# mooch443/trex

Measured on AMD Instinct MI355X. Metric: frames/s end-to-end (segment+CNN-ID), 2048x2048 x100 individuals, higher is better.
Workload: dtype fp16x3-split

## Files before the change

### include/trexhip.h

```cpp
#ifndef TREXHIP_H
#define TREXHIP_H
#include <stddef.h>
#include <stdint.h>
#ifdef __cplusplus
extern "C" {
#endif

#define TREXHIP_ABI_VERSION 25

enum {
    TREXHIP_OK = 0,
    TREXHIP_E_INVALID = -1,
    TREXHIP_E_DEVICE = -2,
    TREXHIP_E_CAPACITY = -3,
    TREXHIP_E_UNSUPPORTED = -4,
    TREXHIP_E_NOMEM = -5
};

#define TREXHIP_FRAME_OVERFLOW_RUNS   1u
#define TREXHIP_FRAME_OVERFLOW_OUTPUT 2u
#define TREXHIP_FRAME_MALFORMED       4u

typedef struct trexhip_params {
    int32_t device;
    int32_t width, height;
    int32_t max_batch;
    int32_t max_runs;
    int32_t max_blobs;
    int32_t max_pixels;
    int32_t threshold;
    int32_t threshold_maximum;
    int32_t enable_difference;
    int32_t absolute_difference;
    int32_t image_invert;
    int32_t inclusive;
    int32_t zero_is_background;
    int32_t connectivity;
    int32_t dilation_size;
    int32_t use_closing;
    int32_t closing_size;
    int32_t n_ranges;
    double  cm_per_pixel;
    double  ranges[16];
    int32_t pixel_encoding;
    int32_t image_adjust, blur_difference, equalize_histogram, correct_luminance, use_adaptive_threshold;
    int32_t device_color_reduce;
    int32_t reserved_[1];
} trexhip_params;
enum { TREXHIP_ENC_GRAY = 0, TREXHIP_ENC_R3G3B2 = 1, TREXHIP_ENC_RGB8 = 2 };

#define TREXHIP_BLOB_IN_RANGE    0u
#define TREXHIP_BLOB_BELOW_RANGE 1u
#define TREXHIP_BLOB_BIG         2u

typedef struct trexhip_run { uint16_t x0, x1, y, pad; } trexhip_run;

typedef struct trexhip_blob {
    uint32_t run_begin, n_runs;
    uint32_t pix_begin, n_pixels;
    uint16_t x0, y0, x1, y1;
    uint32_t bid;
// ... 21 lines not shown
    const trexhip_run* runs;
    const uint8_t* pixels;
    uint32_t pixel_channels;
    uint32_t reserved_;
} trexhip_batch_result;

typedef struct trexhip_device_view {
    const trexhip_frame_info* frames;
    const trexhip_blob* blobs;
    const trexhip_run* runs;
    const uint8_t* pixels;
    const uint32_t* totals;
    const uint32_t* blob_frame;
} trexhip_device_view;

typedef struct trexhip_ctx trexhip_ctx;

int trexhip_abi_version(void);
const char* trexhip_last_error(void);
void trexhip_default_params(trexhip_params* p, int32_t width, int32_t height);

int trexhip_create(const trexhip_params* p, trexhip_ctx** out);
void trexhip_destroy(trexhip_ctx* ctx);
typedef struct trexhip_live_params {
    int32_t threshold, threshold_maximum, inclusive;
    int32_t enable_difference, absolute_difference, image_invert, zero_is_background;
    int32_t n_ranges;
    double  cm_per_pixel;
    double  ranges[16];
} trexhip_live_params;
int trexhip_get_live_params(trexhip_ctx* ctx, trexhip_live_params* out);
int trexhip_update_params(trexhip_ctx* ctx, const trexhip_live_params* lp);
int trexhip_set_stream(trexhip_ctx* ctx, void* hip_stream);

int trexhip_set_background(trexhip_ctx* ctx, const uint8_t* gray, int32_t stride);
int trexhip_set_background_device(trexhip_ctx* ctx, const uint8_t* d_gray);
int trexhip_set_background_color(trexhip_ctx* ctx, const uint8_t* bgr, int32_t stride_bytes, int32_t channels, int32_t color_channel);
int trexhip_set_background_color_device(trexhip_ctx* ctx, const uint8_t* d_bgr, int32_t channels, int32_t color_channel);

int trexhip_generate_average_device(trexhip_ctx* ctx, const uint8_t* d_frames, int32_t n, int32_t method);
int trexhip_get_background(trexhip_ctx* ctx, uint8_t* gray, int32_t stride);

int trexhip_segment_device(trexhip_ctx* ctx, const uint8_t* d_frames, int32_t n);
int trexhip_segment(trexhip_ctx* ctx, const uint8_t* const* frames, int32_t stride, int32_t n);
int trexhip_segment_color(trexhip_ctx* ctx, const uint8_t* const* frames, int32_t stride, int32_t n,
                          int32_t channels, int32_t color_channel);
int trexhip_segment_color_device(trexhip_ctx* ctx, const uint8_t* d_color_frames, int32_t n, int32_t channels, int32_t color_channel);
int trexhip_pixel_channels(trexhip_ctx* ctx);
int trexhip_device_alloc(trexhip_ctx* ctx, size_t bytes, void** out_device_ptr);
int trexhip_device_free(trexhip_ctx* ctx, void* device_ptr);
int trexhip_copy_to_host(trexhip_ctx* ctx, void* host_dst, const void* device_src, size_t bytes);
int trexhip_copy_to_device(trexhip_ctx* ctx, void* device_dst, const void* host_src, size_t bytes);
int trexhip_fetch(trexhip_ctx* ctx, trexhip_batch_result* out);
int trexhip_device_view_get(trexhip_ctx* ctx, trexhip_device_view* out);
int trexhip_synchronize(trexhip_ctx* ctx);

int trexhip_pack_frames_v6_device(trexhip_ctx* ctx, const uint64_t* timestamps, uint8_t* d_out, size_t capacity, uint64_t* d_offsets);

int trexhip_load_frames_v6_device(trexhip_ctx* ctx, const uint8_t* d_bodies, const uint64_t* d_offsets, int32_t n_frames, uint64_t* d_timestamps);

size_t trexhip_lzo1x_bound(size_t n);
int trexhip_lzo1x_compress(const uint8_t* in, size_t n, uint8_t* out, size_t capacity, size_t* out_len);
int trexhip_pv_write_frames(const uint8_t* bodies, const uint64_t* offsets, int32_t n_frames, int32_t always_compress, uint64_t file_offset,
                            uint8_t* out, size_t capacity, uint64_t* index_table, size_t* out_bytes);
int trexhip_lzo1x_decompress(const uint8_t* in, size_t n, uint8_t* out, size_t capacity, size_t* out_len);
int trexhip_pv_read_frames(const uint8_t* data, size_t bytes, uint64_t file_offset, const uint64_t* index_table, int32_t n_frames,
                           uint8_t* bodies, size_t capacity, uint64_t* offsets, size_t* out_bytes);

int trexhip_rethreshold_device(trexhip_ctx* ctx, int32_t threshold, int32_t method, const double* size_ranges, int32_t n_ranges);
int trexhip_rethreshold_per_blob_device(trexhip_ctx* ctx, int32_t threshold, const int32_t* d_blob_thresholds, int32_t method,
                                        const double* size_ranges, int32_t n_ranges);
int trexhip_fetch_rethreshold(trexhip_ctx* ctx, trexhip_batch_result* out);

enum { TREXHIP_FILTER_OUTSIDE_INCLUDE = 0, TREXHIP_FILTER_INSIDE_IGNORE = 1, TREXHIP_FILTER_BDX_IGNORED = 2, TREXHIP_FILTER_OUTSIDE_RANGE = 3,
       TREXHIP_FILTER_SECOND_THRESHOLD = 4 };
enum { TREXHIP_DECISION_COMMITTED = 0, TREXHIP_DECISION_BIG = 1, TREXHIP_DECISION_FILTERED = 16, TREXHIP_DECISION_NONE = 255 };
typedef struct trexhip_prefilter_params {
    int32_t track_threshold;
    int32_t method;
    int32_t track_threshold_2;
    int32_t n_ranges;
    float   threshold_ratio_range[2];
    double  size_ranges[16];
} trexhip_prefilter_params;
typedef struct trexhip_prefilter_tables {
    const float*    d_include_points;  const int32_t* d_include_offsets;  int32_t n_include_shapes, n_include_points;
    const float*    d_ignore_points;   const int32_t* d_ignore_offsets;   int32_t n_ignore_shapes, n_ignore_points;
    const uint32_t* d_ignore_bdx;      const int32_t* d_ignore_bdx_offsets;  int32_t n_ignore_bdx, reserved_;
    int32_t*        d_second_count;
} trexhip_prefilter_tables;
void trexhip_default_prefilter_params(trexhip_prefilter_params* p);
int trexhip_prefilter_device(trexhip_ctx* ctx, const trexhip_prefilter_params* pp, const trexhip_prefilter_tables* tables ,
                             uint8_t* d_decision, int32_t* d_order, int32_t* d_counts, int32_t* d_presumed_nr);

typedef struct trexhip_split_params {
    int32_t track_threshold;
    int32_t track_posture_threshold;
    int32_t calculate_posture;
    int32_t algorithm;
    float   blob_split_max_shrink;
    float   blob_split_global_shrink_limit;
    int32_t n_ranges;
    int32_t reserved_;
    double  size_ranges[16];
} trexhip_split_params;
typedef struct trexhip_split_info {
// ... 18 lines not shown
    int32_t outline_smooth_step;
    int32_t outline_approximate;
    float   outline_curvature_range_ratio;
    float   midline_walk_offset;
    int32_t max_points;
    int32_t posture_closing_steps, peak_mode, posture_direction_smoothing;
} trexhip_posture_params;
typedef struct trexhip_posture_info { int32_t status, n_outline, n_segments, tail_index, head_index, n_traced, reserved[2]; } trexhip_posture_info;
void trexhip_default_posture_params(trexhip_posture_params* p);
int trexhip_posture_device(trexhip_ctx* ctx, int32_t table, const trexhip_posture_params* pp, int32_t n_blobs,
                           float* d_outline, float* d_segments, trexhip_posture_info* d_info);

int trexhip_posture_auto_device(trexhip_ctx* ctx, const trexhip_posture_params* pp, int32_t method, int32_t track_posture_threshold,
                                int32_t n_blobs, float* d_outline, float* d_segments, trexhip_posture_info* d_info,
                                int32_t* d_threshold_used, int32_t* d_iterations);

typedef struct trexhip_midline_params {
    int32_t midline_resolution;
    float   midline_stiff_percentage;
    int32_t midline_invert;
    int32_t midline_start_with_head;
} trexhip_midline_params;
typedef struct trexhip_midline_info { int32_t status, n; float len, angle, offx, offy; int32_t reserved[2]; } trexhip_midline_info;
void trexhip_default_midline_params(trexhip_midline_params* p);
int trexhip_midline_device(trexhip_ctx* ctx, const trexhip_midline_params* mp, int32_t n_blobs, int32_t max_points,
                           const trexhip_posture_info* d_posture_info, float* d_segments, float* d_midline,
                           trexhip_midline_info* d_midline_info);
int trexhip_midline_movement_device(trexhip_ctx* ctx, const trexhip_midline_params* mp, int32_t n_blobs, int32_t max_points,
                                    const trexhip_posture_info* d_posture_info, float* d_segments, float* d_midline,
                                    trexhip_midline_info* d_midline_info, const float* d_movement_direction);

enum { TREXHIP_NORMALIZE_NONE = 0, TREXHIP_NORMALIZE_MOMENTS = 1, TREXHIP_NORMALIZE_POSTURE = 2 };
int trexhip_crops_device(trexhip_ctx* ctx, uint8_t* d_crops, int32_t n_blobs, int32_t out_w, int32_t out_h,
                         int32_t normalization, int32_t difference);

int trexhip_crops_transformed_device(trexhip_ctx* ctx, uint8_t* d_crops, int32_t n_blobs, int32_t out_w, int32_t out_h,
                                     const float* transforms, const float* midline_lengths, int32_t use_legacy,
                                     float image_scale, int32_t difference);
int trexhip_crops_posture_device(trexhip_ctx* ctx, uint8_t* d_crops, int32_t n_blobs, int32_t out_w, int32_t out_h,
                                 const trexhip_midline_info* d_midline_info, const float* midline_lengths, int32_t use_legacy,
                                 float image_scale, int32_t difference);

int trexhip_load_weights(trexhip_ctx* ctx, const void* blob, size_t bytes);
int trexhip_num_classes(trexhip_ctx* ctx);
int trexhip_network_channels(trexhip_ctx* ctx);
int trexhip_network_image_size(trexhip_ctx* ctx, int32_t* width, int32_t* height);
enum { TREXHIP_NET_V118_3 = 0, TREXHIP_NET_V100 = 1, TREXHIP_NET_V110 = 2, TREXHIP_NET_V119 = 3, TREXHIP_NET_V200 = 4 };
int trexhip_network_version(trexhip_ctx* ctx);
size_t trexhip_network_blob_bytes(int32_t version, int32_t classes, int32_t channels, int32_t width, int32_t height);
int trexhip_identify_chunk_crops(trexhip_ctx* ctx, int32_t* crops);
enum { TREXHIP_CNN_FP32 = 0, TREXHIP_CNN_BF16X6 = 1, TREXHIP_CNN_BF16X3 = 2, TREXHIP_CNN_FP16X3 = 3 };
int trexhip_set_identity_precision(trexhip_ctx* ctx, int32_t mode);
int trexhip_identify_device(trexhip_ctx* ctx, const uint8_t* d_crops, int32_t n, float* d_probs, float* d_logits);
int trexhip_identify(trexhip_ctx* ctx, const uint8_t* crops, int32_t n, float* probs);
int trexhip_identify_guard_stats(trexhip_ctx* ctx, uint32_t* rerun_crops, uint32_t* whole_batch);
int trexhip_identify_skip_stats(trexhip_ctx* ctx, uint32_t* passes, uint32_t* listed, uint64_t* bytes_filled);

int trexhip_identify_skip3_stats(trexhip_ctx* ctx, uint32_t* pairs, uint32_t* listed, uint32_t* passes, uint64_t* bytes_filled);

int trexhip_identify_skip3x_stats(trexhip_ctx* ctx, uint32_t* crops_windowed, uint32_t* windowed_passes, uint32_t* full_passes);

int trexhip_identify_skipx_stats(trexhip_ctx* ctx, uint32_t* crops_windowed, uint32_t* windowed_passes, uint32_t* full_passes);

int trexhip_identify_bgrow_stats(trexhip_ctx* ctx, uint32_t* rows_read, uint32_t* rows_made);

int trexhip_identify_fc1_stats(trexhip_ctx* ctx, uint32_t* rows, uint32_t* listed);

int trexhip_export_id_table_device(trexhip_ctx* ctx, const float* d_probs, int32_t n_blobs, int32_t classes,
                                   uint32_t frame_base, void* d_table, int32_t max_rows);
int trexhip_export_id_table_ex_device(trexhip_ctx* ctx, const float* d_probs, int32_t n_blobs, int32_t classes, uint32_t frame_base,
                                      const float* d_midline, const trexhip_midline_info* d_midline_info, int32_t midline_resolution,
                                      void* d_table, int32_t max_rows);

typedef struct trexhip_comm trexhip_comm;
int trexhip_comm_unique_id(void* id128);
int trexhip_comm_create(trexhip_ctx* ctx, const void* id128, int32_t rank, int32_t world, trexhip_comm** out);
void trexhip_comm_destroy(trexhip_comm* comm);
int trexhip_comm_rank(trexhip_comm* comm);
int trexhip_comm_world(trexhip_comm* comm);
int trexhip_comm_gather_device(trexhip_comm* comm, const void* d_send, size_t bytes, void* d_recv_rank0);
int trexhip_comm_gather_device_on(trexhip_comm* comm, trexhip_ctx* stream_ctx, const void* d_send, size_t bytes, void* d_recv_rank0);
int trexhip_comm_count_ranks(trexhip_comm* comm, int32_t* ranks_seen);

enum { TREXHIP_STAGE_ROWS = 0, TREXHIP_STAGE_SEGMENT_ALL = 1, TREXHIP_STAGE_CONV2 = 2, TREXHIP_STAGE_CONV3 = 3,
       TREXHIP_STAGE_CNN_ALL = 4, TREXHIP_STAGE_CROPS = 5, TREXHIP_STAGE_POSTURE = 6,
       TREXHIP_STAGE_UPLOAD_COPY = 8, TREXHIP_STAGE_UPLOAD_DMA = 9, TREXHIP_STAGE_COUNT = 10 };
int trexhip_profile_enable(trexhip_ctx* ctx, int32_t on);
int trexhip_profile_read(trexhip_ctx* ctx, int32_t stage, double* total_ms, int64_t* launches);
int trexhip_profile_reset(trexhip_ctx* ctx);

#define TREXHIP_NET_CATEGORY 100
typedef struct trexhip_trainer trexhip_trainer;
typedef struct {
    int32_t max_batch;
    float lr;
    float beta1, beta2, eps;
    float bn_momentum;
    float dropout;
    int32_t precision;
    uint64_t seed;
} trexhip_train_params;
size_t trexhip_weight_blob_bytes(int32_t classes, int32_t channels);
int trexhip_trainer_create(trexhip_ctx* ctx, const void* blob, size_t bytes, const trexhip_train_params* params, trexhip_trainer** out);
void trexhip_trainer_destroy(trexhip_trainer* trainer);
int trexhip_trainer_set_lr(trexhip_trainer* trainer, float lr);
int64_t trexhip_trainer_steps(trexhip_trainer* trainer);
int trexhip_trainer_image_size(trexhip_trainer* trainer, int32_t* width, int32_t* height);
int trexhip_trainer_version(trexhip_trainer* trainer, int32_t* version);
size_t trexhip_trainer_keep_mask_bytes(trexhip_trainer* trainer, int32_t n);
int trexhip_train_step_device(trexhip_trainer* trainer, const float* d_inputs, const int32_t* d_targets, int32_t n, const uint8_t* d_keep_masks,
                              float* loss, int32_t* correct);
int trexhip_train_eval_device(trexhip_trainer* trainer, const float* d_inputs, const int32_t* d_targets, int32_t n, float* loss, int32_t* correct);
int trexhip_train_eval(trexhip_trainer* trainer, const float* inputs, const int32_t* targets, int32_t n, float* loss, int32_t* correct);
int trexhip_train_step(trexhip_trainer* trainer, const float* inputs, const int32_t* targets, int32_t n, const uint8_t* keep_masks, float* loss,
                       int32_t* correct);
int trexhip_train_predict_device(trexhip_trainer* trainer, const uint8_t* d_crops, int32_t n, float* d_probs);
int trexhip_trainer_read(trexhip_trainer* trainer, int32_t tensor, int32_t kind, float* out, size_t count);
int trexhip_trainer_export(trexhip_trainer* trainer, void* blob, size_t capacity, size_t* bytes);

typedef struct {
    float degrees;
    float translate_x, translate_y;
    float brightness_lo, brightness_hi;
    float contrast_lo, contrast_hi;
    float saturation_lo, saturation_hi;
    float hue_lo, hue_hi;
    uint64_t seed;
} trexhip_augment_params;
typedef struct {
    float angle; int32_t tx, ty;
    float brightness, contrast, saturation, hue;
    int32_t order;
} trexhip_augment_draw;
void trexhip_default_augment_params(trexhip_augment_params* p, int32_t width, int32_t height);
int trexhip_augment_device(trexhip_ctx* ctx, const trexhip_augment_params* ap, const uint8_t* d_pool, const int32_t* d_pool_targets,
                           int32_t pool_size, const int32_t* indices, int32_t n, int32_t width, int32_t height, int32_t channels,
                           trexhip_augment_draw* d_draws, int32_t draws_given, uint64_t counter, float* d_out, int32_t* d_targets_out);

typedef struct {
// ... 68 lines not shown
```

### trex_amd/capi.py

```python
import collections
import ctypes as C
import os
import numpy as np

_HERE = os.path.dirname(os.path.abspath(__file__))
LIB_PATH = os.environ.get("TREXHIP_LIB_PATH") or os.path.join(_HERE, "libtrexhip.so")
_LIB = None

RUN_DTYPE = np.dtype([("x0", "<u2"), ("x1", "<u2"), ("y", "<u2"), ("pad", "<u2")])
BLOB_DTYPE = np.dtype([
    ("run_begin", "<u4"), ("n_runs", "<u4"), ("pix_begin", "<u4"), ("n_pixels", "<u4"),
    ("x0", "<u2"), ("y0", "<u2"), ("x1", "<u2"), ("y1", "<u2"),
    ("bid", "<u4"), ("px_min_max", "<u4"), ("parent", "<u4"), ("flags", "<u4"),
    ("m10", "<u8"), ("m01", "<u8"), ("m20", "<u8"), ("m11", "<u8"), ("m02", "<u8"),
    ("sp", "<u8"), ("spx", "<u8"), ("spy", "<u8"),
])
INFO_DTYPE = np.dtype([
    ("n_blobs", "<u4"), ("n_runs", "<u4"), ("n_pixels", "<u4"),
    ("blob_begin", "<u4"), ("run_begin", "<u4"), ("pix_begin", "<u4"),
    ("n_raw_runs", "<u4"), ("n_raw_blobs", "<u4"), ("flags", "<u4"), ("reserved", "<u4", (3,)),
])
assert BLOB_DTYPE.itemsize == 104 and RUN_DTYPE.itemsize == 8 and INFO_DTYPE.itemsize == 48

CNN_FP32, CNN_BF16X6, CNN_BF16X3, CNN_FP16X3 = 0, 1, 2, 3
STAGE_ROWS, STAGE_SEGMENT_ALL, STAGE_CONV2, STAGE_CONV3, STAGE_CNN_ALL, STAGE_CROPS, STAGE_POSTURE = 0, 1, 2, 3, 4, 5, 6
STAGE_UPLOAD_COPY, STAGE_UPLOAD_DMA = 8, 9


class Params(C.Structure):
    _fields_ = [
        ("device", C.c_int32), ("width", C.c_int32), ("height", C.c_int32),
        ("max_batch", C.c_int32), ("max_runs", C.c_int32), ("max_blobs", C.c_int32), ("max_pixels", C.c_int32),
        ("threshold", C.c_int32), ("threshold_maximum", C.c_int32),
        ("enable_difference", C.c_int32), ("absolute_difference", C.c_int32),
        ("image_invert", C.c_int32), ("inclusive", C.c_int32), ("zero_is_background", C.c_int32),
        ("connectivity", C.c_int32), ("dilation_size", C.c_int32), ("use_closing", C.c_int32),
        ("closing_size", C.c_int32), ("n_ranges", C.c_int32),
        ("cm_per_pixel", C.c_double), ("ranges", C.c_double * 16),
        ("pixel_encoding", C.c_int32),
        ("image_adjust", C.c_int32), ("blur_difference", C.c_int32), ("equalize_histogram", C.c_int32), ("correct_luminance", C.c_int32),
        ("use_adaptive_threshold", C.c_int32), ("device_color_reduce", C.c_int32), ("reserved_", C.c_int32 * 1),
    ]


class LiveParams(C.Structure):
    _fields_ = [("threshold", C.c_int32), ("threshold_maximum", C.c_int32), ("inclusive", C.c_int32),
                ("enable_difference", C.c_int32), ("absolute_difference", C.c_int32), ("image_invert", C.c_int32), ("zero_is_background", C.c_int32),
                ("n_ranges", C.c_int32), ("cm_per_pixel", C.c_double), ("ranges", C.c_double * 16)]


class PostureParams(C.Structure):
    _fields_ = [("outline_resample", C.c_float), ("outline_smooth_samples", C.c_int32), ("outline_smooth_step", C.c_int32),
                ("outline_approximate", C.c_int32), ("outline_curvature_range_ratio", C.c_float),
                ("midline_walk_offset", C.c_float), ("max_points", C.c_int32),
                ("posture_closing_steps", C.c_int32), ("peak_mode", C.c_int32), ("posture_direction_smoothing", C.c_int32)]


class MidlineParams(C.Structure):
    _fields_ = [("midline_resolution", C.c_int32), ("midline_stiff_percentage", C.c_float), ("midline_invert", C.c_int32),
                ("midline_start_with_head", C.c_int32)]


class SplitParams(C.Structure):
    _fields_ = [("track_threshold", C.c_int32), ("track_posture_threshold", C.c_int32), ("calculate_posture", C.c_int32), ("algorithm", C.c_int32),
                ("blob_split_max_shrink", C.c_float), ("blob_split_global_shrink_limit", C.c_float), ("n_ranges", C.c_int32), ("reserved_", C.c_int32),
                ("size_ranges", C.c_double * 16)]


class PrefilterParams(C.Structure):
    _fields_ = [("track_threshold", C.c_int32), ("method", C.c_int32), ("track_threshold_2", C.c_int32), ("n_ranges", C.c_int32),
                ("threshold_ratio_range", C.c_float * 2), ("size_ranges", C.c_double * 16)]


class PrefilterTables(C.Structure):
    _fields_ = [("d_include_points", C.c_void_p), ("d_include_offsets", C.c_void_p), ("n_include_shapes", C.c_int32), ("n_include_points", C.c_int32),
                ("d_ignore_points", C.c_void_p), ("d_ignore_offsets", C.c_void_p), ("n_ignore_shapes", C.c_int32), ("n_ignore_points", C.c_int32),
                ("d_ignore_bdx", C.c_void_p), ("d_ignore_bdx_offsets", C.c_void_p), ("n_ignore_bdx", C.c_int32), ("reserved_", C.c_int32),
                ("d_second_count", C.c_void_p)]

# ... 58 lines not shown

AUGMENT_DRAW_DTYPE = np.dtype([("angle", "<f4"), ("tx", "<i4"), ("ty", "<i4"), ("brightness", "<f4"), ("contrast", "<f4"), ("saturation", "<f4"),
                               ("hue", "<f4"), ("order", "<i4")])
assert AUGMENT_DRAW_DTYPE.itemsize == 32
AUGMENT_IDENTITY_ORDER = 0xE4


class UniquenessResult(C.Structure):
    _fields_ = [("good_frames", C.c_uint32), ("bad_frames", C.c_uint32), ("good_ratio", C.c_float), ("mean_unique", C.c_float), ("mean_unique_raw", C.c_float)]


class ValidationMetrics:
    __slots__ = ("confusion", "per_class_accuracy", "good_frames", "bad_frames", "good_ratio", "mean_unique", "mean_unique_raw",
                 "unique_percent", "unique_percent_raw", "uniqueness_per_class")

    def __init__(self):
        for k in self.__slots__:
            setattr(self, k, None)


class ClassAverages:
    __slots__ = ("samples", "values", "max_index", "max_p")

    def __init__(self, samples, values, max_index, max_p):
        self.samples, self.values, self.max_index, self.max_p = samples, values, max_index, max_p


class VisualFieldResult:
    __slots__ = VF_OUTPUTS

    def __init__(self):
        for k in self.__slots__:
            setattr(self, k, None)


TrackletLabels = collections.namedtuple("TrackletLabels", "counts rows label share skipped")


SYMBOLS = [
    "trexhip_abi_version", "trexhip_network_channels", "trexhip_network_image_size", "trexhip_network_version", "trexhip_network_blob_bytes", "trexhip_identify_chunk_crops", "trexhip_comm_unique_id", "trexhip_comm_create", "trexhip_comm_destroy", "trexhip_comm_rank", "trexhip_comm_world", "trexhip_comm_gather_device", "trexhip_comm_gather_device_on", "trexhip_comm_count_ranks", "trexhip_last_error", "trexhip_default_params", "trexhip_create", "trexhip_destroy",
    "trexhip_set_stream", "trexhip_get_live_params", "trexhip_update_params", "trexhip_set_background", "trexhip_set_background_device", "trexhip_set_background_color", "trexhip_set_background_color_device", "trexhip_generate_average_device", "trexhip_get_background", "trexhip_segment_device",
    "trexhip_segment", "trexhip_segment_color", "trexhip_segment_color_device", "trexhip_rethreshold_device", "trexhip_rethreshold_per_blob_device", "trexhip_fetch_rethreshold", "trexhip_fetch", "trexhip_device_view_get", "trexhip_synchronize",
    "trexhip_profile_enable", "trexhip_profile_read", "trexhip_profile_reset",
    "trexhip_default_posture_params", "trexhip_posture_device", "trexhip_posture_auto_device", "trexhip_pack_frames_v6_device", "trexhip_crops_device", "trexhip_pixel_channels", "trexhip_device_alloc", "trexhip_device_free", "trexhip_copy_to_host", "trexhip_copy_to_device", "trexhip_crops_transformed_device", "trexhip_crops_posture_device", "trexhip_default_midline_params", "trexhip_midline_device", "trexhip_midline_movement_device", "trexhip_default_split_params", "trexhip_split_search_device", "trexhip_export_id_table_device", "trexhip_export_id_table_ex_device", "trexhip_load_weights", "trexhip_set_identity_precision", "trexhip_num_classes", "trexhip_identify_device", "trexhip_identify", "trexhip_identify_guard_stats", "trexhip_identify_skip_stats", "trexhip_identify_skip3_stats", "trexhip_identify_skip3x_stats", "trexhip_identify_skipx_stats", "trexhip_identify_bgrow_stats", "trexhip_identify_fc1_stats",
    "trexhip_weight_blob_bytes", "trexhip_trainer_create", "trexhip_trainer_destroy", "trexhip_trainer_set_lr", "trexhip_trainer_steps", "trexhip_trainer_image_size", "trexhip_trainer_version", "trexhip_trainer_keep_mask_bytes", "trexhip_train_step_device", "trexhip_train_step", "trexhip_train_eval_device", "trexhip_train_eval", "trexhip_trainer_read", "trexhip_trainer_export",
    "trexhip_default_augment_params", "trexhip_augment_device",
    "trexhip_train_predict_device", "trexhip_validation_metrics_device", "trexhip_class_averages_device",
    "trexhip_lzo1x_bound", "trexhip_lzo1x_compress", "trexhip_pv_write_frames",
    "trexhip_load_frames_v6_device", "trexhip_lzo1x_decompress", "trexhip_pv_read_frames",
    "trexhip_default_prefilter_params", "trexhip_prefilter_device",
    "trexhip_default_vf_params", "trexhip_visual_field_device",
    "trexhip_categorize_load_weights", "trexhip_categorize_info", "trexhip_categorize_blob_bytes", "trexhip_categorize_device", "trexhip_categorize",
    "trexhip_tracklet_labels_device", "trexhip_tracklet_medians_device",
]


def lib():
    global _LIB
    if _LIB is None:
        if not os.path.exists(LIB_PATH):
            raise TrexHipError(-1, f"{LIB_PATH} is missing: run __graft_entry__.build() (make -C trex_amd/csrc)")
        L = C.CDLL(LIB_PATH)
        L.trexhip_last_error.restype = C.c_char_p
        L.trexhip_default_params.argtypes = [C.POINTER(Params), C.c_int32, C.c_int32]
        L.trexhip_default_params.restype = None
        L.trexhip_create.argtypes = [C.POINTER(Params), C.POINTER(C.c_void_p)]
        L.trexhip_destroy.argtypes = [C.c_void_p]
        L.trexhip_destroy.restype = None
        L.trexhip_set_stream.argtypes = [C.c_void_p, C.c_void_p]
        L.trexhip_get_live_params.argtypes = [C.c_void_p, C.POINTER(LiveParams)]
        L.trexhip_update_params.argtypes = [C.c_void_p, C.POINTER(LiveParams)]
        L.trexhip_set_background.argtypes = [C.c_void_p, C.c_void_p, C.c_int32]
        L.trexhip_set_background_device.argtypes = [C.c_void_p, C.c_void_p]
        L.trexhip_set_background_color.argtypes = [C.c_void_p, C.c_void_p, C.c_int32, C.c_int32, C.c_int32]
        L.trexhip_set_background_color_device.argtypes = [C.c_void_p, C.c_void_p, C.c_int32, C.c_int32]
        L.trexhip_generate_average_device.argtypes = [C.c_void_p, C.c_void_p, C.c_int32, C.c_int32]
        L.trexhip_get_background.argtypes = [C.c_void_p, C.c_void_p, C.c_int32]
        L.trexhip_segment_device.argtypes = [C.c_void_p, C.c_void_p, C.c_int32]
        L.trexhip_segment.argtypes = [C.c_void_p, C.POINTER(C.c_void_p), C.c_int32, C.c_int32]
        L.trexhip_segment_color.argtypes = [C.c_void_p, C.POINTER(C.c_void_p), C.c_int32, C.c_int32, C.c_int32, C.c_int32]
        L.trexhip_segment_color_device.argtypes = [C.c_void_p, C.c_void_p, C.c_int32, C.c_int32, C.c_int32]
        L.trexhip_rethreshold_device.argtypes = [C.c_void_p, C.c_int32, C.c_int32, C.c_void_p, C.c_int32]
        L.trexhip_rethreshold_per_blob_device.argtypes = [C.c_void_p, C.c_int32, C.c_void_p, C.c_int32, C.c_void_p, C.c_int32]
        L.trexhip_fetch_rethreshold.argtypes = [C.c_void_p, C.POINTER(BatchResult)]
        L.trexhip_fetch.argtypes = [C.c_void_p, C.POINTER(BatchResult)]
        L.trexhip_device_view_get.argtypes = [C.c_void_p, C.POINTER(DeviceView)]
        L.trexhip_synchronize.argtypes = [C.c_void_p]
        L.trexhip_profile_enable.argtypes = [C.c_void_p, C.c_int32]
        L.trexhip_profile_read.argtypes = [C.c_void_p, C.c_int32, C.POINTER(C.c_double), C.POINTER(C.c_int64)]
        L.trexhip_profile_reset.argtypes = [C.c_void_p]
        L.trexhip_default_midline_params.argtypes = [C.POINTER(MidlineParams)]
        L.trexhip_default_midline_params.restype = None
        L.trexhip_midline_device.argtypes = [C.c_void_p, C.POINTER(MidlineParams), C.c_int32, C.c_int32, C.c_void_p, C.c_void_p, C.c_void_p, C.c_void_p]
        L.trexhip_midline_movement_device.argtypes = [C.c_void_p, C.POINTER(MidlineParams), C.c_int32, C.c_int32, C.c_void_p, C.c_void_p, C.c_void_p, C.c_void_p, C.c_void_p]
        L.trexhip_default_split_params.argtypes = [C.POINTER(SplitParams)]
        L.trexhip_default_split_params.restype = None
        L.trexhip_split_search_device.argtypes = [C.c_void_p, C.POINTER(SplitParams), C.c_int32, C.c_void_p, C.c_int32, C.c_void_p, C.c_void_p]
        L.trexhip_crops_posture_device.argtypes = [C.c_void_p, C.c_void_p, C.c_int32, C.c_int32, C.c_int32, C.c_void_p, C.c_void_p, C.c_int32, C.c_float, C.c_int32]
        L.trexhip_default_posture_params.argtypes = [C.POINTER(PostureParams)]
        L.trexhip_default_posture_params.restype = None
        L.trexhip_posture_device.argtypes = [C.c_void_p, C.c_int32, C.POINTER(PostureParams), C.c_int32, C.c_void_p, C.c_void_p, C.c_void_p]
        L.trexhip_posture_auto_device.argtypes = [C.c_void_p, C.POINTER(PostureParams), C.c_int32, C.c_int32, C.c_int32, C.c_void_p, C.c_void_p, C.c_void_p, C.c_void_p, C.c_void_p]
        L.trexhip_crops_transformed_device.argtypes = [C.c_void_p, C.c_void_p, C.c_int32, C.c_int32, C.c_int32, C.c_void_p, C.c_void_p, C.c_int32, C.c_float, C.c_int32]
        L.trexhip_crops_device.argtypes = [C.c_void_p, C.c_void_p] + [C.c_int32] * 5
        L.trexhip_export_id_table_device.argtypes = [C.c_void_p, C.c_void_p, C.c_int32, C.c_int32, C.c_uint32, C.c_void_p, C.c_int32]
        L.trexhip_export_id_table_ex_device.argtypes = [C.c_void_p, C.c_void_p, C.c_int32, C.c_int32, C.c_uint32, C.c_void_p, C.c_void_p, C.c_int32, C.c_void_p, C.c_int32]
        L.trexhip_load_weights.argtypes = [C.c_void_p, C.c_void_p, C.c_size_t]
        L.trexhip_num_classes.argtypes = [C.c_void_p]
        L.trexhip_network_channels.argtypes = [C.c_void_p]
        L.trexhip_network_image_size.argtypes = [C.c_void_p, C.POINTER(C.c_int32), C.POINTER(C.c_int32)]
        L.trexhip_network_version.argtypes = [C.c_void_p]
        L.trexhip_network_blob_bytes.argtypes = [C.c_int32] * 5; L.trexhip_network_blob_bytes.restype = C.c_size_t
        L.trexhip_identify_chunk_crops.argtypes = [C.c_void_p, C.POINTER(C.c_int32)]
        L.trexhip_pack_frames_v6_device.argtypes = [C.c_void_p, C.c_void_p, C.c_void_p, C.c_size_t, C.c_void_p]
        L.trexhip_lzo1x_bound.argtypes = [C.c_size_t]; L.trexhip_lzo1x_bound.restype = C.c_size_t
        L.trexhip_lzo1x_compress.argtypes = [C.c_void_p, C.c_size_t, C.c_void_p, C.c_size_t, C.POINTER(C.c_size_t)]
        L.trexhip_pv_write_frames.argtypes = [C.c_void_p, C.c_void_p, C.c_int32, C.c_int32, C.c_uint64, C.c_void_p, C.c_size_t, C.c_void_p, C.POINTER(C.c_size_t)]
        L.trexhip_load_frames_v6_device.argtypes = [C.c_void_p, C.c_void_p, C.c_void_p, C.c_int32, C.c_void_p]
        L.trexhip_lzo1x_decompress.argtypes = [C.c_void_p, C.c_size_t, C.c_void_p, C.c_size_t, C.POINTER(C.c_size_t)]
        L.trexhip_pv_read_frames.argtypes = [C.c_void_p, C.c_size_t, C.c_uint64, C.c_void_p, C.c_int32, C.c_void_p, C.c_size_t, C.c_void_p, C.POINTER(C.c_size_t)]
        L.trexhip_comm_unique_id.argtypes = [C.c_void_p]
        L.trexhip_comm_create.argtypes = [C.c_void_p, C.c_void_p, C.c_int32, C.c_int32, C.POINTER(C.c_void_p)]
        L.trexhip_comm_destroy.argtypes = [C.c_void_p]
        L.trexhip_comm_destroy.restype = None
        L.trexhip_comm_rank.argtypes = [C.c_void_p]
        L.trexhip_comm_world.argtypes = [C.c_void_p]
        L.trexhip_comm_gather_device.argtypes = [C.c_void_p, C.c_void_p, C.c_size_t, C.c_void_p]
        L.trexhip_comm_gather_device_on.argtypes = [C.c_void_p, C.c_void_p, C.c_void_p, C.c_size_t, C.c_void_p]
        L.trexhip_comm_count_ranks.argtypes = [C.c_void_p, C.POINTER(C.c_int32)]
        L.trexhip_set_identity_precision.argtypes = [C.c_void_p, C.c_int32]
        L.trexhip_identify_device.argtypes = [C.c_void_p, C.c_void_p, C.c_int32, C.c_void_p, C.c_void_p]
        L.trexhip_identify.argtypes = [C.c_void_p, C.c_void_p, C.c_int32, C.c_void_p]
        L.trexhip_identify_guard_stats.argtypes = [C.c_void_p, C.POINTER(C.c_uint32), C.POINTER(C.c_uint32)]
        L.trexhip_identify_skip_stats.argtypes = [C.c_void_p, C.POINTER(C.c_uint32), C.POINTER(C.c_uint32), C.POINTER(C.c_uint64)]
        L.trexhip_identify_skipx_stats.argtypes = [C.c_void_p, C.POINTER(C.c_uint32), C.POINTER(C.c_uint32), C.POINTER(C.c_uint32)]
        L.trexhip_identify_bgrow_stats.argtypes = [C.c_void_p, C.POINTER(C.c_uint32), C.POINTER(C.c_uint32)]
        L.trexhip_identify_skip3x_stats.argtypes = [C.c_void_p, C.POINTER(C.c_uint32), C.POINTER(C.c_uint32), C.POINTER(C.c_uint32)]
        L.trexhip_identify_skip3_stats.argtypes = [C.c_void_p, C.POINTER(C.c_uint32), C.POINTER(C.c_uint32), C.POINTER(C.c_uint32), C.POINTER(C.c_uint64)]
        L.trexhip_identify_fc1_stats.argtypes = [C.c_void_p, C.POINTER(C.c_uint32), C.POINTER(C.c_uint32)]
        L.trexhip_weight_blob_bytes.argtypes = [C.c_int32, C.c_int32]
        L.trexhip_weight_blob_bytes.restype = C.c_size_t
        L.trexhip_trainer_create.argtypes = [C.c_void_p, C.c_void_p, C.c_size_t, C.POINTER(TrainParams), C.POINTER(C.c_void_p)]
        L.trexhip_trainer_destroy.argtypes = [C.c_void_p]
        L.trexhip_trainer_destroy.restype = None
        L.trexhip_trainer_set_lr.argtypes = [C.c_void_p, C.c_float]
        L.trexhip_trainer_steps.argtypes = [C.c_void_p]
        L.trexhip_trainer_steps.restype = C.c_int64
        L.trexhip_trainer_image_size.argtypes = [C.c_void_p, C.POINTER(C.c_int32), C.POINTER(C.c_int32)]
        L.trexhip_trainer_version.argtypes = [C.c_void_p, C.POINTER(C.c_int32)]
        L.trexhip_trainer_keep_mask_bytes.argtypes = [C.c_void_p, C.c_int32]
        L.trexhip_trainer_keep_mask_bytes.restype = C.c_size_t
        L.trexhip_train_step_device.argtypes = [C.c_void_p, C.c_void_p, C.c_void_p, C.c_int32, C.c_void_p, C.POINTER(C.c_float), C.POINTER(C.c_int32)]
        L.trexhip_train_step.argtypes = [C.c_void_p, C.c_void_p, C.c_void_p, C.c_int32, C.c_void_p, C.POINTER(C.c_float), C.POINTER(C.c_int32)]
        L.trexhip_train_eval_device.argtypes = [C.c_void_p, C.c_void_p, C.c_void_p, C.c_int32, C.POINTER(C.c_float), C.POINTER(C.c_int32)]
        L.trexhip_train_eval.argtypes = [C.c_void_p, C.c_void_p, C.c_void_p, C.c_int32, C.POINTER(C.c_float), C.POINTER(C.c_int32)]
        L.trexhip_trainer_read.argtypes = [C.c_void_p, C.c_int32, C.c_int32, C.c_void_p, C.c_size_t]
        L.trexhip_trainer_export.argtypes = [C.c_void_p, C.c_void_p, C.c_size_t, C.POINTER(C.c_size_t)]
        L.trexhip_default_augment_params.argtypes = [C.POINTER(AugmentParams), C.c_int32, C.c_int32]
        L.trexhip_default_augment_params.restype = None
        L.trexhip_augment_device.argtypes = [C.c_void_p, C.POINTER(AugmentParams), C.c_void_p, C.c_void_p, C.c_int32, C.c_void_p, C.c_int32, C.c_int32, C.c_int32,
                                             C.c_int32, C.c_void_p, C.c_int32, C.c_uint64, C.c_void_p, C.c_void_p]
        L.trexhip_train_predict_device.argtypes = [C.c_void_p, C.c_void_p, C.c_int32, C.c_void_p]
        L.trexhip_validation_metrics_device.argtypes = [C.c_void_p, C.c_void_p, C.c_int32, C.c_int32, C.c_void_p, C.c_void_p, C.c_int32, C.c_void_p,
                                                        C.POINTER(UniquenessResult), C.c_void_p, C.c_void_p, C.c_void_p]
        L.trexhip_class_averages_device.argtypes = [C.c_void_p, C.c_void_p, C.c_int32, C.c_int32, C.c_void_p, C.c_int32, C.c_void_p, C.c_void_p, C.c_void_p, C.c_void_p]
        L.trexhip_device_alloc.argtypes = [C.c_void_p, C.c_size_t, C.POINTER(C.c_void_p)]
        L.trexhip_device_free.argtypes = [C.c_void_p, C.c_void_p]
        L.trexhip_copy_to_host.argtypes = [C.c_void_p, C.c_void_p, C.c_void_p, C.c_size_t]
        L.trexhip_copy_to_device.argtypes = [C.c_void_p, C.c_void_p, C.c_void_p, C.c_size_t]
        L.trexhip_default_prefilter_params.argtypes = [C.POINTER(PrefilterParams)]
        L.trexhip_default_prefilter_params.restype = None
        L.trexhip_prefilter_device.argtypes = [C.c_void_p, C.POINTER(PrefilterParams), C.POINTER(PrefilterTables), C.c_void_p, C.c_void_p, C.c_void_p, C.c_void_p]
        L.trexhip_default_vf_params.argtypes = [C.c_void_p, C.POINTER(VfParams)]
        L.trexhip_default_vf_params.restype = None
        L.trexhip_visual_field_device.argtypes = [C.c_void_p, C.POINTER(VfParams), C.c_void_p, C.c_void_p, C.c_void_p, C.c_int32, C.c_void_p, C.c_int32,
                                                  C.c_void_p, C.c_int32, C.c_void_p, C.c_void_p, C.c_void_p, C.c_void_p, C.c_void_p, C.c_void_p]
        L.trexhip_categorize_load_weights.argtypes = [C.c_void_p, C.c_void_p, C.c_size_t]
        L.trexhip_categorize_info.argtypes = [C.c_void_p, C.POINTER(C.c_int32), C.POINTER(C.c_int32), C.POINTER(C.c_int32), C.POINTER(C.c_int32)]
        L.trexhip_categorize_blob_bytes.argtypes = [C.c_int32, C.c_int32, C.c_int32, C.c_int32]
        L.trexhip_categorize_blob_bytes.restype = C.c_size_t
        L.trexhip_categorize_device.argtypes = [C.c_void_p, C.c_void_p, C.c_int32, C.c_void_p, C.c_void_p, C.c_void_p]
        L.trexhip_categorize.argtypes = [C.c_void_p, C.c_void_p, C.c_int32, C.c_void_p]
        L.trexhip_tracklet_labels_device.argtypes = [C.c_void_p, C.c_void_p, C.c_void_p, C.c_int32, C.c_int32, C.c_int32, C.c_void_p, C.c_void_p, C.c_void_p,
                                                     C.c_void_p, C.POINTER(C.c_uint32)]
# ... 110 lines not shown
            bg = np.ascontiguousarray(bg, np.uint8)
            assert bg.shape == (self.params.height, self.params.width)
            _check(lib().trexhip_set_background(self._h, bg.ctypes.data_as(C.c_void_p), bg.shape[1]))
        else:
            assert bg.is_cuda and bg.is_contiguous() and bg.numel() == self.params.height * self.params.width
            _check(lib().trexhip_set_background_device(self._h, C.c_void_p(bg.data_ptr())))

    def generate_average(self, d_frames_ptr, n, method=0):
        _check(lib().trexhip_generate_average_device(self._h, C.c_void_p(d_frames_ptr), n, method))
        out = np.empty((self.params.height, self.params.width), np.uint8)
        _check(lib().trexhip_get_background(self._h, out.ctypes.data_as(C.c_void_p), out.shape[1]))
        return out

    def get_background(self):
        out = np.empty((self.params.height, self.params.width), np.uint8)
        _check(lib().trexhip_get_background(self._h, out.ctypes.data_as(C.c_void_p), out.shape[1]))
        return out

    def segment_device(self, d_ptr, n):
        _check(lib().trexhip_segment_device(self._h, C.c_void_p(d_ptr), n))

    def segment_host(self, frames):
        frames = [np.ascontiguousarray(f, np.uint8) for f in frames]
        ptrs = (C.c_void_p * len(frames))(*[f.ctypes.data for f in frames])
        stride = frames[0].shape[1] if frames else self.params.width
        _check(lib().trexhip_segment(self._h, ptrs, stride, len(frames)))

    def set_background_color(self, bgc, color_channel=-1):
        bgc = np.ascontiguousarray(bgc, np.uint8)
        assert bgc.shape[:2] == (self.params.height, self.params.width)
        _check(lib().trexhip_set_background_color(self._h, bgc.ctypes.data_as(C.c_void_p), bgc.shape[1] * bgc.shape[2], bgc.shape[2], color_channel))

    def segment_color_host(self, frames, color_channel=-1):
        frames = [np.ascontiguousarray(f, np.uint8) for f in frames]
        ch = frames[0].shape[2]
        ptrs = (C.c_void_p * len(frames))(*[f.ctypes.data for f in frames])
        _check(lib().trexhip_segment_color(self._h, ptrs, frames[0].shape[1] * ch, len(frames), ch, color_channel))

    def segment_color_device(self, d_color_ptr, n, channels, color_channel=-1):
        _check(lib().trexhip_segment_color_device(self._h, C.c_void_p(d_color_ptr), n, channels, color_channel))

    def synchronize(self):
        _check(lib().trexhip_synchronize(self._h))

    def fetch_raw(self, rethreshold=False):
        r = BatchResult()
        rc = (lib().trexhip_fetch_rethreshold if rethreshold else lib().trexhip_fetch)(self._h, C.byref(r))
        if rc != 0 and rc != -3:
            _check(rc)
        if rc == -3:
            self.last_capacity_error = lib().trexhip_last_error().decode()
        return r

    def fetch(self, copy=True, rethreshold=False):
        r = BatchResult()
        rc = (lib().trexhip_fetch_rethreshold if rethreshold else lib().trexhip_fetch)(self._h, C.byref(r))
        malformed = rc == -1 and r.n_frames > 0 and bool((_from_addr(r.frames, r.n_frames, INFO_DTYPE)["flags"] & FRAME_MALFORMED).any())
        if rc != 0 and rc != -3 and not malformed:
            _check(rc)
        info = _from_addr(r.frames, r.n_frames, INFO_DTYPE)
        blobs = _from_addr(r.blobs, r.total_blobs, BLOB_DTYPE)
        runs = _from_addr(r.runs, r.total_runs, RUN_DTYPE)
        pc = int(r.pixel_channels) or 1
        pixels = _from_addr(r.pixels, r.total_pixels * pc, np.dtype(np.uint8))
        out = []
        for i in range(r.n_frames):
            fi = info[i]
            if fi["flags"]:
                out.append(FrameResult(fi.copy(), np.zeros(0, BLOB_DTYPE), np.zeros(0, RUN_DTYPE), np.zeros(0, np.uint8)))
                continue
            b = blobs[fi["blob_begin"]:fi["blob_begin"] + fi["n_blobs"]]
            ru = runs[fi["run_begin"]:fi["run_begin"] + fi["n_runs"]]
            px = pixels[int(fi["pix_begin"]) * pc:(int(fi["pix_begin"]) + int(fi["n_pixels"])) * pc]
            if copy:
                b, ru, px = b.copy(), ru.copy(), px.copy()
            out.append(FrameResult(fi.copy(), b, ru, px))
        if malformed:
            e = TrexHipError(rc, lib().trexhip_last_error().decode())
            e.frames = out
            raise e
        if rc == -3:
            self.last_capacity_error = lib().trexhip_last_error().decode()
        return out

    def posture_device(self, n_blobs, d_outline_ptr, d_segments_ptr, d_info_ptr, table=0, **kw):
        pp = PostureParams()
        lib().trexhip_default_posture_params(C.byref(pp))
        for k, v in kw.items():
            setattr(pp, k, v)
        _check(lib().trexhip_posture_device(self._h, table, C.byref(pp), n_blobs, C.c_void_p(d_outline_ptr),
                                            C.c_void_p(d_segments_ptr), C.c_void_p(d_info_ptr)))
        return pp

    def posture_auto_device(self, n_blobs, d_outline_ptr, d_segments_ptr, d_info_ptr, method=0, track_posture_threshold=15, d_threshold_ptr=0, d_iterations_ptr=0, **kw):
        pp = PostureParams()
        lib().trexhip_default_posture_params(C.byref(pp))
        for k, v in kw.items():
            setattr(pp, k, v)
        _check(lib().trexhip_posture_auto_device(self._h, C.byref(pp), method, track_posture_threshold, n_blobs, C.c_void_p(d_outline_ptr),
                                                 C.c_void_p(d_segments_ptr), C.c_void_p(d_info_ptr), C.c_void_p(d_threshold_ptr or 0), C.c_void_p(d_iterations_ptr or 0)))

    def pack_frames_v6_device(self, d_out_ptr, capacity, d_offsets_ptr, timestamps=None):
        ts = np.ascontiguousarray(timestamps, np.uint64) if timestamps is not None else None
        _check(lib().trexhip_pack_frames_v6_device(self._h, ts.ctypes.data if ts is not None else None, C.c_void_p(d_out_ptr), capacity, C.c_void_p(d_offsets_ptr)))

    def load_frames_v6_device(self, d_bodies_ptr, d_offsets_ptr, n, d_timestamps_ptr=0):
# ... 70 lines not shown
        return int(c.value)

    def probabilities(self, crops):
        crops = np.ascontiguousarray(crops, np.uint8)
        w, h = self.network_image_size()
        if w:
            want = (h, w, lib().trexhip_network_channels(self._h))
            if crops.ndim != 4 or tuple(crops.shape[1:]) != want:
                raise ValueError(f"crops must have shape (n, {want[0]}, {want[1]}, {want[2]}) for the loaded network, got {crops.shape}")
        n = crops.shape[0]
        out = np.empty((n, self.num_classes()), np.float32)
        _check(lib().trexhip_identify(self._h, crops.ctypes.data_as(C.c_void_p), n, out.ctypes.data_as(C.c_void_p)))
        return out

    def guard_stats(self):
        a, b = C.c_uint32(0), C.c_uint32(0)
        _check(lib().trexhip_identify_guard_stats(self._h, C.byref(a), C.byref(b)))
        return int(a.value), bool(b.value)

    def skip_stats(self):
        a, b, c = C.c_uint32(0), C.c_uint32(0), C.c_uint64(0)
        _check(lib().trexhip_identify_skip_stats(self._h, C.byref(a), C.byref(b), C.byref(c)))
        return int(a.value), int(b.value), int(c.value)

    def skipx_stats(self):
        a, b, c = C.c_uint32(0), C.c_uint32(0), C.c_uint32(0)
        _check(lib().trexhip_identify_skipx_stats(self._h, C.byref(a), C.byref(b), C.byref(c)))
        return int(a.value), int(b.value), int(c.value)

    def bgrow_stats(self):
        a, b = C.c_uint32(0), C.c_uint32(0)
        _check(lib().trexhip_identify_bgrow_stats(self._h, C.byref(a), C.byref(b)))
        return int(a.value), int(b.value)

    def skip3_stats(self):
        a, b, c, d = C.c_uint32(0), C.c_uint32(0), C.c_uint32(0), C.c_uint64(0)
        _check(lib().trexhip_identify_skip3_stats(self._h, C.byref(a), C.byref(b), C.byref(c), C.byref(d)))
        return int(a.value), int(b.value), int(c.value), int(d.value)

    def skip3x_stats(self):
        a, b, c = C.c_uint32(0), C.c_uint32(0), C.c_uint32(0)
        _check(lib().trexhip_identify_skip3x_stats(self._h, C.byref(a), C.byref(b), C.byref(c)))
        return int(a.value), int(b.value), int(c.value)

    def fc1_stats(self):
        a, b = C.c_uint32(0), C.c_uint32(0)
        _check(lib().trexhip_identify_fc1_stats(self._h, C.byref(a), C.byref(b)))
        return int(a.value), int(b.value)

    def identify_device(self, d_crops_ptr, n, d_probs_ptr, d_logits_ptr=None):
        _check(lib().trexhip_identify_device(self._h, C.c_void_p(d_crops_ptr), n, C.c_void_p(d_probs_ptr),
                                             C.c_void_p(d_logits_ptr) if d_logits_ptr else None))

    def device_alloc(self, nbytes):
        out = C.c_void_p()
        _check(lib().trexhip_device_alloc(self._h, nbytes, C.byref(out)))
        return int(out.value)

    def device_free(self, d_ptr):
        _check(lib().trexhip_device_free(self._h, C.c_void_p(d_ptr or 0)))

    def copy_to_device(self, d_ptr, array):
        a = np.ascontiguousarray(array)
        _check(lib().trexhip_copy_to_device(self._h, C.c_void_p(d_ptr), a.ctypes.data_as(C.c_void_p), a.nbytes))

    def copy_to_host(self, d_ptr, shape, dtype):
        out = np.empty(shape, dtype)
        _check(lib().trexhip_copy_to_host(self._h, out.ctypes.data_as(C.c_void_p), C.c_void_p(d_ptr), out.nbytes))
        return out

    def augment_device(self, d_pool_ptr, pool_size, n, width, height, channels, d_out_ptr, ap=None, indices=None, d_pool_targets_ptr=0,
                       d_targets_out_ptr=0, d_draws_ptr=0, draws_given=False, counter=0):
        idx = None
        if indices is not None:
            idx = np.ascontiguousarray(indices, np.int32)
            if idx.shape != (n,):
                raise ValueError(f"indices must hold n = {n} entries, got shape {idx.shape}")
        _check(lib().trexhip_augment_device(self._h, C.byref(ap) if ap is not None else None, C.c_void_p(d_pool_ptr), C.c_void_p(d_pool_targets_ptr or 0), pool_size,
                                            idx.ctypes.data_as(C.c_void_p) if idx is not None else None, n, width, height, channels,
                                            C.c_void_p(d_draws_ptr or 0), 1 if draws_given else 0, counter, C.c_void_p(d_out_ptr), C.c_void_p(d_targets_out_ptr or 0)))

    def validation_metrics(self, d_probs_ptr, n, classes, d_targets_ptr=0, frame_ranges=None):
        out = ValidationMetrics()
        conf = np.zeros((classes, classes), np.uint32) if d_targets_ptr else None
        fr = None
        res = UniquenessResult()
        up = upr = upc = None
        if frame_ranges is not None:
            fr = np.ascontiguousarray(frame_ranges, np.int32).reshape(-1, 2)
            up, upr, upc = np.zeros(len(fr), np.float32), np.zeros(len(fr), np.float32), np.zeros(classes, np.float32)
        ptr = lambda a: a.ctypes.data_as(C.c_void_p) if a is not None else None
        _check(lib().trexhip_validation_metrics_device(self._h, C.c_void_p(d_probs_ptr or 0), n, classes, C.c_void_p(d_targets_ptr or 0), ptr(fr),
                                                       len(fr) if fr is not None else 0, ptr(conf), C.byref(res) if fr is not None else None,
                                                       ptr(up), ptr(upr), ptr(upc)))
        if conf is not None:
            rows = conf.sum(axis=1, dtype=np.int64)
            out.confusion = conf
            out.per_class_accuracy = np.zeros(classes, np.float64)
            np.divide(np.diagonal(conf), rows, out=out.per_class_accuracy, where=rows > 0)
        if fr is not None:
            out.good_frames, out.bad_frames = int(res.good_frames), int(res.bad_frames)
            out.good_ratio, out.mean_unique, out.mean_unique_raw = float(res.good_ratio), float(res.mean_unique), float(res.mean_unique_raw)
            out.unique_percent, out.unique_percent_raw, out.uniqueness_per_class = up, upr, upc
        return out

    def class_averages(self, d_probs_ptr, n, classes, d_ids_ptr, n_ids):
# ... 442 lines not shown
```

### trex_amd/csrc/capi.hip

```cpp
#include "internal.h"
#include "cnn_plan.h"
#include <cstdio>
#include <cstring>
#include <cstdlib>
#include <algorithm>
#include <new>
#include <vector>

namespace trexhip {

static thread_local std::string g_error;
void set_error(const std::string& msg) { g_error = msg; }

static void stage_fold(Stage& s, bool all) {
    size_t keep = 0;
    for (size_t i = 0; i < s.pending.size(); ++i) {
        EvPair p = s.pending[i];
        hipError_t q = all ? hipEventSynchronize(p.b) : hipEventQuery(p.b);
        float ms = 0.f;
        if (q == hipSuccess && hipEventElapsedTime(&ms, p.a, p.b) == hipSuccess) {
            s.total_ms += ms; s.launches++;
            s.freelist.push_back(p);
        } else if (q == hipErrorNotReady) {
            s.pending[keep++] = p;
// ... 6 lines not shown
}
void stage_begin(trexhip_ctx* ctx, int stage) {
    if (!ctx->profiling) return;
    Stage& s = ctx->stages[stage];
    if (s.pending.size() > 1024) stage_fold(s, false);
    EvPair p;
    if (!s.freelist.empty()) { p = s.freelist.back(); s.freelist.pop_back(); }
    else {
        hipEventCreateWithFlags(&p.a, hipEventDisableSystemFence); hipEventCreateWithFlags(&p.b, hipEventDisableSystemFence);
    }
    hipEventRecord(p.a, ctx->stream);
    s.cur = p;
}
void stage_end(trexhip_ctx* ctx, int stage) {
    if (!ctx->profiling) return;
    Stage& s = ctx->stages[stage];
    if (!s.cur.a) return;
    hipEventRecord(s.cur.b, ctx->stream);
    s.pending.push_back(s.cur);
    s.cur = EvPair();
}
void stage_read(trexhip_ctx* ctx, int stage) { stage_fold(ctx->stages[stage], true); }
void stage_free(trexhip_ctx* ctx) {
    for (auto& s : ctx->stages) {
        stage_fold(s, true);
        for (auto& p : s.freelist) { hipEventDestroy(p.a); hipEventDestroy(p.b); }
        s.freelist.clear();
    }
}

static int alloc_tables(Mem& m, BlobTables& t, LabelState& l, size_t B, size_t H, size_t R, size_t NB, size_t P, size_t pix_ch, const char* who) {
    int rc = TREXHIP_OK;
#define TRY(x) do { if (rc == TREXHIP_OK) rc = (x); } while (0)
    TRY(m.device(&l.d_row_cnt, B * H, who)); TRY(m.device(&l.d_row_base, B * (H + 1), who)); TRY(m.device(&l.d_raster, B * R, who));
    TRY(m.device(&l.d_parent, B * R, who)); TRY(m.device(&l.d_root_ord, B * R, who)); TRY(m.device(&l.d_cnt_runs, B * R, who));
    TRY(m.device(&l.d_cnt_px, B * R, who)); TRY(m.device(&l.d_cur_run, B * R, who)); TRY(m.device(&l.d_pix_begin, B * R, who));
    TRY(m.device(&l.d_blob_map, B * R, who));
    if (!t.d_totals) TRY(m.device(&t.d_totals, 4, who));
    TRY(m.device(&t.d_info, B, who)); TRY(m.device(&t.d_blobs, B * NB, who)); TRY(m.device(&t.d_blob_frame, B * NB, who));
    TRY(m.device(&t.d_runs, B * R, who)); TRY(m.device(&t.d_pixels, B * P * pix_ch, who));
    TRY(m.pinned(&t.h_info, B, who)); TRY(m.pinned(&t.h_totals, 4, who)); TRY(m.pinned(&t.h_blobs, B * NB, who));
    TRY(m.pinned(&t.h_runs, B * R, who)); TRY(m.pinned(&t.h_pixels, B * P * pix_ch, who));
#undef TRY
    return rc;
}

static int fetch_info(trexhip_ctx* ctx, BlobTables& t) {
    TH_CHECK_HIP(hipMemcpyAsync(t.h_info, t.d_info, sizeof(trexhip_frame_info) * t.valid_n, hipMemcpyDeviceToHost, ctx->stream));
    TH_CHECK_HIP(hipMemcpyAsync(t.h_totals, t.d_totals, sizeof(uint32_t) * 4, hipMemcpyDeviceToHost, ctx->stream));
    TH_CHECK_HIP(hipStreamSynchronize(ctx->stream));
    return TREXHIP_OK;
}

static int fetch_tables(trexhip_ctx* ctx, BlobTables& t, bool copy, trexhip_batch_result* out) {
    std::memset(out, 0, sizeof(*out));
    out->n_frames = t.valid_n;
    out->frames = t.h_info; out->blobs = t.h_blobs; out->runs = t.h_runs; out->pixels = t.h_pixels;
    out->pixel_channels = (uint32_t)ctx->pix_ch;
    if (t.valid_n == 0) return TREXHIP_OK;
    const uint32_t tb = std::min(t.h_totals[0], ctx->cfg.pool_blobs), tr = std::min(t.h_totals[1], ctx->cfg.pool_runs), tp = std::min(t.h_totals[2], ctx->cfg.pool_pixels);
    if (copy) {
        hipStream_t s = ctx->stream;
        if (tb) TH_CHECK_HIP(hipMemcpyAsync(t.h_blobs, t.d_blobs, sizeof(trexhip_blob) * tb, hipMemcpyDeviceToHost, s));
        if (tr) TH_CHECK_HIP(hipMemcpyAsync(t.h_runs, t.d_runs, sizeof(trexhip_run) * tr, hipMemcpyDeviceToHost, s));
        if (tp) TH_CHECK_HIP(hipMemcpyAsync(t.h_pixels, t.d_pixels, (size_t)tp * ctx->pix_ch, hipMemcpyDeviceToHost, s));
        TH_CHECK_HIP(hipStreamSynchronize(s));
    }
    out->total_blobs = tb; out->total_runs = tr; out->total_pixels = tp;
    t.fetched = true;
    return TREXHIP_OK;
}

static int fill_cfg(trexhip_ctx* ctx) {
    const trexhip_params& p = ctx->p;
    SegCfg& c = ctx->cfg;
    c.W = p.width; c.H = p.height; c.B = p.max_batch; c.ctr_frames = p.max_batch; c.R = p.max_runs;
    c.T = p.height * TREXHIP_ROW_SLOT + p.max_runs;
    const int thr = p.threshold < 0 ? -p.threshold : p.threshold;
    if (p.threshold_maximum < 255) { c.tmin = thr; c.tmax = p.threshold_maximum; }
    else { c.tmin = p.inclusive ? thr : thr + 1; c.tmax = 255; }
    c.enable_diff = p.enable_difference; c.absdiff = p.absolute_difference;
    c.invert = p.image_invert; c.zero_bg = p.zero_is_background;
    c.slack = p.connectivity == 4 ? 0 : 1;
    c.n_ranges = p.n_ranges;
    c.sqcm = (float)(p.cm_per_pixel * p.cm_per_pixel);
    for (int i = 0; i < 16; ++i) c.ranges[i] = p.ranges[i];
    c.pool_blobs = (uint32_t)p.max_batch * (uint32_t)p.max_blobs;
    c.pool_runs = (uint32_t)p.max_batch * (uint32_t)p.max_runs;
    c.pool_pixels = (uint32_t)p.max_batch * (uint32_t)p.max_pixels;
    c.cap_blobs = (uint32_t)p.max_blobs; c.cap_pixels = (uint32_t)p.max_pixels;
    return TREXHIP_OK;
}

}

using namespace trexhip;

extern "C" int trexhip_rethreshold_per_blob_device(trexhip_ctx* ctx, int32_t threshold, const int32_t* d_blob_thresholds, int32_t method,
                                                   const double* size_ranges, int32_t n_ranges);

extern "C" {

int trexhip_abi_version(void) { return TREXHIP_ABI_VERSION; }
const char* trexhip_last_error(void) { return g_error.c_str(); }

void trexhip_default_params(trexhip_params* p, int32_t width, int32_t height) {
    if (!p) return;
    std::memset(p, 0, sizeof(*p));
    p->device = 0;
    p->width = width; p->height = height;
    p->max_batch = 16;
    p->max_runs = 65536;
    p->max_blobs = 2048;
    p->max_pixels = 1 << 20;
    p->threshold = 15; p->threshold_maximum = 255;
    p->enable_difference = 1; p->absolute_difference = 1;
    p->image_invert = 0; p->zero_is_background = 1;
    p->inclusive = 1;
    p->connectivity = 8;
// ... 28 lines not shown
    if (p->n_ranges < 0 || p->n_ranges > 8) { set_error("trexhip_create: n_ranges must be 0..8"); return TREXHIP_E_INVALID; }
    if ((p->use_closing && (p->closing_size < 1 || p->closing_size > 15)) || p->dilation_size > 7 || p->dilation_size < -7) {
        set_error("trexhip_create: structuring elements larger than 15x15 are not supported (closing_size <= 15, |dilation_size| <= 7)");
        return TREXHIP_E_UNSUPPORTED;
    }
    if (p->pixel_encoding < 0 || p->pixel_encoding > 2) { set_error("trexhip_create: pixel_encoding must be TREXHIP_ENC_GRAY / R3G3B2 / RGB8"); return TREXHIP_E_INVALID; }
    if (p->pixel_encoding != TREXHIP_ENC_GRAY && p->image_invert) {
        set_error("trexhip_create: image_invert with a colour pixel_encoding is not supported"); return TREXHIP_E_UNSUPPORTED;
    }
    int ndev = 0;
    TH_CHECK_HIP(hipGetDeviceCount(&ndev));
    if (p->device < 0 || p->device >= ndev) { set_error("trexhip_create: no such HIP device"); return TREXHIP_E_DEVICE; }
    TH_CHECK_HIP(hipSetDevice(p->device));
    trexhip_ctx* ctx = new (std::nothrow) trexhip_ctx();
    if (!ctx) { set_error("out of host memory"); return TREXHIP_E_NOMEM; }
    ctx->p = *p;
    ctx->pix_ch = p->pixel_encoding == TREXHIP_ENC_RGB8 ? 3 : 1;
    fill_cfg(ctx);
    { int cus = 0; if (hipDeviceGetAttribute(&cus, hipDeviceAttributeMultiprocessorCount, p->device) == hipSuccess && cus > 0) ctx->n_cus = cus; }
    if (const char* e = std::getenv("TREXHIP_CONV_GEOM")) ctx->tune_conv_geom = std::atoi(e) & GEOM_MASK;
    if (const char* e = std::getenv("TREXHIP_CCL_BANDS")) ctx->tune_ccl_bands = std::atoi(e);
    const size_t B = p->max_batch, H = p->height, W = p->width, R = p->max_runs, NB = p->max_blobs, P = p->max_pixels;
    if (hipStreamCreateWithFlags(&ctx->own_stream, hipStreamNonBlocking) != hipSuccess) { set_error("hipStreamCreate failed"); delete ctx; return TREXHIP_E_DEVICE; }
    ctx->stream = ctx->own_stream;
    Mem& m = ctx->mem;
    const char* who = "trexhip_create";
    int rc = m.device(&ctx->d_bg, H * W + 16, who);
#define TRY(x) do { if (rc == TREXHIP_OK) rc = (x); } while (0)
    TRY(m.device(&ctx->d_ctr, B * TREXHIP_CTR_STRIDE + 4, who));
    if (rc == TREXHIP_OK && hipMemset(ctx->d_ctr, 0, sizeof(uint32_t) * (B * TREXHIP_CTR_STRIDE + 4)) != hipSuccess) { set_error("hipMemset of the counters failed"); rc = TREXHIP_E_DEVICE; }
    TRY(m.device(&ctx->d_band_fail, B, who));
    if (rc == TREXHIP_OK && hipMemset(ctx->d_band_fail, 0, sizeof(uint32_t) * B) != hipSuccess) { set_error("hipMemset of the band flags failed"); rc = TREXHIP_E_DEVICE; }
    TRY(m.device(&ctx->d_row_off, B * H, who));
    TRY(m.device(&ctx->d_tmp_runs, B * (H * TREXHIP_ROW_SLOT + R), who));
    if (rc == TREXHIP_OK) ctx->tables.d_totals = ctx->d_ctr + B * TREXHIP_CTR_STRIDE;
    TRY(alloc_tables(m, ctx->tables, ctx->label, B, H, R, NB, P, ctx->pix_ch, who));
    ctx->tables.fetched = true;
    if (p->use_closing || p->dilation_size != 0) {
        const size_t WBw = (W + 31) / 32;
        TRY(m.device(&ctx->d_bits[0], B * H * WBw + 4, who));
        TRY(m.device(&ctx->d_bits[1], B * H * WBw + 4, who));
    }
    TRY(m.pinned(&ctx->h_ccl_hint, 2, who));
    if (rc == TREXHIP_OK) ctx->h_ccl_hint[0] = ctx->h_ccl_hint[1] = 0u;
#undef TRY
    if (rc != TREXHIP_OK) { trexhip_destroy(ctx); return rc; }
    *out = ctx;
    return TREXHIP_OK;
}

void trexhip_destroy(trexhip_ctx* ctx) {
    if (!ctx) return;
    hipSetDevice(ctx->p.device);
    if (ctx->stream) hipStreamSynchronize(ctx->stream);
    net_free(ctx);
    ctx->pass2.mem.free_all();
    upload_free(ctx);
    ctx->mem.free_all();
    stage_free(ctx);
    if (ctx->own_stream) hipStreamDestroy(ctx->own_stream);
    delete ctx;
}

int trexhip_pixel_channels(trexhip_ctx* ctx) { return ctx ? ctx->pix_ch : 0; }

int trexhip_device_alloc(trexhip_ctx* ctx, size_t bytes, void** out_device_ptr) {
    if (!ctx || !out_device_ptr) { set_error("trexhip_device_alloc: null argument"); return TREXHIP_E_INVALID; }
    *out_device_ptr = nullptr;
    TH_CHECK_HIP(hipSetDevice(ctx->p.device));
    TH_CHECK_HIP(hipMalloc(out_device_ptr, bytes ? bytes : 1));
    return TREXHIP_OK;
}

int trexhip_device_free(trexhip_ctx* ctx, void* device_ptr) {
    if (!ctx) { set_error("null ctx"); return TREXHIP_E_INVALID; }
    if (!device_ptr) return TREXHIP_OK;
    TH_CHECK_HIP(hipSetDevice(ctx->p.device));
    TH_CHECK_HIP(hipStreamSynchronize(ctx->stream));
    TH_CHECK_HIP(hipFree(device_ptr));
    return TREXHIP_OK;
}

int trexhip_copy_to_host(trexhip_ctx* ctx, void* host_dst, const void* device_src, size_t bytes) {
    if (!ctx || (bytes && (!host_dst || !device_src))) { set_error("trexhip_copy_to_host: null argument"); return TREXHIP_E_INVALID; }
    TH_CHECK_HIP(hipSetDevice(ctx->p.device));
    if (bytes) TH_CHECK_HIP(hipMemcpyAsync(host_dst, device_src, bytes, hipMemcpyDeviceToHost, ctx->stream));
    TH_CHECK_HIP(hipStreamSynchronize(ctx->stream));
    return TREXHIP_OK;
}

int trexhip_copy_to_device(trexhip_ctx* ctx, void* device_dst, const void* host_src, size_t bytes) {
    if (!ctx || (bytes && (!device_dst || !host_src))) { set_error("trexhip_copy_to_device: null argument"); return TREXHIP_E_INVALID; }
    TH_CHECK_HIP(hipSetDevice(ctx->p.device));
    if (bytes) TH_CHECK_HIP(hipMemcpyAsync(device_dst, host_src, bytes, hipMemcpyHostToDevice, ctx->stream));
    TH_CHECK_HIP(hipStreamSynchronize(ctx->stream));
    return TREXHIP_OK;
}

int trexhip_get_live_params(trexhip_ctx* ctx, trexhip_live_params* out) {
    if (!ctx || !out) { set_error("trexhip_get_live_params: null argument"); return TREXHIP_E_INVALID; }
    const trexhip_params& p = ctx->p;
    std::memset(out, 0, sizeof(*out));
    out->threshold = p.threshold; out->threshold_maximum = p.threshold_maximum; out->inclusive = p.inclusive;
    out->enable_difference = p.enable_difference; out->absolute_difference = p.absolute_difference;
    out->image_invert = p.image_invert; out->zero_is_background = p.zero_is_background;
    out->n_ranges = p.n_ranges; out->cm_per_pixel = p.cm_per_pixel;
    for (int i = 0; i < 16; ++i) out->ranges[i] = p.ranges[i];
    return TREXHIP_OK;
}

int trexhip_update_params(trexhip_ctx* ctx, const trexhip_live_params* lp) {
    if (!ctx || !lp) { set_error("trexhip_update_params: null argument"); return TREXHIP_E_INVALID; }
    if (lp->n_ranges < 0 || lp->n_ranges > 8) { set_error("trexhip_update_params: n_ranges must be 0..8 (detect_size_filter with more than 8 ranges is not supported)"); return TREXHIP_E_INVALID; }
    if (!(lp->cm_per_pixel > 0.0)) { set_error("trexhip_update_params: cm_per_pixel must be positive"); return TREXHIP_E_INVALID; }
    if (ctx->p.pixel_encoding != TREXHIP_ENC_GRAY && lp->image_invert) {
        set_error("trexhip_update_params: image_invert with a colour pixel_encoding is not supported"); return TREXHIP_E_UNSUPPORTED;
    }
    trexhip_params& p = ctx->p;
    p.threshold = lp->threshold; p.threshold_maximum = lp->threshold_maximum; p.inclusive = lp->inclusive;
    p.enable_difference = lp->enable_difference; p.absolute_difference = lp->absolute_difference;
    p.image_invert = lp->image_invert; p.zero_is_background = lp->zero_is_background;
    p.n_ranges = lp->n_ranges; p.cm_per_pixel = lp->cm_per_pixel;
    for (int i = 0; i < 16; ++i) p.ranges[i] = i < 2 * lp->n_ranges ? lp->ranges[i] : 0.0;
    return fill_cfg(ctx);
}

int trexhip_set_stream(trexhip_ctx* ctx, void* hip_stream) {
    if (!ctx) { set_error("null ctx"); return TREXHIP_E_INVALID; }
    TH_CHECK_HIP(hipStreamSynchronize(ctx->stream));
    ctx->stream = hip_stream ? reinterpret_cast<hipStream_t>(hip_stream) : ctx->own_stream;
    return TREXHIP_OK;
}

int trexhip_set_background(trexhip_ctx* ctx, const uint8_t* gray, int32_t stride) {
    if (!ctx || !gray) { set_error("trexhip_set_background: null argument"); return TREXHIP_E_INVALID; }
    if (stride < ctx->p.width) { set_error("trexhip_set_background: stride < width"); return TREXHIP_E_INVALID; }
    TH_CHECK_HIP(hipSetDevice(ctx->p.device));
    TH_CHECK_HIP(hipMemcpy2DAsync(ctx->d_bg, ctx->p.width, gray, stride, ctx->p.width, ctx->p.height,
                                  hipMemcpyHostToDevice, ctx->stream));
    TH_CHECK_HIP(hipStreamSynchronize(ctx->stream));
    ctx->has_bg = true;
    return TREXHIP_OK;
}

int trexhip_set_background_device(trexhip_ctx* ctx, const uint8_t* d_gray) {
    if (!ctx || !d_gray) { set_error("trexhip_set_background_device: null argument"); return TREXHIP_E_INVALID; }
    TH_CHECK_HIP(hipSetDevice(ctx->p.device));
    TH_CHECK_HIP(hipMemcpyAsync(ctx->d_bg, d_gray, (size_t)ctx->p.width * ctx->p.height, hipMemcpyDeviceToDevice, ctx->stream));
    TH_CHECK_HIP(hipStreamSynchronize(ctx->stream));
    ctx->has_bg = true;
    return TREXHIP_OK;
}

static int check_segment_args(trexhip_ctx* ctx, const void* frames, int32_t n) {
    if (!ctx || !frames) { set_error("trexhip_segment: null argument"); return TREXHIP_E_INVALID; }
    if (!ctx->has_bg) { set_error("trexhip_segment: background image not set"); return TREXHIP_E_INVALID; }
    if (n < 0 || n > ctx->p.max_batch) { set_error("trexhip_segment: n outside 0..max_batch"); return TREXHIP_E_INVALID; }
    return TREXHIP_OK;
}

int trexhip_segment_device(trexhip_ctx* ctx, const uint8_t* d_frames, int32_t n) {
    int rc = check_segment_args(ctx, d_frames, n);
    if (rc) return rc;
    if (ctx->pix_ch != 1 || ctx->p.pixel_encoding != TREXHIP_ENC_GRAY) { set_error("trexhip_segment_device: a colour pixel_encoding needs colour input (trexhip_segment_color*)"); return TREXHIP_E_INVALID; }
    ctx->d_color_src = nullptr; ctx->color_ch = 0;
    TH_CHECK_HIP(hipSetDevice(ctx->p.device));
    if (n == 0) { ctx->tables.valid_n = 0; ctx->tables.fetched = false; return TREXHIP_OK; }
    return launch_segment(ctx, d_frames, n);
}

int trexhip_segment(trexhip_ctx* ctx, const uint8_t* const* frames, int32_t stride, int32_t n) {
    int rc = check_segment_args(ctx, frames, n);
    if (rc) return rc;
    if (ctx->p.pixel_encoding != TREXHIP_ENC_GRAY) { set_error("trexhip_segment: a colour pixel_encoding needs colour input (trexhip_segment_color*)"); return TREXHIP_E_INVALID; }
    ctx->d_color_src = nullptr; ctx->color_ch = 0;
    if (stride < ctx->p.width) { set_error("trexhip_segment: stride < width"); return TREXHIP_E_INVALID; }
    TH_CHECK_HIP(hipSetDevice(ctx->p.device));
    if (n == 0) { ctx->tables.valid_n = 0; ctx->tables.fetched = false; return TREXHIP_OK; }
    const size_t W = ctx->p.width, H = ctx->p.height;
    rc = ensure_staging(ctx, "trexhip_segment");
    if (rc) return rc;
    for (int i = 0; i < n; ++i)
        if (!frames[i]) { set_error("trexhip_segment: null frame pointer"); return TREXHIP_E_INVALID; }
    rc = upload_frames(ctx, frames, n, H, W, (size_t)stride, ctx->d_staging, nullptr);
    if (rc) return rc;
    return launch_segment(ctx, ctx->d_staging, n);
}

int trexhip_synchronize(trexhip_ctx* ctx) {
    if (!ctx) { set_error("null ctx"); return TREXHIP_E_INVALID; }
    TH_CHECK_HIP(hipStreamSynchronize(ctx->stream));
    return TREXHIP_OK;
}


}
namespace trexhip {
__global__ __launch_bounds__(256) void k_export(const trexhip_frame_info* __restrict__ info, const uint32_t* __restrict__ totals,
                                                const trexhip_blob* __restrict__ blobs, const trexhip_run* __restrict__ runs, const uint8_t* __restrict__ pixels,
                                                trexhip_frame_info* __restrict__ h_info, uint32_t* __restrict__ h_totals, trexhip_blob* __restrict__ h_blobs,
                                                trexhip_run* __restrict__ h_runs, uint8_t* __restrict__ h_pixels, const int n,
                                                const uint32_t pool_blobs, const uint32_t pool_runs, const uint32_t pool_pixels, const int pix_ch) {
    const uint32_t tb = min(totals[0], pool_blobs), tr = min(totals[1], pool_runs), tp = min(totals[2], pool_pixels);
    const size_t gtid = (size_t)blockIdx.x * 256 + threadIdx.x, gstep = (size_t)gridDim.x * 256;
    auto words = [&](const void* src, void* dst, const size_t nw) {
        const uint32_t* a = static_cast<const uint32_t*>(src);
        uint32_t* b = static_cast<uint32_t*>(dst);
        for (size_t i = gtid; i < nw; i += gstep) b[i] = a[i];
    };
    words(info, h_info, (size_t)n * sizeof(trexhip_frame_info) / 4);
    if (gtid < 4) h_totals[gtid] = totals[gtid];
    words(blobs, h_blobs, (size_t)tb * sizeof(trexhip_blob) / 4);
    words(runs, h_runs, (size_t)tr * sizeof(trexhip_run) / 4);
    const size_t pb = (size_t)tp * pix_ch;
    words(pixels, h_pixels, pb / 4);
    if (gtid < (pb & 3)) h_pixels[(pb & ~(size_t)3) + gtid] = pixels[(pb & ~(size_t)3) + gtid];
}
static_assert(sizeof(trexhip_frame_info) % 4 == 0 && sizeof(trexhip_blob) % 4 == 0 && sizeof(trexhip_run) % 4 == 0, "k_export copies 4-byte words");
static constexpr int EXPORT_MAX_FRAMES = 16;
static int export_or_fetch_info(trexhip_ctx* ctx, bool by_kernel) {
    BlobTables& t = ctx->tables;
    if (!by_kernel) return fetch_info(ctx, t);
    hipLaunchKernelGGL(k_export, dim3(32), dim3(256), 0, ctx->stream, t.d_info, t.d_totals, t.d_blobs, t.d_runs, t.d_pixels, t.h_info, t.h_totals, t.h_blobs,
                       t.h_runs, t.h_pixels, t.valid_n, ctx->cfg.pool_blobs, ctx->cfg.pool_runs, ctx->cfg.pool_pixels, ctx->pix_ch);
    TH_CHECK_HIP(hipGetLastError());
    TH_CHECK_HIP(hipStreamSynchronize(ctx->stream));
    return TREXHIP_OK;
}
}
extern "C" {

int trexhip_fetch(trexhip_ctx* ctx, trexhip_batch_result* out) {
    if (!ctx || !out) { set_error("trexhip_fetch: null argument"); return TREXHIP_E_INVALID; }
    TH_CHECK_HIP(hipSetDevice(ctx->p.device));
    BlobTables& t = ctx->tables;
    const int n = t.valid_n;
    const bool by_kernel = n <= EXPORT_MAX_FRAMES;
    if (n) {
        int rc1 = export_or_fetch_info(ctx, by_kernel);
        if (rc1) return rc1;
        bool pending = false;
        for (int i = 0; i < n; ++i) pending |= t.h_info[i].reserved[0] == 1u;
        if (pending) {
            rc1 = launch_pending(ctx);
            if (rc1 == TREXHIP_OK) rc1 = export_or_fetch_info(ctx, by_kernel);
            if (rc1) return rc1;
        }
    }
    int rc = fetch_tables(ctx, t, !by_kernel, out);
    if (rc || n == 0) return rc;
    for (int i = 0; i < n; ++i)
        if (t.h_info[i].flags & TREXHIP_FRAME_MALFORMED) {
            char buf[160];
            std::snprintf(buf, sizeof(buf), "frame %d of the batch is malformed: its V_6 body breaks the layout (flags=%u); it holds no blobs", i, t.h_info[i].flags);
            set_error(buf);
            return TREXHIP_E_INVALID;
        }
    for (int i = 0; i < n; ++i)
        if (t.h_info[i].flags) {
            char buf[160];
            std::snprintf(buf, sizeof(buf), "frame %d of the batch exceeded capacity (flags=%u, raw runs=%u): raise max_runs/max_blobs/max_pixels",
                          i, t.h_info[i].flags, t.h_info[i].n_raw_runs);
            set_error(buf);
            rc = TREXHIP_E_CAPACITY;
        }
    return rc;
}

static int pass2_alloc(trexhip_ctx* ctx, const char* who) {
    Pass2& q = ctx->pass2;
    if (q.allocated) return TREXHIP_OK;
    const size_t B = ctx->p.max_batch, R = ctx->p.max_runs;
    int rc = alloc_tables(q.mem, q.tables, q.label, B, ctx->p.height, R, ctx->p.max_blobs, ctx->p.max_pixels, ctx->pix_ch, who);
    if (rc == TREXHIP_OK) rc = q.mem.device(&q.d_sub_cnt, B * R, who);
    if (rc == TREXHIP_OK) rc = q.mem.device(&q.d_sub_base, B * R, who);
    if (rc == TREXHIP_OK) rc = q.mem.device(&q.d_run_parent, B * R, who);
    if (rc != TREXHIP_OK) { q.mem.free_all(); q = Pass2(); }
    q.allocated = rc == TREXHIP_OK;
    return rc;
}

int trexhip_rethreshold_device(trexhip_ctx* ctx, int32_t threshold, int32_t method, const double* size_ranges, int32_t n_ranges) {
    return trexhip_rethreshold_per_blob_device(ctx, threshold, nullptr, method, size_ranges, n_ranges);
}

int trexhip_rethreshold_per_blob_device(trexhip_ctx* ctx, int32_t threshold, const int32_t* d_blob_thresholds, int32_t method,
                                        const double* size_ranges, int32_t n_ranges) {
    int rc = trexhip::rethreshold_prepare(ctx, "trexhip_rethreshold_device", method, size_ranges, n_ranges);
    if (rc) return rc;
    return launch_rethreshold(ctx, threshold, method, size_ranges, n_ranges, d_blob_thresholds);
}

int trexhip_fetch_rethreshold(trexhip_ctx* ctx, trexhip_batch_result* out) {
    if (!ctx || !out) { set_error("trexhip_fetch_rethreshold: null argument"); return TREXHIP_E_INVALID; }
    Pass2& q = ctx->pass2;
    if (!q.allocated || q.tables.valid_n == 0) { set_error("trexhip_fetch_rethreshold: no re-thresholded batch"); return TREXHIP_E_INVALID; }
    TH_CHECK_HIP(hipSetDevice(ctx->p.device));
    const int n = q.tables.valid_n;
    int rc = fetch_info(ctx, q.tables);
    if (rc == TREXHIP_OK) rc = fetch_tables(ctx, q.tables, true, out);
    if (rc) return rc;
    for (int i = 0; i < n; ++i)
        if (q.tables.h_info[i].flags) { set_error("a frame exceeded capacity during re-threshold: raise max_runs/max_blobs/max_pixels"); return TREXHIP_E_CAPACITY; }
    return TREXHIP_OK;
}

int trexhip_device_view_get(trexhip_ctx* ctx, trexhip_device_view* out) {
    if (!ctx || !out) { set_error("trexhip_device_view_get: null argument"); return TREXHIP_E_INVALID; }
    out->frames = ctx->tables.d_info; out->blobs = ctx->tables.d_blobs; out->runs = ctx->tables.d_runs; out->pixels = ctx->tables.d_pixels;
    out->totals = ctx->tables.d_totals; out->blob_frame = ctx->tables.d_blob_frame;
    return TREXHIP_OK;
}

int trexhip_profile_enable(trexhip_ctx* ctx, int32_t on) {
    if (!ctx) { set_error("null ctx"); return TREXHIP_E_INVALID; }
    ctx->profiling = on != 0;
    return TREXHIP_OK;
}

int trexhip_profile_read(trexhip_ctx* ctx, int32_t stage, double* total_ms, int64_t* launches) {
    if (!ctx || stage < 0 || stage >= TREXHIP_STAGE_COUNT) { set_error("trexhip_profile_read: bad argument"); return TREXHIP_E_INVALID; }
// ... 44 lines not shown
```

### trex_amd/csrc/cnn.hip

```cpp
#include "cnn_net.h"
#include "cnn_arch.h"
#include "cnn_split.h"
#include "conv_tiled.h"
#include "cnn_weights.h"
#include <algorithm>
#include <cmath>
#include <cstdio>
#include <cstdlib>
#include <cstring>
#include <vector>

namespace trexhip {

template <int CH>
__global__ __launch_bounds__(256, 2) void k_conv1(const uint8_t* __restrict__ crops, const float* __restrict__ w ,
                                                  const float* __restrict__ bias , float* __restrict__ out, int S) {
    extern __shared__ __attribute__((aligned(16))) float lds[];
    const int PW = S + 4;
    float* wl = lds;
    float* img = lds + CH * 25 * 16;
    const int crop = blockIdx.x;
    const uint8_t* src = crops + (size_t)crop * S * S * CH;
    for (int i = threadIdx.x; i < CH * PW * PW; i += 256) img[i] = 0.f;
    for (int i = threadIdx.x; i < CH * 25 * 16; i += 256) wl[i] = w[i];
// ... 1112 lines not shown
                lg[r] = s;
                if (logits_out) logits_out[(size_t)crop * C + c] = s;
            }
            mx = fmaxf(mx, lg[r]);
        }
    }
    mx = wave_max(mx);
#pragma unroll
    for (int r = 0; r < 16; ++r)
        if (r < nrep && r * 64 + lane < C) { lg[r] = expf(lg[r] - mx); sum += lg[r]; }
    sum = 1.f / wave_sum(sum);
#pragma unroll
    for (int r = 0; r < 16; ++r)
        if (r < nrep && r * 64 + lane < C) probs[(size_t)crop * C + r * 64 + lane] = lg[r] * sum;
}

static void destroy_graph_entry(Net::GraphEntry& g) {
    if (g.exec) {
        if (g.last) (void)hipEventSynchronize(g.last);
        (void)hipGraphExecDestroy(g.exec);
    }
    if (g.last) (void)hipEventDestroy(g.last);
    g.exec = nullptr; g.last = nullptr;
}
static void drop_graphs(Net* n) {
    for (auto& g : n->graphs) destroy_graph_entry(g);
    n->graphs.clear();
}

void free_net(Net* n) {
    if (!n) return;
    drop_graphs(n);
    delete n->arch;
    n->weights.free_all();
    n->batch.free_all();
    delete n;
}

template <class T>
static int upload(Net* net, T** dst, const void* data, size_t bytes) {
    const int rc = net->weights.device_bytes(dst, bytes, "trexhip_load_weights");
    if (rc != TREXHIP_OK) return rc;
    TH_CHECK_HIP(hipMemcpy(*dst, data, bytes, hipMemcpyHostToDevice));
    return TREXHIP_OK;
}
template <class T, class V>
static int upload(Net* net, T** dst, const std::vector<V>& v) { return upload(net, dst, v.data(), v.size() * sizeof(V)); }
template <class T>
static int upload(Net* net, T** dst, float* inv, const ScaledImage& im) { *inv = im.inv; return upload(net, dst, im.v); }

#define TRY(x) do { if (rc == TREXHIP_OK) rc = (x); } while (0)
static int make_empty_v3(trexhip_ctx* ctx, Net* net);
int net_load(trexhip_ctx* ctx, const void* blob, size_t bytes) {
    const int arch = blob_arch_id(blob, bytes);
    if (arch >= TREXHIP_NET_V100 && arch <= TREXHIP_NET_V200) return arch_load(ctx, blob, bytes);
    WeightBlob wb;
    const int prc = parse_weight_blob(blob, bytes, "trexhip_load_weights", &wb, [](int W, int H) -> int {
        if (W < 8 || W > 256 || H < 8 || H > 256) {
            set_error("trexhip_load_weights: individual_image_size " + std::to_string(W) + "x" + std::to_string(H) + " is outside 8..256 x 8..256");
            return TREXHIP_E_UNSUPPORTED;
        }
        return TREXHIP_OK;
    });
    if (prc != TREXHIP_OK) return prc;
    const int classes = wb.classes, W = wb.W, H = wb.H, CH = wb.CH;
    const bool at80 = W == 80 && H == 80;

    TH_CHECK_HIP(hipSetDevice(ctx->p.device));
    free_net(static_cast<Net*>(ctx->net));
    ctx->net = nullptr;
    Net* net = new Net();
    net->classes = classes; net->W = W; net->H = H; net->CH = CH;
    int rc = TREXHIP_OK;
    const Folded c1 = fold_conv1(&wb.t[T_C1W], CH);
    TRY(upload(net, &net->w1, c1.w)); TRY(upload(net, &net->b1, c1.b));
    if (at80) TRY(upload(net, &net->w1h, &net->inv1h, pack_conv1_frags(c1.w, CH)));
    const Folded c2 = fold_conv(&wb.t[T_C2W], 64, 16, 16);
    TRY(upload(net, &net->w2, c2.w)); TRY(upload(net, &net->b2, c2.b));
    TRY(upload(net, &net->w2s, pack_bf16x3(c2.w, 16, 64)));
    TRY(upload(net, &net->w2h, &net->inv2h, pack_f16x2(c2.w, 16, 64)));
    if (at80) TRY(upload(net, &net->w2w, &net->inv2w, pack_wino_f16(c2.w, 16, 64)));
    const Folded c3 = fold_conv(&wb.t[T_C3W], 128, 64, 16);
    TRY(upload(net, &net->w3s, pack_bf16x3(c3.w, 64, 128)));
    TRY(upload(net, &net->w3h, &net->inv3h, pack_f16x2(c3.w, 64, 128)));
    if (at80) TRY(upload(net, &net->w3w, &net->inv3w, pack_wino_f16(c3.w, 64, 128)));
    TRY(net->weights.device_bytes(&net->d_ovf, OVF_WORDS * 4, "trexhip_load_weights"));
    if (rc == TREXHIP_OK && hipMemset(net->d_ovf, 0, OVF_WORDS * 4) != hipSuccess) rc = TREXHIP_E_DEVICE;
    const Folded c3x = fold_conv(&wb.t[T_C3W], 128, 64, 32);
    TRY(upload(net, &net->w3, c3x.w)); TRY(upload(net, &net->b3, c3x.b));
    const Folded f1 = pack_fc1(wb.t[T_F1W], wb.t[T_F1B], W, H);
    TRY(upload(net, &net->wf1, f1.w)); TRY(upload(net, &net->bf1, f1.b));
    if (at80) TRY(upload(net, &net->wf1h, &net->invf1h, pack_fc1_f16(f1.w)));
    TRY(upload(net, &net->lng, wb.t[T_LNG], 100 * sizeof(float)));
    TRY(upload(net, &net->lnb, wb.t[T_LNB], 100 * sizeof(float)));
    TRY(upload(net, &net->wf2t, pack_fc2(wb.t[T_F2W], classes)));
    TRY(upload(net, &net->bf2, wb.t[T_F2B], classes * sizeof(float)));
    if (at80 && CH == 1) TRY(make_empty_v3(ctx, net));
    if (rc != TREXHIP_OK) { free_net(net); return rc; }
    ctx->net = net;
    return TREXHIP_OK;
}

static int ensure_act(trexhip_ctx* ctx, Net* net, int n) {
    if (n <= net->max_crops) return TREXHIP_OK;
    drop_graphs(net);
    net->batch.free_all();
    net->h_probs = nullptr;
    net->max_crops = 0;
    Mem& B = net->batch;
    const char* who = "trexhip_identify_device";
    const size_t N = n;
    const size_t W = net->W, H = net->H;
    int rc = B.device_bytes(&net->d_ovfc, N, who);
    TRY(B.device_bytes(&net->act1, N * (H / 2) * (W / 2) * 16 * 4, who));
    TRY(B.device_bytes(&net->act2, N * (H / 4) * (W / 4) * 64 * 4, who));
    TRY(B.device_bytes(&net->act3, N * (H / 8) * (W / 8) * 128 * 4, who));
    TRY(B.device_bytes(&net->fc1, N * 128 * 4 * FC1_KSPLIT, who));
    TRY(B.device_bytes(&net->probs, N * net->classes * 4, who));
    TRY(B.device_bytes(&net->logits, N * net->classes * 4, who));
    if (W == 80 && H == 80) {
        TRY(B.device_bytes(&net->v2, N * 40 * V2_ROWB, who));
        const size_t img = net->v3e ? (size_t)SkipGeom::V3_ROWS * V3_ROWB : 0;
        TRY(B.device_bytes(&net->v3, N * 20 * V3_ROWB + 2 * img, who));
        if (rc == TREXHIP_OK && img) {
            TH_CHECK_HIP(hipMemcpyAsync(net->v3, net->v3e, img, hipMemcpyDeviceToDevice, ctx->stream));
            TH_CHECK_HIP(hipMemcpyAsync(net->v3 + img + N * 20 * V3_ROWB, net->v3e, img, hipMemcpyDeviceToDevice, ctx->stream));
            net->v3 += img;
        }
    }
    if (net->v3e) {
        const size_t n_pass = (N * SkipGeom::V3_ROWS + SkipGeom::RPP - 1) / SkipGeom::RPP;
        TRY(B.device_bytes(&net->skip_bands, N * sizeof(int2), who));
        TRY(B.device_bytes(&net->skip_counts, ((n_pass + SKIP_LB - 1) / SKIP_LB) * SKIP_NCNT * 4, who));
        TRY(B.device_bytes(&net->skip_list, (n_pass + SKIP_PAD) * 4, who));
        TRY(B.device_bytes(&net->skipx_cols, N * sizeof(int2), who));
        TRY(B.device_bytes(&net->skipx_list, (N * skipx_passes({0, SkipGeom::V3_ROWS - 1}) + SKIP_PAD) * 4, who));
        TRY(B.device_bytes(&net->skipx_rows, (N * skipx_passes({0, SkipGeom::V3_ROWS - 1}) + SKIP_PAD) * 4, who));
        const size_t blocks3 = (N + Skip3Geom::BLOCK - 1) / Skip3Geom::BLOCK;
        TRY(B.device_bytes(&net->skip3_counts, ((blocks3 + SKIP3_TB - 1) / SKIP3_TB) * sizeof(uint4), who));
        TRY(B.device_bytes(&net->skip3_tcounts, blocks3 * 2 * sizeof(uint32_t), who));
        TRY(B.device_bytes(&net->skip3_desc, blocks3 * Skip3Geom::BLOCK_PASSES * Skip3Geom::DESC * 4, who));
        TRY(B.device_bytes(&net->skip3_rows, blocks3 * Skip3Geom::BLOCK_PASSES * Skip3Reach::WORDS * 4, who));
        TRY(B.device_bytes(&net->skip3x_desc, blocks3 * Skip3XGeom::BLOCK_PASSES * Skip3XGeom::DESC * 4, who));
        TRY(B.device_bytes(&net->skip3x_rows, blocks3 * Skip3XGeom::BLOCK_PASSES * Skip3Reach::WORDS * 4, who));
        TRY(B.device_bytes(&net->fc1_list, Skip3Geom::PAIRS * N * sizeof(int), who));
    }
    TRY(B.device_bytes(&net->crops, N * net->W * net->H * net->CH, who));
    TRY(B.pinned(&net->h_probs, N * net->classes, who));
    if (rc != TREXHIP_OK) return rc;
    TH_CHECK_HIP(hipMemsetAsync(net->d_ovfc, 0, N, ctx->stream));
    net->max_crops = n;
    return TREXHIP_OK;
}
#undef TRY

std::vector<LdsAttr>& lds_attrs() { static std::vector<LdsAttr> v; return v; }

static const ByChannels K_CONV1{Kern(k_conv1<1>, 256, (84 * 84 + 25 * 16) * 4, false), Kern(k_conv1<3>, 256, 3 * (84 * 84 + 25 * 16) * 4, false)};
// ... 79 lines not shown
                     p.head_plans ? net.ovf(OVF_RANGE) : nullptr, net.d_ovfc, p.head_plans ? net.ovf(OVF_PLAN) : nullptr);
}

static void launch_rerun(const Pass& f) {
    const uint32_t* g = f.net.ovf(OVF_PLAN);
    if (!f.p.head_plans) K_GUARD_PLAN(f.s, 1, f.net.ovf(OVF_RANGE), f.net.d_ovfc, f.n, f.net.ovf(OVF_PLAN));
    if (f.p.rerun_conv1) launch_conv1(f, Conv1::MFMA, g);
    for (const int layer : {2, 3}) {
        if (f.p.chain == Chain::ANY_SIZE) any_conv(f.s, f.net, f.p, layer, TREXHIP_CNN_BF16X6, g);
        else launch_exact(f, layer, TREXHIP_CNN_BF16X6, g);
    }
    launch_tail(f, g);
}

static int make_empty_v3(trexhip_ctx* ctx, Net* net) {
    const char* who = "trexhip_load_weights";
    uint8_t* zero = nullptr;
    int rc = net->weights.device_bytes(&net->v3e, (size_t)SkipGeom::V3_ROWS * V3_ROWB, who);
    if (rc == TREXHIP_OK) rc = net->weights.device_bytes(&net->act3e, (size_t)Skip3Geom::PAIRS * 10 * 128 * 4, who);
    if (rc == TREXHIP_OK) rc = net->weights.device_bytes(&net->fc1e, (size_t)FC1_KSPLIT * 128 * 4, who);
    if (rc == TREXHIP_OK) rc = net->weights.device_bytes(&net->d_skip, SK_WORDS * 4, who);
    if (rc == TREXHIP_OK) rc = net->weights.device_bytes(&net->act2e, (size_t)SkipGeom::V3_ROWS * 20 * 64 * 4, who);
    if (rc == TREXHIP_OK) rc = net->weights.device_bytes(&net->bgtab, (size_t)W2xGeom::NBG * W2xGeom::BG_UNITS * sizeof(uint4), who);
    if (rc == TREXHIP_OK) rc = net->weights.device_bytes(&zero, SkipGeom::CROP_ROWS * 80, who);
    if (rc != TREXHIP_OK) return rc;
    const CnnPlan p = cnn_plan(80, 80, 1, TREXHIP_CNN_FP16X3, true, GEOM_ROLE_SPLIT | GEOM_NO_SKIP, 1, ctx->n_cus);
    TH_CHECK_HIP(hipFuncSetAttribute(reinterpret_cast<const void*>(K_CONV12_RS.fn), hipFuncAttributeMaxDynamicSharedMemorySize, K_CONV12_RS.lds));
    TH_CHECK_HIP(hipMemsetAsync(net->d_skip, 0, SK_WORDS * 4, ctx->stream));
    TH_CHECK_HIP(hipMemsetAsync(zero, 0, SkipGeom::CROP_ROWS * 80, ctx->stream));
    K_CONV12_RS(ctx->stream, p.conv2.grid, zero, net->w1h, net->b1, net->inv1h, net->w2w, net->b2, net->v3e, net->inv2w, net->d_skip + SK_EMPTY_RANGE, 1,
                net->d_skip + SK_EMPTY_CTR, p.pk2, nullptr, nullptr, nullptr, net->act2e, nullptr, nullptr);
    TH_CHECK_HIP(hipGetLastError());
    TH_CHECK_HIP(hipFuncSetAttribute(reinterpret_cast<const void*>(K_CONV12_RSX.fn), hipFuncAttributeMaxDynamicSharedMemorySize, K_CONV12_RSX.lds));
    K_CONV12_RSX(ctx->stream, 1, zero, net->w1h, net->b1, net->inv1h, net->w2w, net->b2, net->v3e, net->inv2w, net->d_skip + SK_EMPTY_RANGE, 1,
                 net->d_skip + SKX_CTR, 1, nullptr, nullptr, nullptr, net->act2e, nullptr, net->bgtab);
    TH_CHECK_HIP(hipGetLastError());
    TH_CHECK_HIP(hipFuncSetAttribute(reinterpret_cast<const void*>(K_CONV3_WPAIR.fn), hipFuncAttributeMaxDynamicSharedMemorySize, K_CONV3_WPAIR.lds));
    K_CONV3_WPAIR(ctx->stream, p.conv3.grid, net->v3e, net->w3w, net->b3, net->act3e, net->inv3w, 1, net->d_skip + SK3_EMPTY_CTR, p.n_big3, nullptr, nullptr, nullptr);
    TH_CHECK_HIP(hipGetLastError());
    const CnnPlan pf = cnn_plan(80, 80, 1, TREXHIP_CNN_FP16X3, true, 0, 1, ctx->n_cus);
    K_FC1_SPLIT4(ctx->stream, dim3(1, pf.planes), net->act3e, net->wf1h, net->bf1, net->fc1e, 1, pf.K, net->invf1h, net->d_skip + SK3_FC1E_RANGE, nullptr,
                 nullptr, nullptr, 0);
    TH_CHECK_HIP(hipGetLastError());
    uint32_t range = 0;
    TH_CHECK_HIP(hipMemcpyAsync(&range, net->d_skip + SK3_FC1E_RANGE, 4, hipMemcpyDeviceToHost, ctx->stream));
    TH_CHECK_HIP(hipStreamSynchronize(ctx->stream));
    if (range) {
        const uint32_t one = 1;
        TH_CHECK_HIP(hipMemcpy(net->d_skip + SK_EMPTY_RANGE, &one, 4, hipMemcpyHostToDevice));
    }
    return TREXHIP_OK;
}

static void launch_skip_prep(const Pass& f, const bool direct, const bool x3 ) {
    const Net& net = f.net;
    const CnnPlan& p = f.p;
    const int n = f.n, lb = ceil_div(p.conv2.items, SKIP_LB);
    int2* cols = p.skipx ? net.skipx_cols : nullptr;
    K_CROP_BANDS(f.s, ceil_div(n, 4), f.crops, n, net.skip_bands, cols || x3 ? net.skipx_cols : nullptr);
    K_PASS_COUNT(f.s, lb, net.skip_bands, cols, n, net.d_skip, net.skip_counts, (int)p.bgrows);
    K_PASS_LIST(f.s, lb, net.skip_bands, cols, n, net.d_skip, net.skip_counts, net.skip_list, net.skipx_list, net.skipx_rows, (int)p.bgrows);
    if (p.skip3) {
        const int2* cols3 = x3 ? net.skipx_cols : nullptr;
        K_PAIR_COUNT(f.s, p.skip3_grid, net.skip_bands, cols3, n, net.d_skip, net.skip3_counts, net.skip3_tcounts);
        K_PAIR_LIST(f.s, p.skip3_grid, net.skip_bands, cols3, n, net.d_skip, net.skip3_counts, net.skip3_tcounts, net.skip3_desc, net.skip3x_desc);
        if (p.fc1_listed) K_FC1_LIST(f.s, Skip3Geom::PAIRS, net.skip_bands, n, net.d_skip, net.fc1_list, net.max_crops);
    }
    K_V3_FILL(f.s, ceil_div(n * SkipGeom::V3_ROWS, SKIP_FILL_TB), net.skip_bands, cols, n, net.d_skip, reinterpret_cast<const uint4*>(net.v3e),
              reinterpret_cast<uint4*>(net.v3), (int)direct);
}

static int net_forward_launch(trexhip_ctx* ctx, const uint8_t* d_crops, int n, float* d_probs, float* d_logits) {
    const Net& net = *static_cast<Net*>(ctx->net);
    if (!ctx->attr_cnn) {
        for (const LdsAttr& a : lds_attrs()) TH_CHECK_HIP(hipFuncSetAttribute(a.fn, hipFuncAttributeMaxDynamicSharedMemorySize, a.bytes));
        ctx->attr_cnn = true;
    }
    const CnnPlan p = cnn_plan(net.W, net.H, net.CH, ctx->cnn_mode, (reinterpret_cast<uintptr_t>(d_crops) & 15) == 0, ctx->tune_conv_geom, n, ctx->n_cus);
    const Pass f{net, p, ctx->stream, ctx->cnn_mode, d_crops, n, d_probs, d_logits};
    hipStream_t s = f.s;
    const long long alloc_rows = (long long)net.max_crops * SkipGeom::V3_ROWS;
    const bool direct = p.v3_direct && skip3_direct_fits(alloc_rows);
    const bool x3 = p.skip3x && direct && skip3x_direct_fits(alloc_rows);
    stage_begin(ctx, TREXHIP_STAGE_CNN_ALL);
    launch_conv1(f, p.conv1, nullptr);
    if (p.chain == Chain::ANY_SIZE) {
        any_conv(s, net, p, 2, f.mode, nullptr);
        any_conv(s, net, p, 3, f.mode, nullptr);
    } else {
        const bool pre = p.chain == Chain::ROLE_SPLIT || p.chain == Chain::FUSED_2WG || p.chain == Chain::TWO_KERNEL;
        stage_begin(ctx, TREXHIP_STAGE_CONV2);
        switch (p.chain) {
        case Chain::ROLE_SPLIT:
            if (p.skip) launch_skip_prep(f, direct, x3);
            if (p.skipx)
                K_CONV12_RSX(s, p.conv2.grid, d_crops, net.w1h, net.b1, net.inv1h, net.w2w, net.b2, net.v3, net.inv2w, net.ovf(OVF_RANGE), n, net.d_skip + SKX_CTR,
                             p.pk2, net.d_ovfc, net.skipx_list, net.d_skip + SKX_PASSES, net.act2e, net.skipx_rows, net.bgtab);
            K_CONV12_RS(s, p.conv2.grid, d_crops, net.w1h, net.b1, net.inv1h, net.w2w, net.b2, net.v3, net.inv2w, net.ovf(OVF_RANGE), n, net.ovf(OVF_PASS2),
                        p.pk2, net.d_ovfc, p.skip ? net.skip_list : nullptr, p.skip ? net.d_skip + (p.skipx ? SKX_FULL : SK_LEN) : nullptr, nullptr, nullptr, nullptr);
            break;
        case Chain::FUSED_2WG:
            K_CONV12_WPRE(s, p.conv2.grid, d_crops, net.w1h, net.b1, net.inv1h, net.w2w, net.b2, net.v3, net.inv2w, net.ovf(OVF_RANGE), n, net.ovf(OVF_PASS2),
                          p.pk2, net.d_ovfc);
            break;
        case Chain::TWO_KERNEL:
            K_CONV2_WPRE2(s, p.conv2.grid, net.v2, net.w2w, net.b2, net.v3, net.inv2w, net.ovf(OVF_RANGE), n, net.ovf(OVF_PASS2));
            break;
        case Chain::FP32_ACT:
            K_CONV2_STREAM(s, p.conv2.grid, net.act1, net.w2h, net.b2, net.act2, net.inv2h, net.ovf(OVF_RANGE), p.conv2.items);
            break;
        default: launch_exact(f, 2, f.mode, nullptr);
        }
        stage_end(ctx, TREXHIP_STAGE_CONV2);
        stage_begin(ctx, TREXHIP_STAGE_CONV3);
        if (pre) {
            if (p.skip3) {
                K_ACT3_FILL(s, p.act3_fill.grid, net.skip_bands, x3 ? net.skipx_cols : nullptr, n, net.d_skip, reinterpret_cast<const uint4*>(net.act3e),
                            reinterpret_cast<uint4*>(net.act3), net.skip3_desc, net.skip3_rows, net.skip3x_desc, net.skip3x_rows, alloc_rows, (int)direct, (int)!p.fc1_listed);
                if (x3)
                    K_CONV3_WPAIR_LISTX(s, p.conv3.grid, net.v3, net.w3w, net.b3, net.act3, net.inv3w, n, net.d_skip + SK3X_CTR, 0, net.skip3x_desc, net.skip3x_rows, net.d_skip);
                K_CONV3_WPAIR_LIST(s, p.conv3.grid, net.v3, net.w3w, net.b3, net.act3, net.inv3w, n, net.ovf(OVF_PASS3), 0, net.skip3_desc, net.skip3_rows, net.d_skip);
            }
            K_CONV3_WPAIR(s, p.conv3.grid, net.v3, net.w3w, net.b3, net.act3, net.inv3w, n, net.ovf(OVF_PASS3), p.n_big3, nullptr, nullptr, p.skip3 ? net.d_skip : nullptr);
        }
        else if (p.chain == Chain::FP32_ACT)
            K_CONV3_WINO(s, p.conv3.grid, net.act2, net.w3w, net.b3, net.act3, net.inv3w, net.ovf(OVF_RANGE), n, net.ovf(OVF_PASS3));
        else launch_exact(f, 3, f.mode, nullptr);
        stage_end(ctx, TREXHIP_STAGE_CONV3);
    }
    launch_tail(f, nullptr);
    if (p.rerun) launch_rerun(f);
    stage_end(ctx, TREXHIP_STAGE_CNN_ALL);
    TH_CHECK_HIP(hipGetLastError());
    return TREXHIP_OK;
}

static constexpr int GRAPH_MAX_CROPS = 6400;
static constexpr size_t GRAPH_CACHE = 8;
static constexpr int GRAPH_MIN_SEEN = 3;

static int net_forward_inner(trexhip_ctx* ctx, const uint8_t* d_crops, int n, float* d_probs, float* d_logits);
int net_forward(trexhip_ctx* ctx, const uint8_t* d_crops, int n, float* d_probs, float* d_logits) {
    Net* net = static_cast<Net*>(ctx->net);
    if (ctx->cnn_mode == TREXHIP_CNN_FP16X3) {
        if (!net->ovf_clean) TH_CHECK_HIP(hipMemsetAsync(net->d_ovf, 0, OVF_PLAN * 4, ctx->stream));
        net->ovf_clean = false;
    }
    const int rc = net_forward_inner(ctx, d_crops, n, d_probs, d_logits);
    if (rc == TREXHIP_OK) { net->last_mode = ctx->cnn_mode; if (ctx->cnn_mode == TREXHIP_CNN_FP16X3) net->ovf_clean = true; }
    net->last_fc1_n = rc == TREXHIP_OK && !net->arch && cnn_plan(net->W, net->H, net->CH, ctx->cnn_mode, (reinterpret_cast<uintptr_t>(d_crops) & 15) == 0,
                                                                 ctx->tune_conv_geom, n, ctx->n_cus).fc1_listed ? n : 0;
    return rc;
}

static bool capture_chain(trexhip_ctx* ctx, Net* net, Net::GraphEntry* cand, const uint8_t* d_crops, int n, float* d_probs, float* d_logits) {
    hipGraph_t graph = nullptr;
    hipGraphExec_t exec = nullptr;
    hipEvent_t ev = nullptr;
    bool ok = hipStreamBeginCapture(ctx->stream, hipStreamCaptureModeThreadLocal) == hipSuccess;
    if (ok) {
        const int rc = net_forward_launch(ctx, d_crops, n, d_probs, d_logits);
        const hipError_t e_end = hipStreamEndCapture(ctx->stream, &graph);
        ok = rc == TREXHIP_OK && e_end == hipSuccess && graph && hipGraphInstantiate(&exec, graph, nullptr, nullptr, 0) == hipSuccess &&
             hipEventCreateWithFlags(&ev, hipEventDisableTiming) == hipSuccess;
    }
    if (graph) (void)hipGraphDestroy(graph);
    if (!ok) {
        (void)hipGetLastError();
        if (exec) (void)hipGraphExecDestroy(exec);
        net->graphs_ok = false;
        return false;
    }
    cand->exec = exec; cand->last = ev;
    return true;
}

static int net_forward_inner(trexhip_ctx* ctx, const uint8_t* d_crops, int n, float* d_probs, float* d_logits) {
    Net* net = static_cast<Net*>(ctx->net);
    if (net->arch) return arch_forward(ctx, *net, d_crops, n, d_probs, d_logits);
    static const bool enabled = [] { const char* e = std::getenv("TREXHIP_GRAPHS"); return !(e && std::atoi(e) == 0); }();
    if (!enabled || !net->graphs_ok || n > GRAPH_MAX_CROPS || ctx->profiling || !ctx->attr_cnn) return net_forward_launch(ctx, d_crops, n, d_probs, d_logits);
    hipStream_t s = ctx->stream;
    const Net::GraphKey key{d_crops, n, d_probs, d_logits, ctx->cnn_mode, ctx->tune_conv_geom, s};
    ++net->tick;
    Net::GraphEntry* cand = nullptr;
    for (auto& g : net->graphs)
        if (g.key == key) { cand = &g; break; }
    if (!cand) {
        if (net->graphs.size() >= GRAPH_CACHE) {
            size_t lru = 0;
            for (size_t i = 1; i < net->graphs.size(); ++i) if (net->graphs[i].used < net->graphs[lru].used) lru = i;
            destroy_graph_entry(net->graphs[lru]);
            net->graphs.erase(net->graphs.begin() + (long)lru);
        }
        net->graphs.push_back({key, nullptr, net->tick, nullptr, 1});
        return net_forward_launch(ctx, d_crops, n, d_probs, d_logits);
    }
    cand->used = net->tick;
    if (!cand->exec && (++cand->seen < GRAPH_MIN_SEEN || !capture_chain(ctx, net, cand, d_crops, n, d_probs, d_logits)))
        return net_forward_launch(ctx, d_crops, n, d_probs, d_logits);
    TH_CHECK_HIP(hipGraphLaunch(cand->exec, s));
    TH_CHECK_HIP(hipEventRecord(cand->last, s));
    return TREXHIP_OK;
}

static int identify_prepare(trexhip_ctx* ctx, const bool args, const char* who, const int32_t n, Net** net) {
    *net = nullptr;
    if (!args) { set_error(std::string(who) + ": null argument"); return TREXHIP_E_INVALID; }
    Net* loaded = static_cast<Net*>(ctx->net);
    if (!loaded) { set_error("trexhip_identify: weights not loaded (VINetwork status().weights.loaded())"); return TREXHIP_E_INVALID; }
    if (n < 0) { set_error("trexhip_identify: n < 0"); return TREXHIP_E_INVALID; }
    if (n == 0) return TREXHIP_OK;
    TH_CHECK_HIP(hipSetDevice(ctx->p.device));
    const int rc = loaded->arch ? arch_ensure_act(ctx, loaded, n) : ensure_act(ctx, loaded, n);
    if (rc == TREXHIP_OK) *net = loaded;
    return rc;
}

}

using namespace trexhip;

extern "C" {

int trexhip_load_weights(trexhip_ctx* ctx, const void* blob, size_t bytes) {
    if (!ctx || !blob) { set_error("trexhip_load_weights: null argument"); return TREXHIP_E_INVALID; }
    return net_load(ctx, blob, bytes);
}

int trexhip_identify_device(trexhip_ctx* ctx, const uint8_t* d_crops, int32_t n, float* d_probs, float* d_logits) {
    Net* net;
    const int rc = identify_prepare(ctx, ctx && d_crops && d_probs, "trexhip_identify_device", n, &net);
    if (rc || !net) return rc;
    return net_forward(ctx, d_crops, n, d_probs, d_logits);
}

int trexhip_identify(trexhip_ctx* ctx, const uint8_t* crops, int32_t n, float* probs) {
    Net* net;
    int rc = identify_prepare(ctx, ctx && crops && probs, "trexhip_identify", n, &net);
    if (rc || !net) return rc;
    const size_t cb = (size_t)net->W * net->H * net->CH;
    TH_CHECK_HIP(hipMemcpyAsync(net->crops, crops, cb * n, hipMemcpyHostToDevice, ctx->stream));
    rc = net_forward(ctx, net->crops, n, net->probs, nullptr);
    if (rc) return rc;
    TH_CHECK_HIP(hipMemcpyAsync(probs, net->probs, (size_t)n * net->classes * 4, hipMemcpyDeviceToHost, ctx->stream));
    TH_CHECK_HIP(hipStreamSynchronize(ctx->stream));
    return TREXHIP_OK;
}

int trexhip_identify_guard_stats(trexhip_ctx* ctx, uint32_t* rerun_crops, uint32_t* whole_batch) {
    if (!ctx || !ctx->net) { set_error("trexhip_identify_guard_stats: no context / weights not loaded"); return TREXHIP_E_INVALID; }
    Net* net = static_cast<Net*>(ctx->net);
    uint32_t plan[2] = {0, 0};
    TH_CHECK_HIP(hipStreamSynchronize(ctx->stream));
    if (net->last_mode == TREXHIP_CNN_FP16X3 && net->arch) {
        uint32_t st[2] = {0, 0};
        TH_CHECK_HIP(hipMemcpy(st, net->ovf(ARCH_STAT_RERUN), 8, hipMemcpyDeviceToHost));
        if (rerun_crops) *rerun_crops = st[0];
        if (whole_batch) *whole_batch = st[1] ? 1u : 0u;
        return TREXHIP_OK;
    }
    if (net->last_mode == TREXHIP_CNN_FP16X3) TH_CHECK_HIP(hipMemcpy(plan, net->ovf(OVF_PLAN), 8, hipMemcpyDeviceToHost));
    if (rerun_crops) *rerun_crops = plan[1] == 1u ? plan[0] : 0u;
    if (whole_batch) *whole_batch = plan[1] == 2u ? 1u : 0u;
    return TREXHIP_OK;
}

static int read_skip_words(trexhip_ctx* ctx, const char* who, uint32_t (&w)[SK_WORDS]) {
    if (!ctx || !ctx->net) { set_error(std::string(who) + ": no context / weights not loaded"); return TREXHIP_E_INVALID; }
    const Net* net = static_cast<Net*>(ctx->net);
    std::fill(w, w + SK_WORDS, 0u);
    TH_CHECK_HIP(hipStreamSynchronize(ctx->stream));
    if (net->d_skip) TH_CHECK_HIP(hipMemcpy(w, net->d_skip, sizeof w, hipMemcpyDeviceToHost));
    return TREXHIP_OK;
}

int trexhip_identify_skip_stats(trexhip_ctx* ctx, uint32_t* passes, uint32_t* listed, uint64_t* bytes_filled) {
    uint32_t w[SK_WORDS];
    if (const int rc = read_skip_words(ctx, "trexhip_identify_skip_stats", w)) return rc;
    if (passes) *passes = w[SK_NPASS];
    if (listed) *listed = w[SK_LEN];
    if (bytes_filled) *bytes_filled = (uint64_t)w[SK_FILLED] * V3_ROWB;
    return TREXHIP_OK;
}

int trexhip_identify_skipx_stats(trexhip_ctx* ctx, uint32_t* crops_windowed, uint32_t* windowed_passes, uint32_t* full_passes) {
    uint32_t w[SK_WORDS];
// ... 12 lines not shown
    return TREXHIP_OK;
}

int trexhip_identify_skip3x_stats(trexhip_ctx* ctx, uint32_t* crops_windowed, uint32_t* windowed_passes, uint32_t* full_passes) {
    uint32_t w[SK_WORDS];
    if (const int rc = read_skip_words(ctx, "trexhip_identify_skip3x_stats", w)) return rc;
    if (crops_windowed) *crops_windowed = w[SK3_USE] ? w[SK3X_CROPS] : 0u;
    if (windowed_passes) *windowed_passes = w[SK3_USE] ? w[SK3X_PASSES] : 0u;
    if (full_passes) *full_passes = w[SK3_USE] ? w[SK3_PASSES] : 0u;
    return TREXHIP_OK;
}

int trexhip_identify_skip3_stats(trexhip_ctx* ctx, uint32_t* pairs, uint32_t* listed, uint32_t* passes, uint64_t* bytes_filled) {
    uint32_t w[SK_WORDS];
    if (const int rc = read_skip_words(ctx, "trexhip_identify_skip3_stats", w)) return rc;
    if (pairs) *pairs = w[SK3_PAIRS];
    if (listed) *listed = w[SK3_LISTED];
    uint32_t by_rows = w[SK3_PASSES];
    if (passes && w[SK3_USE] && w[SK3X_PASSES]) {
        const Net* net = static_cast<Net*>(ctx->net);
        const int n = (int)(w[SK3_PAIRS] / Skip3Geom::PAIRS);
        std::vector<int2> bands((size_t)n);
        TH_CHECK_HIP(hipMemcpy(bands.data(), net->skip_bands, (size_t)n * sizeof(int2), hipMemcpyDeviceToHost));
        int count = 0;
        for (int c0 = 0; c0 < n; c0 += Skip3Geom::BLOCK) {
            Skip3Pass p{};
            for (int c = c0; c < n && c < c0 + Skip3Geom::BLOCK; ++c) {
                const SkipPairs r = skip3_pairs({bands[(size_t)c].x, bands[(size_t)c].y});
                if (r.lo <= r.hi) skip3_add_run(p, count, c * Skip3Geom::PAIRS + r.lo, r.hi - r.lo + 1, [](int, const Skip3Pass&) {});
            }
            skip3_flush(p, count, [](int, const Skip3Pass&) {});
        }
        by_rows = (uint32_t)count;
    }
    if (passes) *passes = w[SK3_USE] ? by_rows : 0u;
    if (bytes_filled) *bytes_filled = (uint64_t)w[SK3_FILLED] * (10 * 128 * 4);
    return TREXHIP_OK;
}

int trexhip_identify_fc1_stats(trexhip_ctx* ctx, uint32_t* rows, uint32_t* listed) {
    uint32_t w[SK_WORDS];
    if (const int rc = read_skip_words(ctx, "trexhip_identify_fc1_stats", w)) return rc;
    const Net* net = static_cast<Net*>(ctx->net);
    uint32_t sum = 0;
    for (int q = 0; q < Skip3Geom::PAIRS && net->last_fc1_n; ++q) sum += w[SK3_FC1_LEN + q];
    if (rows) *rows = (uint32_t)net->last_fc1_n * Skip3Geom::PAIRS;
    if (listed) *listed = sum;
    return TREXHIP_OK;
}

int trexhip_set_identity_precision(trexhip_ctx* ctx, int32_t mode) {
    if (!ctx || mode < 0 || mode > 3) { set_error("trexhip_set_identity_precision: mode must be one of TREXHIP_CNN_*"); return TREXHIP_E_INVALID; }
    ctx->cnn_mode = mode;
    return TREXHIP_OK;
}

int trexhip_num_classes(trexhip_ctx* ctx) {
    if (!ctx || !ctx->net) return 0;
    return static_cast<Net*>(ctx->net)->classes;
}

int trexhip_network_version(trexhip_ctx* ctx) {
    if (!ctx || !ctx->net) return 0;
    const Net* net = static_cast<const Net*>(ctx->net);
    return net->arch ? net->arch->plan.spec->id : TREXHIP_NET_V118_3;
}

size_t trexhip_network_blob_bytes(int32_t version, int32_t classes, int32_t channels, int32_t width, int32_t height) {
    return arch_blob_bytes(version, classes, channels, width, height);
}

int trexhip_identify_chunk_crops(trexhip_ctx* ctx, int32_t* crops) {
    if (!ctx || !crops) { set_error("trexhip_identify_chunk_crops: null argument"); return TREXHIP_E_INVALID; }
    const Net* net = static_cast<const Net*>(ctx->net);
    *crops = net && net->arch ? net->arch->plan.chunk : 0;
    return TREXHIP_OK;
}

int trexhip_network_channels(trexhip_ctx* ctx) {
    if (!ctx || !ctx->net) return 0;
    return static_cast<Net*>(ctx->net)->CH;
}

int trexhip_network_image_size(trexhip_ctx* ctx, int32_t* width, int32_t* height) {
    if (!ctx) { set_error("trexhip_network_image_size: null context"); return TREXHIP_E_INVALID; }
    const Net* net = static_cast<const Net*>(ctx->net);
    if (width) *width = net ? net->W : 0;
    if (height) *height = net ? net->H : 0;
    return TREXHIP_OK;
}

}

namespace trexhip {
void net_free(trexhip_ctx* ctx) {
    free_net(static_cast<Net*>(ctx->net)); ctx->net = nullptr;
    free_net(static_cast<Net*>(ctx->cat)); ctx->cat = nullptr;
}
}
```

### trex_amd/csrc/internal.h

```cpp
#pragma once
#include <hip/hip_runtime.h>
#include <stdint.h>
#include <functional>
#include <string>
#include <vector>
#include "../../include/trexhip.h"

#define TREXHIP_ROW_SLOT 16
#define TREXHIP_CTR_STRIDE 32

namespace trexhip {

void set_error(const std::string& msg);

#define TH_CHECK_HIP(expr)                                                                    \
    do {                                                                                      \
        hipError_t _e = (expr);                                                               \
        if (_e != hipSuccess) {                                                               \
            ::trexhip::set_error(std::string(#expr) + ": " + hipGetErrorString(_e));          \
            return TREXHIP_E_DEVICE;                                                          \
        }                                                                                     \
    } while (0)

struct SegCfg {
    int W, H, B;
    int ctr_frames;
    int R;
    int T;
    int tmin;
    int tmax;
    int enable_diff, absdiff, invert, zero_bg;
    int slack;
    int n_ranges;
    float sqcm;
    double ranges[16];
    uint32_t pool_blobs, pool_runs, pool_pixels;
    uint32_t cap_blobs, cap_pixels;
};

struct EvPair { hipEvent_t a = nullptr, b = nullptr; };
struct Stage {
    std::vector<EvPair> pending, freelist;
    EvPair cur;
    double total_ms = 0.0;
    int64_t launches = 0;
};

}

namespace trexhip {
struct Mem {
    std::vector<void*> dev, host;
    int alloc(void** p, size_t bytes, bool pinned, const char* who);
    template <typename T> int device_bytes(T** p, size_t bytes, const char* who) { return alloc(reinterpret_cast<void**>(p), bytes, false, who); }
    template <typename T> int device(T** p, size_t count, const char* who) { return device_bytes(p, (count ? count : 1) * sizeof(T), who); }
    template <typename T> int pinned(T** p, size_t count, const char* who) { return alloc(reinterpret_cast<void**>(p), (count ? count : 1) * sizeof(T), true, who); }
    void release(void* d);
    void free_all();
};
// ... 17 lines not shown
    trexhip_blob* h_blobs = nullptr;
    trexhip_run* h_runs = nullptr;
    uint8_t* h_pixels = nullptr;
    int valid_n = 0;
    bool fetched = false;
};
struct LabelState {
    uint32_t* d_row_cnt = nullptr;
    uint32_t* d_row_base = nullptr;
    trexhip_run* d_raster = nullptr;
    uint32_t* d_parent = nullptr;
    uint32_t* d_root_ord = nullptr;
    uint32_t* d_cnt_runs = nullptr;
    uint32_t* d_cnt_px = nullptr;
    uint32_t* d_cur_run = nullptr;
    uint32_t* d_pix_begin = nullptr;
    int32_t* d_blob_map = nullptr;
};
struct Pass2 {
    bool allocated = false;
    Mem mem;
    BlobTables tables;
    LabelState label;
    uint32_t *d_sub_cnt = nullptr, *d_sub_base = nullptr, *d_run_parent = nullptr;
};
}

namespace trexhip {
enum { UP_SLOTS = 3 };
static constexpr size_t UP_CHUNK_BYTES = (size_t)32 << 20;
struct Uploader {
    hipStream_t copy_stream = nullptr;
    hipEvent_t ev_start[UP_SLOTS] = {}, ev_done[UP_SLOTS] = {};
    bool busy[UP_SLOTS] = {};
    int frames_in[UP_SLOTS] = {};
    uint8_t* ring = nullptr;
    size_t slot_bytes = 0;
    void* pool = nullptr;
    double copy_ms = 0.0, dma_ms = 0.0;
    int64_t copy_n = 0, dma_n = 0;
};
}

struct trexhip_ctx {
    trexhip_params p;
    trexhip::SegCfg cfg;
    hipStream_t own_stream = nullptr;
    hipStream_t stream = nullptr;
    bool has_bg = false;
    int batch_invert = 0, batch_zero_bg = 0;

    trexhip::Mem mem;
    trexhip::BlobTables tables;
    trexhip::LabelState label;
    uint8_t* d_bg = nullptr;
    uint8_t* d_staging = nullptr;
    const uint8_t* d_frames = nullptr;
    uint32_t* d_ctr = nullptr;
    uint32_t* d_band_fail = nullptr;
    uint32_t* d_row_off = nullptr;
    uint32_t* d_tmp_runs = nullptr;
    trexhip::Scratch warp;
    trexhip::Scratch len;
    trexhip::Scratch aug_idx;
    trexhip::Scratch val;
    trexhip::Scratch avg;
    trexhip::Scratch vf;
    trexhip::Scratch autos;
    trexhip::Scratch pre;
    trexhip::Scratch load;
    trexhip::Scratch bg_color;
    uint32_t* d_bits[2] = {nullptr, nullptr};
    uint8_t* d_color = nullptr;

    void* net = nullptr;
    void* cat = nullptr;
    trexhip::Scratch vote;
    trexhip::Scratch med;
    trexhip::Pass2 pass2;
    int cnn_mode = TREXHIP_CNN_FP16X3;

    bool profiling = false;
    int tune_conv_geom = 0;
    bool attr_cnn = false, attr_ccl = false, attr_split = false, attr_prefilter = false;
    bool ctr_dirty = false;
    int attr_posture_bytes = 0;
    int pix_ch = 1;
    const uint8_t* d_color_src = nullptr;
    int color_ch = 0;
    int bg_color_ch = 0;
    int n_cus = 256;
    int tune_ccl_bands = -1;
    uint32_t* h_ccl_hint = nullptr;
    uint32_t ccl_calls = 0;
    trexhip::Stage stages[TREXHIP_STAGE_COUNT];
    trexhip::Uploader up;
};

namespace trexhip {
int launch_segment(trexhip_ctx* ctx, const uint8_t* d_frames, int n);
void stage_begin(trexhip_ctx* ctx, int stage);
void stage_end(trexhip_ctx* ctx, int stage);
void net_free(trexhip_ctx* ctx);
int launch_pending(trexhip_ctx* ctx);
int launch_morphology(trexhip_ctx* ctx, const uint8_t* d_frames, int n, const uint32_t** result);
int launch_rethreshold(trexhip_ctx* ctx, int thr, int method, const double* ranges, int n_ranges, const int32_t* d_blob_thr);
int rethreshold_prepare(trexhip_ctx* ctx, const char* who, int32_t method, const double* size_ranges, int32_t n_ranges);
int launch_prefilter(trexhip_ctx* ctx, const trexhip_prefilter_params* pp, const trexhip_prefilter_tables* tb, uint8_t* d_decision, int32_t* d_order,
                     int32_t* d_counts, int32_t* d_presumed_nr);
int launch_to_gray(trexhip_ctx* ctx, const uint8_t* d_color, uint8_t* d_gray, size_t npix, int channels, int color_channel);
int ensure_staging(trexhip_ctx* ctx, const char* who);
void upload_free(trexhip_ctx* ctx);
int upload_frames(trexhip_ctx* ctx, const uint8_t* const* frames, int n, size_t rows, size_t row_bytes, size_t stride, uint8_t* d_dst,
                  const std::function<int(int, int)>& after_chunk, int reduce_channels = 0, int color_channel = -1);
}
```

### trex_amd/csrc/posture.hip

```cpp
#include "internal.h"
#include <algorithm>

namespace trexhip {

static constexpr int P_NP = 4096;
static constexpr int P_NR = 2048;
static constexpr int P_ROWS = 1022;
__host__ __device__ constexpr int posture_wave_lds(int np, int nr, int nrows) { return np * 8 * 2 + np * 4 * 2 + nr * 4 + (nrows + 2) * 4; }
__host__ __device__ constexpr size_t posture_walk_lds(int max_points) { return (size_t)max_points * 8 + ((((size_t)max_points / 2 + 1) * 4 + 7) & ~(size_t)7); }
__host__ __device__ inline int walk_max_offset(float offset, int n) { float mo = offset * (float)n; if (mo < 3.0f) mo = 3.0f; return (int)mo; }

struct PostureCfg {
    float outline_resample; int smooth_samples, smooth_step, approximate;
    float curvature_range_ratio, midline_walk_offset; int max_points;
    int nr_cap, rows_cap;
    int walk_group;
};

struct WaveBlob {
    float2 *bufA, *bufB, *pts, *other;
    float *s_curv, *s_t;
    uint32_t* s_runs; int* s_row;
    int np;
    __device__ __forceinline__ WaveBlob(uint8_t* plds, int wave, const PostureCfg& P) : np(P.max_points) {
// ... 711 lines not shown
    void widen() { P.nr_cap = P_NR; P.rows_cap = P_ROWS; size(); }
    void size() {
        const int wave_lds = posture_wave_lds(P.max_points, P.nr_cap, P.rows_cap);
        wpb = 4;
        while (wpb > 1 && wpb * wave_lds > 150 * 1024) wpb >>= 1;
        lds_bytes = wpb * wave_lds;
    }
};

static int launch_posture(trexhip_ctx* ctx, const PosturePlan& plan, const BlobTables& t, int n, const PostureOut& out, const int32_t* sel, const trexhip_blob* origin) {
    if (plan.lds_bytes > ctx->attr_posture_bytes) {
        TH_CHECK_HIP(hipFuncSetAttribute(reinterpret_cast<const void*>(&k_posture), hipFuncAttributeMaxDynamicSharedMemorySize, plan.lds_bytes));
        ctx->attr_posture_bytes = plan.lds_bytes;
    }
    stage_begin(ctx, TREXHIP_STAGE_POSTURE);
    hipLaunchKernelGGL(k_posture, dim3((n + plan.wpb - 1) / plan.wpb), dim3(plan.wpb * 64), plan.lds_bytes, ctx->stream, plan.P, t.d_info, t.d_blob_frame, t.d_blobs, t.d_runs,
                       n, ctx->tables.valid_n, out.outline, out.segments, out.info, sel, origin);
    if (plan.P.walk_group & 8) launch_posture_walk<8>(ctx->stream, plan.P, n, out);
    if (plan.P.walk_group & 16) launch_posture_walk<16>(ctx->stream, plan.P, n, out);
    stage_end(ctx, TREXHIP_STAGE_POSTURE);
    return TREXHIP_OK;
}

static int validate_posture_params(const trexhip_ctx* ctx, const trexhip_posture_params* pp) {
    if (pp->max_points < 8 || pp->max_points > P_NP || (pp->max_points & 1)) { set_error("trexhip_posture_device: max_points must be even and in 8..4096"); return TREXHIP_E_INVALID; }
    if (pp->outline_smooth_samples < 0 || pp->outline_smooth_samples * (pp->outline_smooth_step > 0 ? pp->outline_smooth_step : 1) > 16 || pp->outline_smooth_step < 1) {
        set_error("trexhip_posture_device: outline_smooth_samples*outline_smooth_step must be <= 16"); return TREXHIP_E_UNSUPPORTED;
    }
    if (pp->outline_approximate > 15 || (pp->outline_approximate > 3 && pp->max_points < 128)) {
        set_error("trexhip_posture_device: outline_approximate > 15 (or > 3 with max_points < 128) is not supported"); return TREXHIP_E_UNSUPPORTED;
    }
    if (pp->posture_closing_steps != 0) { set_error("trexhip_posture_device: posture_closing_steps > 0 is not implemented (closing inside pixel::threshold_get_biggest_blob, Posture.cpp:335)"); return TREXHIP_E_UNSUPPORTED; }
    if (pp->peak_mode != 0) { set_error("trexhip_posture_device: peak_mode = broad is not implemented (needs periodic::find_peaks' peak ranges / integrals, Outline.cpp:627-661); only pointy"); return TREXHIP_E_UNSUPPORTED; }
    if (pp->posture_direction_smoothing < 0) { set_error("trexhip_posture_device: posture_direction_smoothing must not be negative"); return TREXHIP_E_INVALID; }
    if (!ctx->d_frames || ctx->tables.valid_n == 0 || !ctx->tables.fetched) { set_error("trexhip_posture_device: segment and fetch a batch first"); return TREXHIP_E_INVALID; }
    return TREXHIP_OK;
}

}

using namespace trexhip;

extern "C" int trexhip_posture_device(trexhip_ctx* ctx, int32_t table, const trexhip_posture_params* pp, int32_t n_blobs,
                                      float* d_outline, float* d_segments, trexhip_posture_info* d_info) {
    if (!ctx || !pp || !d_outline || !d_segments || !d_info) { set_error("trexhip_posture_device: null argument"); return TREXHIP_E_INVALID; }
    if (int rc = validate_posture_params(ctx, pp)) return rc;
    if (n_blobs < 0 || (uint32_t)n_blobs > ctx->cfg.pool_blobs) { set_error("trexhip_posture_device: n_blobs outside the blob pool"); return TREXHIP_E_INVALID; }
    if (n_blobs == 0) return TREXHIP_OK;
    if (table == 1) {
        if (!ctx->pass2.allocated || ctx->pass2.tables.valid_n == 0) { set_error("trexhip_posture_device: no re-thresholded batch"); return TREXHIP_E_INVALID; }
    } else if (table != 0) { set_error("trexhip_posture_device: table must be 0 (detect) or 1 (re-threshold)"); return TREXHIP_E_INVALID; }
    const BlobTables& t = table == 0 ? ctx->tables : ctx->pass2.tables;
    TH_CHECK_HIP(hipSetDevice(ctx->p.device));
    const PosturePlan plan(pp, t, n_blobs, false);
    if (int rc = launch_posture(ctx, plan, t, n_blobs, PostureOut{reinterpret_cast<float2*>(d_outline), reinterpret_cast<float4*>(d_segments), d_info}, nullptr, nullptr)) return rc;
    TH_CHECK_HIP(hipGetLastError());
    return TREXHIP_OK;
}

namespace trexhip {
struct AutoState {
    unsigned long long* best;
    float2* first;
    int32_t *thr, *sel, *first_n, *first_thr, *used, *iters;
    uint32_t* active;
    static size_t bytes(int n, int max_points) { return (size_t)n * (6 * sizeof(int32_t) + sizeof(unsigned long long) + (size_t)max_points * sizeof(float2)) + 64; }
    static AutoState carve(uint8_t* base, int n, int max_points) {
        AutoState a;
        auto take = [&](size_t each) { uint8_t* p = base; base += (size_t)n * each; return p; };
        a.best = reinterpret_cast<unsigned long long*>(take(8));
        a.first = reinterpret_cast<float2*>(take((size_t)max_points * sizeof(float2)));
        int32_t** const words[6] = {&a.thr, &a.sel, &a.first_n, &a.first_thr, &a.used, &a.iters};
        for (int32_t** w : words) *w = reinterpret_cast<int32_t*>(take(4));
        a.active = reinterpret_cast<uint32_t*>(base);
        return a;
    }
};
__global__ void k_auto_init(const int n, const int tpt, const AutoState a, trexhip_posture_info* info) {
    const int b = blockIdx.x * 256 + threadIdx.x;
    if (b >= n) return;
    a.thr[b] = tpt; a.first_n[b] = 0; a.first_thr[b] = -1; a.used[b] = -1; a.iters[b] = 0; a.best[b] = 0ull;
    trexhip_posture_info z = {}; z.status = 1; info[b] = z;
}
__global__ void k_auto_pick(const trexhip_blob* __restrict__ sub, const uint32_t* __restrict__ totals2, const uint32_t pool, const int n,
                            unsigned long long* best) {
    const uint32_t s = blockIdx.x * 256u + threadIdx.x;
    const uint32_t tot = totals2[0] < pool ? totals2[0] : pool;
    if (s >= tot) return;
    const trexhip_blob B = sub[s];
    if (B.parent >= (uint32_t)n || B.n_pixels == 0) return;
    atomicMax(best + B.parent, ((unsigned long long)B.n_pixels << 32) | (unsigned long long)(0xffffffffu - s));
}
__global__ void k_auto_sel(const int n, const int32_t* thr, const unsigned long long* best, int32_t* sel) {
    const int b = blockIdx.x * 256 + threadIdx.x;
    if (b >= n) return;
    sel[b] = (thr[b] >= 0 && best[b] != 0ull) ? (int32_t)(0xffffffffu - (uint32_t)best[b]) : -1;
}
__global__ __launch_bounds__(256) void k_auto_step(const int n, const int tpt, const int max_points, const trexhip_blob* __restrict__ detect,
                                                   const trexhip_blob* __restrict__ sub, const AutoState a, float2* outline, trexhip_posture_info* info,
                                                   const int nr_cap, const int rows_cap) {
    const int lane = threadIdx.x & 63, b = blockIdx.x * 4 + (threadIdx.x >> 6);
    if (b >= n) return;
    const int t = a.thr[b];
    if (t < 0) return;
    const int s = a.sel[b];
    if (s == -2) return;
// ... 4 lines not shown
        const int sr = (int)sub[s].n_runs, srows = sub[s].y1 - sub[s].y0 + 1;
        if ((sr > nr_cap || srows > rows_cap) && sr <= P_NR && srows <= P_ROWS) {
            if (lane == 0) atomicAdd(a.active + 1, 1u);
            return;
        }
    }
    __builtin_amdgcn_wave_barrier();
    if (lane == 0) { a.iters[b] += 1; a.best[b] = 0ull; a.sel[b] = -2; }
    if (s >= 0 && last.status == 0) { if (lane == 0) { a.used[b] = t; a.thr[b] = -1; } return; }
    float2* mine = outline + (size_t)b * max_points;
    float2* keep = a.first + (size_t)b * max_points;
    int fn = a.first_n[b];
    if (s >= 0 && fn == 0 && last.n_outline > 0) {
        for (int i = lane; i < last.n_outline; i += 64) keep[i] = mine[i];
        fn = last.n_outline;
        if (lane == 0) { a.first_n[b] = fn; a.first_thr[b] = t; }
    }
    const uint32_t initial = detect[b].n_pixels;
    const uint32_t minimum = initial / 10u > 1u ? initial / 10u : 1u;
    const int tn = t + 2;
    if (count < minimum || tn >= tpt + 100) {
        __builtin_amdgcn_wave_barrier();
        for (int i = lane; i < fn; i += 64) mine[i] = keep[i];
        if (lane == 0) {
            last.n_outline = fn; last.n_segments = 0;
            if (last.status == 0) last.status = 1;
            info[b] = last;
            a.used[b] = fn > 0 ? (a.first_thr[b] >= 0 ? a.first_thr[b] : t) : -1;
            a.thr[b] = -1;
        }
        return;
    }
    if (lane == 0) { a.thr[b] = tn; atomicAdd(a.active, 1u); }
}
}

extern "C" int trexhip_posture_auto_device(trexhip_ctx* ctx, const trexhip_posture_params* pp, int32_t method, int32_t track_posture_threshold,
                                           int32_t n_blobs, float* d_outline, float* d_segments, trexhip_posture_info* d_info,
                                           int32_t* d_threshold_used, int32_t* d_iterations) {
    if (!ctx || !pp || !d_outline || !d_segments || !d_info) { set_error("trexhip_posture_auto_device: null argument"); return TREXHIP_E_INVALID; }
    if (method < 0 || method > 2) { set_error("trexhip_posture_auto_device: method must be 0 (absolute), 1 (sign) or 2 (none)"); return TREXHIP_E_INVALID; }
    if (track_posture_threshold < 0 || track_posture_threshold > 255) { set_error("trexhip_posture_auto_device: track_posture_threshold must be 0..255"); return TREXHIP_E_INVALID; }
    if (int rc = validate_posture_params(ctx, pp)) return rc;
    if (n_blobs < 0 || (uint32_t)n_blobs > ctx->cfg.pool_blobs) { set_error("trexhip_posture_auto_device: n_blobs outside the blob pool"); return TREXHIP_E_INVALID; }
    if (n_blobs == 0) return TREXHIP_OK;
    TH_CHECK_HIP(hipSetDevice(ctx->p.device));
    const int n = n_blobs, MPt = pp->max_points;
    if (int rc = ctx->autos.reserve(ctx, AutoState::bytes(n, MPt), "trexhip_posture_auto_device")) return rc;
    const AutoState a = AutoState::carve(ctx->autos.as<uint8_t>(), n, MPt);
    const PostureOut out{reinterpret_cast<float2*>(d_outline), reinterpret_cast<float4*>(d_segments), d_info};
    hipStream_t s = ctx->stream;
    const dim3 g256((unsigned)((n + 255) / 256));
    hipLaunchKernelGGL(k_auto_init, g256, dim3(256), 0, s, n, (int)track_posture_threshold, a, d_info);
    PosturePlan plan(pp, ctx->tables, n, true);
    for (int round = 0; round < 51; ++round) {
        int rc = trexhip_rethreshold_per_blob_device(ctx, 0, a.thr, method, nullptr, 0);
        if (rc) return rc;
        const BlobTables& q = ctx->pass2.tables;
        hipLaunchKernelGGL(k_auto_pick, dim3((ctx->cfg.pool_blobs + 255u) / 256u), dim3(256), 0, s, q.d_blobs, q.d_totals, ctx->cfg.pool_blobs, n, a.best);
        hipLaunchKernelGGL(k_auto_sel, g256, dim3(256), 0, s, n, a.thr, a.best, a.sel);
        uint32_t still[2] = {0, 0};
        for (int attempt = 0; attempt < 2; ++attempt) {
            TH_CHECK_HIP(hipMemsetAsync(a.active, 0, 8, s));
            if (int rc2 = launch_posture(ctx, plan, q, n, out, a.sel, ctx->tables.d_blobs)) return rc2;
            hipLaunchKernelGGL(k_auto_step, dim3((n + 3) / 4), dim3(256), 0, s, n, (int)track_posture_threshold, MPt, ctx->tables.d_blobs, q.d_blobs, a,
                               out.outline, d_info, plan.P.nr_cap, plan.P.rows_cap);
            TH_CHECK_HIP(hipGetLastError());
            TH_CHECK_HIP(hipMemcpyAsync(still, a.active, 8, hipMemcpyDeviceToHost, s));
            TH_CHECK_HIP(hipStreamSynchronize(s));
            if (still[1] == 0) break;
            plan.widen();
        }
        if (still[0] == 0) break;
    }
    if (d_threshold_used) TH_CHECK_HIP(hipMemcpyAsync(d_threshold_used, a.used, (size_t)n * 4, hipMemcpyDeviceToDevice, s));
    if (d_iterations) TH_CHECK_HIP(hipMemcpyAsync(d_iterations, a.iters, (size_t)n * 4, hipMemcpyDeviceToDevice, s));
    return TREXHIP_OK;
}

extern "C" void trexhip_default_posture_params(trexhip_posture_params* p) {
    if (!p) return;
    p->outline_resample = 1.0f; p->outline_smooth_samples = 4; p->outline_smooth_step = 1; p->outline_approximate = 3;
    p->outline_curvature_range_ratio = 0.03f; p->midline_walk_offset = 0.025f; p->max_points = 512;
    p->posture_closing_steps = 0; p->peak_mode = 0; p->posture_direction_smoothing = 0;
}
```

### trex_amd/csrc/segment.hip

```cpp
#include "internal.h"
#include <cstddef>

namespace trexhip {

static constexpr int WAVE = 64;
static constexpr int ROW_SLOT = TREXHIP_ROW_SLOT;
static constexpr int CTR_STRIDE = TREXHIP_CTR_STRIDE;

__device__ __forceinline__ uint32_t lane_id() { return threadIdx.x & 63; }

template <int LPB> __device__ __forceinline__ uint32_t group_incl_scan(uint32_t v) {
    v += (uint32_t)__builtin_amdgcn_update_dpp(0, (int)v, 0x111, 0xf, 0xf, true);
    v += (uint32_t)__builtin_amdgcn_update_dpp(0, (int)v, 0x112, 0xf, 0xf, true);
    v += (uint32_t)__builtin_amdgcn_update_dpp(0, (int)v, 0x114, 0xf, 0xf, true);
    v += (uint32_t)__builtin_amdgcn_update_dpp(0, (int)v, 0x118, 0xf, 0xf, true);
    if constexpr (LPB >= 32) v += (uint32_t)__builtin_amdgcn_update_dpp(0, (int)v, 0x142, 0xa, 0xf, false);
    if constexpr (LPB == 64) v += (uint32_t)__builtin_amdgcn_update_dpp(0, (int)v, 0x143, 0xc, 0xf, false);
    return v;
}
__device__ __forceinline__ uint32_t row_incl_scan(uint32_t v) {
    v += (uint32_t)__builtin_amdgcn_update_dpp(0, (int)v, 0x111, 0xf, 0xf, true);
    v += (uint32_t)__builtin_amdgcn_update_dpp(0, (int)v, 0x112, 0xf, 0xf, true);
    v += (uint32_t)__builtin_amdgcn_update_dpp(0, (int)v, 0x114, 0xf, 0xf, true);
    v += (uint32_t)__builtin_amdgcn_update_dpp(0, (int)v, 0x118, 0xf, 0xf, true);
// ... 1406 lines not shown
        const uint32_t ext[8] = {x0, y0, ~x1, ~y1, pmin, ~pmax, 0xffffffffu, 0xffffffffu};
        const uint32_t te = wave_min8x32<LPB>(ext, lane);
        x0 = bcast_lane<LPB, lane_of_q(0)>(te); y0 = bcast_lane<LPB, lane_of_q(1)>(te);
        x1 = ~bcast_lane<LPB, lane_of_q(2)>(te); y1 = ~bcast_lane<LPB, lane_of_q(3)>(te);
        pmin = bcast_lane<LPB, lane_of_q(4)>(te); pmax = ~bcast_lane<LPB, lane_of_q(5)>(te);
        if (!active) continue;
        trexhip_blob* out = blobs + bi;
        if (sub < 8) {
            const uint32_t q = 4u * (sub & 1u) + 2u * ((sub >> 1) & 1u) + ((sub >> 2) & 1u);
            (&out->m10)[q] = tot;
        }
        if (sub == 0) {
            const trexhip_run first = rr[0];
            out->n_pixels = po;
            out->run_begin = B.run_begin - fi.run_begin; out->pix_begin = B.pix_begin - fi.pix_begin;
            out->x0 = (uint16_t)x0; out->y0 = (uint16_t)y0; out->x1 = (uint16_t)x1; out->y1 = (uint16_t)y1;
            out->bid = make_bid(first.x0, first.x1, first.y, B.n_runs);
            out->px_min_max = pmin | (pmax << 8);
        }
    }
}

template <bool COLOUR, int LPB>
__global__ __launch_bounds__(256) void k_gather(const SegCfg c, const int only_pending, const uint8_t* __restrict__ frames,
                                                const uint32_t* __restrict__ totals,
                                                const trexhip_frame_info* __restrict__ info,
                                                const uint32_t* __restrict__ blob_frame,
                                                trexhip_blob* __restrict__ blobs,
                                                const trexhip_run* __restrict__ runs,
                                                uint8_t* __restrict__ pixels, const uint32_t f0, const uint32_t f1,
                                                const uint8_t* __restrict__ color, const int color_ch, const int enc_) {
    constexpr uint32_t BPW = 64 / LPB;
    gather_blobs<COLOUR, LPB>(c, only_pending, frames, info, blob_frame, blobs, runs, pixels, f0, f1, color, color_ch, enc_,
                              (blockIdx.x * 4 + (threadIdx.x >> 6)) * BPW, gridDim.x * 4 * BPW, min(totals[0], c.pool_blobs), -1, 0u, 0u);
}

#define LAUNCH_GATHER(grid_, stream_, ...) do { if (ctx->p.pixel_encoding != TREXHIP_ENC_GRAY) hipLaunchKernelGGL((k_gather<true, 64>), grid_, dim3(256), 0, stream_, __VA_ARGS__); \
                                                 else hipLaunchKernelGGL((k_gather<false, 32>), grid_, dim3(256), 0, stream_, __VA_ARGS__); } while (0)
template <bool ALIGNED>
static void launch_rows(int nch, dim3 grid, hipStream_t s, const uint8_t* frames, const uint8_t* bg,
                        const SegCfg& c, uint32_t* ctr, uint32_t* row_cnt, uint32_t* row_off, uint32_t* tmp, const uint32_t* bits) {
    switch (nch) {
        case 1: hipLaunchKernelGGL((k_rows<1, ALIGNED>), grid, dim3(256), 0, s, frames, bg, c, ctr, row_cnt, row_off, tmp, bits); break;
        case 2: hipLaunchKernelGGL((k_rows<2, ALIGNED>), grid, dim3(256), 0, s, frames, bg, c, ctr, row_cnt, row_off, tmp, bits); break;
        case 3: hipLaunchKernelGGL((k_rows<3, ALIGNED>), grid, dim3(256), 0, s, frames, bg, c, ctr, row_cnt, row_off, tmp, bits); break;
        case 4: hipLaunchKernelGGL((k_rows<4, ALIGNED>), grid, dim3(256), 0, s, frames, bg, c, ctr, row_cnt, row_off, tmp, bits); break;
        case 5: case 6:
                hipLaunchKernelGGL((k_rows<6, ALIGNED>), grid, dim3(256), 0, s, frames, bg, c, ctr, row_cnt, row_off, tmp, bits); break;
        default: hipLaunchKernelGGL((k_rows<8, ALIGNED>), grid, dim3(256), 0, s, frames, bg, c, ctr, row_cnt, row_off, tmp, bits); break;
    }
}

int launch_segment(trexhip_ctx* ctx, const uint8_t* d_frames, int n) {
    SegCfg c = ctx->cfg;
    c.B = n;
    ctx->batch_invert = c.invert; ctx->batch_zero_bg = c.zero_bg;
    hipStream_t s = ctx->stream;
    const int H = c.H, W = c.W;
    const int nch = (W + 1023) / 1024;
    if (nch > 8) { set_error("frame width > 8192 is not supported yet"); return TREXHIP_E_UNSUPPORTED; }
    stage_begin(ctx, TREXHIP_STAGE_SEGMENT_ALL);
    if (ctx->ctr_dirty) TH_CHECK_HIP(hipMemsetAsync(ctx->d_ctr, 0, sizeof(uint32_t) * ((size_t)ctx->p.max_batch * CTR_STRIDE + 4), s));
    ctx->ctr_dirty = true;
    const bool aligned = (W % 16 == 0) && ((reinterpret_cast<uintptr_t>(d_frames) & 15) == 0) &&
                         ((reinterpret_cast<uintptr_t>(ctx->d_bg) & 15) == 0);
    const uint32_t* bits = nullptr;
    if (ctx->p.use_closing || ctx->p.dilation_size != 0) {
        int rcm = launch_morphology(ctx, d_frames, n, &bits);
        if (rcm) return rcm;
    }
    using LdsM = CclLds<CCL_M_NMAX, CCL_M_SA>;
    using LdsS = CclLds<CCL_S_NMAX, CCL_S_SA>;
    if (!ctx->attr_ccl) {
        TH_CHECK_HIP(hipFuncSetAttribute(reinterpret_cast<const void*>(&k_ccl_lds<1024, CCL_NMAX, CCL_SORT>), hipFuncAttributeMaxDynamicSharedMemorySize, CCL_LDS_BYTES));
        TH_CHECK_HIP(hipFuncSetAttribute(reinterpret_cast<const void*>(&k_ccl_lds<512, CCL_M_NMAX, CCL_M_SA>), hipFuncAttributeMaxDynamicSharedMemorySize, LdsM::BYTES));
        TH_CHECK_HIP(hipFuncSetAttribute(reinterpret_cast<const void*>(&k_ccl_lds<256, CCL_S_NMAX, CCL_S_SA>), hipFuncAttributeMaxDynamicSharedMemorySize, LdsS::BYTES));
        TH_CHECK_HIP(hipFuncSetAttribute(reinterpret_cast<const void*>(&k_ccl_band), hipFuncAttributeMaxDynamicSharedMemorySize, CCLB_LDS_BYTES));
        ctx->attr_ccl = true;
    }
    if ((++ctx->ccl_calls & 63) == 0) { ctx->h_ccl_hint[0] = 0u; ctx->h_ccl_hint[1] = 0u; }
    int inst = 3;
    if (n >= 2 * ctx->n_cus) {
        const uint32_t over_s = __atomic_load_n(&ctx->h_ccl_hint[0], __ATOMIC_RELAXED), over_m = __atomic_load_n(&ctx->h_ccl_hint[1], __ATOMIC_RELAXED);
        inst = over_m ? 3 : (over_s ? 2 : 1);
        if (c.R <= CCL_S_NMAX) inst = 1; else if (c.R <= CCL_M_NMAX && inst > 2) inst = 2;
    }
    uint32_t* totals = ctx->tables.d_totals;
    const bool fuse_gather = ctx->p.pixel_encoding == TREXHIP_ENC_GRAY && 4 * n >= 3 * ctx->n_cus;

    stage_begin(ctx, TREXHIP_STAGE_ROWS);
    const unsigned want = (unsigned)(((size_t)H * n + 3) / 4);
    const int nch32 = (W + 2047) / 2048;
    const bool wide = aligned && !bits && W % 32 == 0 && nch32 <= 4 && W >= 1024;
    unsigned cap = 8192u;
    if (wide) { cap = want / 4; if (cap < 2048u) cap = 2048u; }
    const dim3 grid_rows(want < cap ? want : cap);
    if (wide) {
        int mode = 0;
        if (c.enable_diff && !c.invert && c.tmax >= 255 && c.tmin >= 1) mode = (c.absdiff ? 1 : 2) | (c.zero_bg ? 4 : 0);
        int K = 0;
        for (int k = 8; k >= 2; --k) if (n % k == 0) { K = k; break; }
        const dim3 grid_b(K ? (unsigned)(((size_t)H * (n / K) + 3) / 4) : 1u);
#define TH_ROWS32(NCH_, MODE_) do { if (K && NCH_ == 1) hipLaunchKernelGGL((k_rows32b<1, MODE_>), grid_b, dim3(256), 0, s, d_frames, ctx->d_bg, c, K, ctx->d_ctr, ctx->label.d_row_cnt, ctx->d_row_off, ctx->d_tmp_runs); \
                                    else if (K && NCH_ == 2) hipLaunchKernelGGL((k_rows32b<2, MODE_>), grid_b, dim3(256), 0, s, d_frames, ctx->d_bg, c, K, ctx->d_ctr, ctx->label.d_row_cnt, ctx->d_row_off, ctx->d_tmp_runs); \
                                    else hipLaunchKernelGGL((k_rows32<NCH_, MODE_>), grid_rows, dim3(256), 0, s, d_frames, ctx->d_bg, c, ctx->d_ctr, ctx->label.d_row_cnt, ctx->d_row_off, ctx->d_tmp_runs); } while (0)
#define TH_ROWS32_M(NCH_) do { switch (mode) { case 1: TH_ROWS32(NCH_, 1); break; case 2: TH_ROWS32(NCH_, 2); break; case 5: TH_ROWS32(NCH_, 5); break; \
// ... 219 lines not shown
```

### trex_amd/csrc/split.hip

```cpp
#include "internal.h"

namespace trexhip {

static constexpr int S_PX = 16384;
static constexpr int S_RUNS = 1024;
static constexpr int S_SUB = 2048;
static constexpr int S_PX_SMALL = 2048, S_RUNS_SMALL = 256, S_SUB_SMALL = 1024;
static constexpr int S_PX_HUGE = 61440, S_RUNS_HUGE = 2048, S_SUB_HUGE = 4096;
constexpr int split_lds_bytes(int px, int runs, int sub) { return runs * 4 + sub * 12 + 1024 + runs * 2 + (runs + 2) * 2 + sub * 2 + 256 + px; }

enum { A_KEEP = 0, A_KEEP_ABORT = 1, A_REMOVE = 2, A_ABORT = 3, A_TOO_FEW = 4, A_SKIP = 5, A_NO_CHANCE = 6 };

struct SplitCfg {
    int W, H, B, invert, slack, method, initial_threshold, algorithm, n_ranges;
    float sqcm, max_shrink, global_shrink;
    double ranges[16];
    double max_start, max_end;
};

__device__ __forceinline__ uint32_t wmax_u32(uint32_t v) {
#pragma unroll
    for (int d = 32; d >= 1; d >>= 1) v = max(v, (uint32_t)__shfl_xor((int)v, d));
    return v;
}
// ... 226 lines not shown
            const int start = begin, end = max_pixel;
            const int fs_end = start + (int)((double)(end - start) * 0.3);
            for (int ti = 0; ti < 3 && best == -1 && !capacity; ++ti) {
                bool done = false;
                for (int offset = 0; offset < 2 && !done; ++offset) {
                    if (best != -1) break;
                    for (int t = start + ti * 2 + offset; t < fs_end && !capacity; t += 6) {
                        if (best != -1 && t >= best) break;
                        const int a = perform(t);
                        if (a == A_ABORT || a == A_KEEP_ABORT) { if (a == A_KEEP_ABORT) done = true; break; }
                    }
                }
                if (done || best != -1) continue;
                for (int t = fs_end + ti; t < end && !capacity; t += 3) {
                    if (best != -1 && t >= best) break;
                    const int a = perform(t);
                    if (a == A_ABORT || a == A_KEEP_ABORT) break;
                }
            }
        }
    }
    if (!capacity && best != -1 && action != A_KEEP_ABORT) evaluate(best_eff, first_size, max_size, n_kept, bound);
    if (lane == 0) {
        if (capacity) { res.status = 2; best = -1; best_eff = -1; }
        res.threshold = best; res.effective_threshold = best_eff;
        res.n_result = best != -1 ? n_kept : 0;
        res.min_size_bound = best != -1 ? bound : 0.0;
        res.n_evaluated = n_eval; res.min_pixel = min_pixel; res.max_pixel = max_pixel; res.first_size = first_size;
        out_info[bi] = res;
        out_thr[bi] = best_eff;
    }
}

int launch_split_search(trexhip_ctx* ctx, const trexhip_split_params* sp, int method, const int32_t* d_presumed, int n_blobs, int32_t* d_thr,
                        trexhip_split_info* d_info) {
    SplitCfg C = {};
    C.W = ctx->cfg.W; C.H = ctx->cfg.H; C.B = ctx->tables.valid_n; C.invert = ctx->batch_invert; C.slack = ctx->cfg.slack; C.method = method;
    C.initial_threshold = (sp->calculate_posture ? max(sp->track_threshold, sp->track_posture_threshold) : sp->track_threshold) + 1;
    C.algorithm = sp->algorithm; C.n_ranges = sp->n_ranges;
    C.sqcm = ctx->cfg.sqcm; C.max_shrink = sp->blob_split_max_shrink; C.global_shrink = sp->blob_split_global_shrink_limit;
    C.max_start = -1; C.max_end = -1;
    for (int i = 0; i < sp->n_ranges; ++i) {
        C.ranges[2 * i] = sp->size_ranges[2 * i]; C.ranges[2 * i + 1] = sp->size_ranges[2 * i + 1];
        if (C.max_start == -1 || C.ranges[2 * i] < C.max_start) C.max_start = C.ranges[2 * i];
        if (C.max_end == -1 || C.ranges[2 * i + 1] > C.max_end) C.max_end = C.ranges[2 * i + 1];
    }
    hipLaunchKernelGGL((k_split_search<S_PX_SMALL, S_RUNS_SMALL, S_SUB_SMALL, 0, 0>), dim3((unsigned)n_blobs), dim3(64),
                       split_lds_bytes(S_PX_SMALL, S_RUNS_SMALL, S_SUB_SMALL), ctx->stream, C, ctx->d_frames,
                       ctx->d_bg, ctx->tables.d_info, ctx->tables.d_blob_frame, ctx->tables.d_blobs, ctx->tables.d_runs, d_presumed, n_blobs, d_thr, d_info);
    hipLaunchKernelGGL((k_split_search<S_PX, S_RUNS, S_SUB, S_PX_SMALL, S_RUNS_SMALL>), dim3((unsigned)n_blobs), dim3(64),
                       split_lds_bytes(S_PX, S_RUNS, S_SUB), ctx->stream, C, ctx->d_frames,
                       ctx->d_bg, ctx->tables.d_info, ctx->tables.d_blob_frame, ctx->tables.d_blobs, ctx->tables.d_runs, d_presumed, n_blobs, d_thr, d_info);
    bool huge = false;
    for (int i = 0; i < n_blobs && !huge; ++i) huge = ctx->tables.h_blobs[i].n_pixels > (uint32_t)S_PX || ctx->tables.h_blobs[i].n_runs > (uint32_t)S_RUNS;
    if (huge) {
        const int bytes = split_lds_bytes(S_PX_HUGE, S_RUNS_HUGE, S_SUB_HUGE);
        if (!ctx->attr_split) {
            TH_CHECK_HIP(hipFuncSetAttribute(reinterpret_cast<const void*>(&k_split_search<S_PX_HUGE, S_RUNS_HUGE, S_SUB_HUGE, S_PX, S_RUNS>),
                                             hipFuncAttributeMaxDynamicSharedMemorySize, bytes));
            ctx->attr_split = true;
        }
        hipLaunchKernelGGL((k_split_search<S_PX_HUGE, S_RUNS_HUGE, S_SUB_HUGE, S_PX, S_RUNS>), dim3((unsigned)n_blobs), dim3(64), bytes, ctx->stream, C,
                           ctx->d_frames, ctx->d_bg, ctx->tables.d_info, ctx->tables.d_blob_frame, ctx->tables.d_blobs, ctx->tables.d_runs, d_presumed, n_blobs, d_thr, d_info);
    }
    TH_CHECK_HIP(hipGetLastError());
    return TREXHIP_OK;
}

}

using namespace trexhip;

extern "C" void trexhip_default_split_params(trexhip_split_params* p) {
    if (!p) return;
    *p = trexhip_split_params{};
    p->track_threshold = 15; p->track_posture_threshold = 15; p->calculate_posture = 1; p->algorithm = 1;
    p->blob_split_max_shrink = 0.2f; p->blob_split_global_shrink_limit = 0.2f;
}

extern "C" int trexhip_split_search_device(trexhip_ctx* ctx, const trexhip_split_params* sp, int32_t method, const int32_t* d_presumed_nr,
                                           int32_t n_blobs, int32_t* d_thresholds, trexhip_split_info* d_info) {
    if (!ctx || !sp || !d_presumed_nr || !d_thresholds || !d_info) { set_error("trexhip_split_search_device: null argument"); return TREXHIP_E_INVALID; }
    if (method < 0 || method > 2) { set_error("trexhip_split_search_device: method must be 0 (absolute), 1 (signed) or 2 (none)"); return TREXHIP_E_INVALID; }
    if (sp->algorithm == 3 || sp->algorithm == 4) { set_error("trexhip_split_search_device: blob_split_algorithm = fill / fill_approximate (cv::watershed, SplitBlob.cpp:419-485) is not implemented by this backend"); return TREXHIP_E_UNSUPPORTED; }
    if (sp->algorithm < 0 || sp->algorithm > 2) { set_error("trexhip_split_search_device: algorithm must be 0 (none), 1 (threshold) or 2 (threshold_approximate)"); return TREXHIP_E_INVALID; }
    if (sp->n_ranges < 0 || sp->n_ranges > 8) { set_error("trexhip_split_search_device: at most 8 size ranges"); return TREXHIP_E_INVALID; }
    if (!ctx->d_frames || ctx->tables.valid_n == 0 || !ctx->tables.fetched) { set_error("trexhip_split_search_device: segment and fetch a batch first"); return TREXHIP_E_INVALID; }
    if (n_blobs < 0 || (uint32_t)n_blobs > ctx->cfg.pool_blobs) { set_error("trexhip_split_search_device: n_blobs outside the blob pool"); return TREXHIP_E_INVALID; }
    if (n_blobs == 0) return TREXHIP_OK;
    TH_CHECK_HIP(hipSetDevice(ctx->p.device));
    return launch_split_search(ctx, sp, method, d_presumed_nr, n_blobs, d_thresholds, d_info);
}
```

### trex_amd/csrc/unpack.hip

```cpp
#include "internal.h"
#include "pv_read.h"

namespace trexhip {

struct LoadBlob { uint32_t off, n_lines, n_pixels, start_y, run_begin, pix_begin; };
struct LoadFrame { uint32_t n_blobs, n_lines, n_pixels, flags; };

__device__ __forceinline__ uint32_t lw_sum32(uint32_t v) {
#pragma unroll
    for (int d = 32; d >= 1; d >>= 1) v += (uint32_t)__shfl_xor((int)v, d);
    return v;
}
__device__ __forceinline__ uint32_t lw_min32(uint32_t v) {
#pragma unroll
    for (int d = 32; d >= 1; d >>= 1) v = min(v, (uint32_t)__shfl_xor((int)v, d));
    return v;
}
__device__ __forceinline__ uint32_t lw_max32(uint32_t v) {
#pragma unroll
    for (int d = 32; d >= 1; d >>= 1) v = max(v, (uint32_t)__shfl_xor((int)v, d));
    return v;
}
__device__ __forceinline__ uint64_t lw_sum64(uint64_t v) {
#pragma unroll
// ... 232 lines not shown
                                                      uint32_t* __restrict__ tmp_x, uint32_t* __restrict__ tmp_yk) {
    const uint32_t f = blockIdx.y, lane = threadIdx.x & 63u;
    const trexhip_frame_info fi = info[f];
    if (fi.flags) return;
    const uint32_t* rb = row_base + (size_t)f * (H + 1);
    for (uint32_t k = blockIdx.x * 4u + (threadIdx.x >> 6); k < fi.n_blobs; k += gridDim.x * 4u) {
        const uint32_t run_begin = blobs[fi.blob_begin + k].run_begin, n_runs = blobs[fi.blob_begin + k].n_runs;
        for (uint32_t j = lane; j < n_runs; j += 64) {
            const trexhip_run q = runs[fi.run_begin + run_begin + j];
            if (q.y >= H) continue;
            const uint32_t pos = rb[q.y] + atomicAdd(row_cur + (size_t)f * H + q.y, 1u);
            if (pos >= fi.n_runs) continue;
            tmp_x[(size_t)f * R + pos] = (uint32_t)q.x0 | ((uint32_t)q.x1 << 16);
            tmp_yk[(size_t)f * R + pos] = (uint32_t)q.y | (k << 16);
        }
    }
}

__global__ __launch_bounds__(256) void k_load_rank(const uint32_t H, const uint32_t R, const trexhip_frame_info* __restrict__ info,
                                                   const uint32_t* __restrict__ row_base, const uint32_t* __restrict__ tmp_x,
                                                   const uint32_t* __restrict__ tmp_yk, trexhip_run* __restrict__ raster, uint32_t* __restrict__ label) {
    const uint32_t f = blockIdx.y, p = blockIdx.x * 256u + threadIdx.x;
    const trexhip_frame_info fi = info[f];
    if (fi.flags || p >= fi.n_runs) return;
    const size_t fo = (size_t)f * R;
    const uint32_t a = tmp_x[fo + p], b = tmp_yk[fo + p];
    const uint32_t y = b & 0xffffu, k = b >> 16;
    const uint32_t* rb = row_base + (size_t)f * (H + 1);
    const uint32_t s0 = rb[y], s1 = min(rb[y + 1], fi.n_runs);
    const uint32_t key = ((a & 0xffffu) << 16) | k;
    uint32_t rank = 0;
    for (uint32_t j = s0; j < s1; ++j) {
        const uint32_t kj = ((tmp_x[fo + j] & 0xffffu) << 16) | (tmp_yk[fo + j] >> 16);
        rank += (kj < key || (kj == key && j < p)) ? 1u : 0u;
    }
    if (s0 + rank >= fi.n_runs) return;
    trexhip_run q; q.x0 = (uint16_t)(a & 0xffffu); q.x1 = (uint16_t)(a >> 16); q.y = (uint16_t)y; q.pad = 0;
    raster[fo + s0 + rank] = q;
    label[fo + s0 + rank] = k;
}

}

using namespace trexhip;

extern "C" int trexhip_load_frames_v6_device(trexhip_ctx* ctx, const uint8_t* d_bodies, const uint64_t* d_offsets, int32_t n_frames,
                                             uint64_t* d_timestamps) {
    if (!ctx || !d_bodies || !d_offsets) { set_error("trexhip_load_frames_v6_device: null argument"); return TREXHIP_E_INVALID; }
    if (n_frames < 1 || n_frames > ctx->p.max_batch) { set_error("trexhip_load_frames_v6_device: n_frames outside 1..max_batch"); return TREXHIP_E_INVALID; }
    if (ctx->p.pixel_encoding != TREXHIP_ENC_GRAY) { set_error("trexhip_load_frames_v6_device: the V_6 layout holds one byte per pixel (gray); colour encodings came with V_12"); return TREXHIP_E_UNSUPPORTED; }
    if (ctx->p.width > 32768) { set_error("trexhip_load_frames_v6_device: LegacyShortHorizontalLine holds x1 < 32768 (pv.h:36)"); return TREXHIP_E_UNSUPPORTED; }
    if (ctx->p.max_blobs > 65535) { set_error("trexhip_load_frames_v6_device: a frame holds at most 65535 objects (u16 n, pv.cpp:686)"); return TREXHIP_E_UNSUPPORTED; }
    TH_CHECK_HIP(hipSetDevice(ctx->p.device));
    const size_t B = (size_t)ctx->p.max_batch, W = (size_t)ctx->p.width, H = (size_t)ctx->p.height, NB = (size_t)ctx->p.max_blobs;
    if (int rc = ensure_staging(ctx, "trexhip_load_frames_v6_device")) return rc;
    if (int rc = ctx->load.reserve(ctx, B * NB * sizeof(LoadBlob) + B * sizeof(LoadFrame), "trexhip_load_frames_v6_device")) return rc;
    LoadBlob* index = ctx->load.as<LoadBlob>();
    LoadFrame* meta = reinterpret_cast<LoadFrame*>(index + B * NB);
    const int n = n_frames;
    const uint32_t w = (uint32_t)W, h = (uint32_t)H, R = (uint32_t)ctx->p.max_runs;
    hipStream_t s = ctx->stream;
    const unsigned long long* offs = reinterpret_cast<const unsigned long long*>(d_offsets);
    uint32_t* totals = ctx->tables.d_totals;
    TH_CHECK_HIP(hipMemsetAsync(ctx->label.d_row_cnt, 0, sizeof(uint32_t) * (size_t)n * H, s));
    hipLaunchKernelGGL(k_load_index, dim3(n), dim3(64), 0, s, d_bodies, offs, w, h, (uint32_t)NB, R, (uint32_t)ctx->p.max_pixels, index, meta,
                       reinterpret_cast<unsigned long long*>(d_timestamps));
    hipLaunchKernelGGL(k_load_scan, dim3(1), dim3(256), 0, s, meta, n, ctx->tables.d_info, totals);
    const unsigned gx_blobs = (unsigned)((NB + 3) / 4 < 64 ? (NB + 3) / 4 : 64);
    hipLaunchKernelGGL(k_load_decode, dim3(gx_blobs, n), dim3(256), 0, s, d_bodies, offs, w, h, (uint32_t)NB, R, index, ctx->tables.d_info, ctx->tables.d_blobs,
                       ctx->tables.d_blob_frame, ctx->tables.d_runs, ctx->tables.d_pixels, ctx->d_staging, ctx->label.d_row_cnt, ctx->label.d_root_ord, ctx->label.d_blob_map);
    hipLaunchKernelGGL(k_load_rows, dim3(n), dim3(256), 0, s, h, ctx->tables.d_info, ctx->label.d_row_cnt, ctx->label.d_row_base);
    hipLaunchKernelGGL(k_load_scatter, dim3(gx_blobs, n), dim3(256), 0, s, h, R, ctx->tables.d_info, ctx->tables.d_blobs, ctx->tables.d_runs, ctx->label.d_row_base, ctx->label.d_row_cnt,
                       ctx->label.d_cur_run, ctx->label.d_pix_begin);
    hipLaunchKernelGGL(k_load_rank, dim3((R + 255u) / 256u, n), dim3(256), 0, s, h, R, ctx->tables.d_info, ctx->label.d_row_base, ctx->label.d_cur_run, ctx->label.d_pix_begin,
                       ctx->label.d_raster, ctx->label.d_parent);
    TH_CHECK_HIP(hipGetLastError());
    ctx->d_frames = ctx->d_staging;
    ctx->d_color_src = nullptr; ctx->color_ch = 0;
    ctx->batch_invert = 0;
    ctx->batch_zero_bg = ctx->cfg.zero_bg;
    ctx->tables.valid_n = n;
    ctx->tables.fetched = false;
    ctx->pass2.tables.valid_n = 0;
    ctx->pass2.tables.fetched = false;
    return TREXHIP_OK;
}
```

### trex_amd/pipeline.py

```python
import torch

from . import capi, dist as tdist


class Lane:

    def __init__(self, pl):
        self.pl = pl
        o = pl.opt
        p = capi.default_params(pl.W, pl.H, device=pl.local, max_batch=pl.B, max_blobs=pl.max_blobs, max_pixels=1 << 18, max_runs=32768,
                                pixel_encoding=capi.ENC_RGB8 if pl.rgb else capi.ENC_GRAY)
        self.seg = capi.Segmenter(p)
        self.seg.set_background(pl.bg)
        dev = pl.dev
        if pl.with_cnn:
            self.seg.load_weights(pl.weight_blob)
            self.seg.set_identity_precision({"fp32": 0, "bf16x6": 1, "bf16x3": 2, "fp16x3": 3}[o["cnn_mode"]])
        self.crops = torch.empty((pl.pool, 80, 80, 3) if pl.rgb else (pl.pool, 80, 80), dtype=torch.uint8, device=dev)
        self.probs = torch.empty((pl.pool, pl.classes), dtype=torch.float32, device=dev)
        self.table = torch.zeros((pl.rows, pl.rowlen), dtype=torch.int32, device=dev)
        self.table_host = torch.empty((pl.world * pl.rows, pl.rowlen), dtype=torch.int32).pin_memory() if pl.rank == 0 else None
        self.comm = None
        self.table_all = None
        if pl.use_dist:
            if pl.gather == "library":
                if pl.shared_comm is None:
                    pl.shared_comm = capi.Comm(self.seg, pl.rank, pl.world, pl.next_comm_id())
                self.comm = pl.shared_comm
            self.table_all = torch.zeros((pl.world * pl.rows, pl.rowlen), dtype=torch.int32, device=dev) if pl.rank == 0 else None
            if pl.rank == 0:
                self.table = self.table_all[:pl.rows]
        if pl.with_posture:
            MP = pl.MP
            self.p_outline = torch.empty((pl.pool, MP, 2), dtype=torch.float32, device=dev)
            self.p_segs = torch.empty((pl.pool, MP // 2 + 1, 4), dtype=torch.float32, device=dev)
            self.p_info = torch.empty((pl.pool, 8), dtype=torch.int32, device=dev)
            self.p_mid = torch.empty((pl.pool, 25, 4), dtype=torch.float32, device=dev)
            self.p_minfo = torch.empty((pl.pool, 8), dtype=torch.int32, device=dev)
        self.stream = torch.cuda.Stream(device=dev)
        self.copy_stream = torch.cuda.Stream(device=dev) if (pl.rank == 0 and pl.use_dist) else None
        self.gathered = torch.cuda.Event() if self.copy_stream is not None else None
        self.seg.set_stream(self.stream.cuda_stream)
        self.hi = torch.cuda.Stream(device=dev, priority=-1) if o["detect_priority"] else None
        self.n = 0
        self.done = torch.cuda.Event()
        self.after = None
        self.res = None

    def detect(self, frames_ptr):
        pl = self.pl
        if self.hi is not None:
            self.seg.set_stream(self.hi.cuda_stream)
        if pl.host_frames is not None:
            if pl.bgra_in:
                self.seg.segment_color_host(pl.host_frames)
            else:
                self.seg.segment_host(pl.host_frames)
        elif pl.bgra_in:
            self.seg.segment_color_device(frames_ptr, pl.B, 4)
        else:
            self.seg.segment_device(frames_ptr, pl.B)

    def identify(self, step_idx):
        pl, seg = self.pl, self.seg
        o = pl.opt
        res = self.res = seg.fetch_raw()
        n = self.n = int(res.total_blobs)
        assert n <= pl.rows, "identity table too small"
        if self.hi is not None:
            seg.set_stream(self.stream.cuda_stream)
        if pl.with_posture and n:
            seg.posture_device(n, self.p_outline.data_ptr(), self.p_segs.data_ptr(), self.p_info.data_ptr(), max_points=pl.MP)
            seg.midline_device(n, pl.MP, self.p_info.data_ptr(), self.p_segs.data_ptr(), self.p_mid.data_ptr(), self.p_minfo.data_ptr())
        if pl.with_cnn:
            if n:
                if o["normalize"] == "posture":
                    seg.crops_posture_device(self.crops.data_ptr(), n, self.p_minfo.data_ptr())
                else:
                    seg.crops_device(self.crops.data_ptr(), n, normalization=1 if o["normalize"] == "moments" else 0)
                if self.after is not None and n > 1024:
                    self.stream.wait_event(self.after.done)
                seg.identify_device(self.crops.data_ptr(), n, self.probs.data_ptr())
            self.done.record(self.stream)
            frame_base, _ = tdist.step_frames(step_idx, pl.rank, pl.world, pl.B)
            if pl.with_posture:
                seg.export_id_table_ex(self.probs.data_ptr(), n, pl.classes, frame_base, self.table.data_ptr(), pl.rows,
                                       self.p_mid.data_ptr() if n else 0, self.p_minfo.data_ptr() if n else 0, 25)
            else:
                seg.export_id_table(self.probs.data_ptr(), n, pl.classes, frame_base, self.table.data_ptr(), pl.rows)
            if pl.use_dist and self.comm is not None:
                self.comm.gather_device(self.table.data_ptr(), self.table.numel() * 4, self.table_all.data_ptr() if pl.rank == 0 else 0, seg=seg)
            elif pl.use_dist:
                import torch.distributed as dist
                with torch.cuda.stream(self.stream):
                    dist.gather(self.table, list(self.table_all.view(pl.world, pl.rows, pl.rowlen).unbind(0)) if pl.rank == 0 else None, dst=0)
            if pl.rank == 0 and self.copy_stream is not None:
                self.gathered.record(self.stream)
                self.copy_stream.wait_event(self.gathered)
                with torch.cuda.stream(self.copy_stream):
                    self.table_host.copy_(self.table_all, non_blocking=True)
            elif pl.rank == 0:
                with torch.cuda.stream(self.stream):
                    self.table_host.copy_(self.table, non_blocking=True)
        else:
            self.done.record(self.stream)

    def drain(self):
        self.stream.synchronize()
        if self.copy_stream is not None:
            self.copy_stream.synchronize()


class Pipeline:
    def __init__(self, W, H, n_ind, B, classes, bg, weight_blob=None, *, local=0, rank=0, world=1, use_dist=False, comm_ids=None,
                 with_cnn=True, with_posture=False, normalize="none", rgb=False, bgra_in=False, cnn_mode="fp16x3",
                 lanes=2, pipeline=True, detect_priority=True, host_frames=None, gather="library"):
        self.W, self.H, self.B, self.classes, self.bg = W, H, B, classes, bg
        self.local, self.rank, self.world, self.use_dist = local, rank, world, use_dist
        assert gather in ("library", "torch")
        self.gather = gather
        self._comm_ids = list(comm_ids or [])
        self.dev = torch.device("cuda", local)
        self.with_cnn, self.with_posture, self.rgb, self.bgra_in = with_cnn, with_posture or normalize == "posture", rgb, bgra_in or rgb
        self.weight_blob = weight_blob
        self.host_frames = host_frames
        self.opt = {"normalize": normalize, "cnn_mode": cnn_mode, "detect_priority": detect_priority}
        self.max_blobs = 4 * n_ind
        self.pool = B * self.max_blobs
        self.rows = B * n_ind * 5 // 4
        self.MP = 256
        self.rowlen = (tdist.HDR_EX + classes + 3 * 25) if self.with_posture else (tdist.HDR + classes)
        self.shared_comm = None
        self.lanes = [Lane(self) for _ in range(max(2, lanes))] if pipeline else [Lane(self)]
        if len(self.lanes) > 1:
            for k, ln in enumerate(self.lanes):
                ln.after = self.lanes[(k - 1) % len(self.lanes)]
                ln.done.record(ln.stream)
        torch.cuda.synchronize()

    def next_comm_id(self):
        if self.world == 1:
            return None
        assert self._comm_ids, "Pipeline(use_dist=True, world > 1) needs comm_ids = [trexhip_comm_unique_id() of rank 0]"
        return self._comm_ids.pop(0)

    def run(self, k, frames_ptr, on_batch=None):
        lanes = self.lanes
        L = len(lanes)
        D = max(1, L - 1)
        fp = frames_ptr if callable(frames_ptr) else (lambda i: frames_ptr)
        owner = {}

        def finish(ln):
            ln.drain()
            if on_batch is not None and id(ln) in owner:
                on_batch(owner.pop(id(ln)), ln)

        for i in range(min(D, k)):
            lanes[i % L].detect(fp(i))
        for i in range(k):
# ... 26 lines not shown
```

Before: 48570.

## Make blob-table fetch asynchronous and hoist CNN skip-list prep before lane wait

```diff
diff --git a/include/trexhip.h b/include/trexhip.h
--- a/include/trexhip.h
+++ b/include/trexhip.h
@@ -6,7 +6,7 @@
 extern "C" {
 #endif
 
-#define TREXHIP_ABI_VERSION 25
+#define TREXHIP_ABI_VERSION 26
 
 enum {
     TREXHIP_OK = 0,
@@ -134,6 +134,8 @@
 int trexhip_copy_to_host(trexhip_ctx* ctx, void* host_dst, const void* device_src, size_t bytes);
 int trexhip_copy_to_device(trexhip_ctx* ctx, void* device_dst, const void* host_src, size_t bytes);
 int trexhip_fetch(trexhip_ctx* ctx, trexhip_batch_result* out);
+int trexhip_fetch_begin(trexhip_ctx* ctx, trexhip_batch_result* out);
+int trexhip_fetch_wait(trexhip_ctx* ctx);
 int trexhip_device_view_get(trexhip_ctx* ctx, trexhip_device_view* out);
 int trexhip_synchronize(trexhip_ctx* ctx);
 
@@ -258,6 +260,8 @@
 enum { TREXHIP_CNN_FP32 = 0, TREXHIP_CNN_BF16X6 = 1, TREXHIP_CNN_BF16X3 = 2, TREXHIP_CNN_FP16X3 = 3 };
 int trexhip_set_identity_precision(trexhip_ctx* ctx, int32_t mode);
 int trexhip_identify_device(trexhip_ctx* ctx, const uint8_t* d_crops, int32_t n, float* d_probs, float* d_logits);
+int trexhip_identify_prepare_device(trexhip_ctx* ctx, const uint8_t* d_crops, int32_t n);
+int trexhip_identify_prepare_stats(trexhip_ctx* ctx, uint32_t* records, uint32_t* hits);
 int trexhip_identify(trexhip_ctx* ctx, const uint8_t* crops, int32_t n, float* probs);
 int trexhip_identify_guard_stats(trexhip_ctx* ctx, uint32_t* rerun_crops, uint32_t* whole_batch);
 int trexhip_identify_skip_stats(trexhip_ctx* ctx, uint32_t* passes, uint32_t* listed, uint64_t* bytes_filled);
@@ -290,7 +294,8 @@
 
 enum { TREXHIP_STAGE_ROWS = 0, TREXHIP_STAGE_SEGMENT_ALL = 1, TREXHIP_STAGE_CONV2 = 2, TREXHIP_STAGE_CONV3 = 3,
        TREXHIP_STAGE_CNN_ALL = 4, TREXHIP_STAGE_CROPS = 5, TREXHIP_STAGE_POSTURE = 6,
-       TREXHIP_STAGE_UPLOAD_COPY = 8, TREXHIP_STAGE_UPLOAD_DMA = 9, TREXHIP_STAGE_COUNT = 10 };
+       TREXHIP_STAGE_UPLOAD_COPY = 8, TREXHIP_STAGE_UPLOAD_DMA = 9,
+       TREXHIP_STAGE_PREPARE = 10, TREXHIP_STAGE_COUNT = 11 };
 int trexhip_profile_enable(trexhip_ctx* ctx, int32_t on);
 int trexhip_profile_read(trexhip_ctx* ctx, int32_t stage, double* total_ms, int64_t* launches);
 int trexhip_profile_reset(trexhip_ctx* ctx);
diff --git a/trex_amd/capi.py b/trex_amd/capi.py
--- a/trex_amd/capi.py
+++ b/trex_amd/capi.py
@@ -25,6 +25,7 @@
 CNN_FP32, CNN_BF16X6, CNN_BF16X3, CNN_FP16X3 = 0, 1, 2, 3
 STAGE_ROWS, STAGE_SEGMENT_ALL, STAGE_CONV2, STAGE_CONV3, STAGE_CNN_ALL, STAGE_CROPS, STAGE_POSTURE = 0, 1, 2, 3, 4, 5, 6
 STAGE_UPLOAD_COPY, STAGE_UPLOAD_DMA = 8, 9
+STAGE_PREPARE = 10
 
 
 class Params(C.Structure):
@@ -189,6 +190,7 @@
     "trexhip_default_vf_params", "trexhip_visual_field_device",
     "trexhip_categorize_load_weights", "trexhip_categorize_info", "trexhip_categorize_blob_bytes", "trexhip_categorize_device", "trexhip_categorize",
     "trexhip_tracklet_labels_device", "trexhip_tracklet_medians_device",
+    "trexhip_identify_prepare_device", "trexhip_fetch_begin", "trexhip_fetch_wait", "trexhip_identify_prepare_stats",
 ]
 
 
@@ -221,6 +223,8 @@
         L.trexhip_rethreshold_per_blob_device.argtypes = [C.c_void_p, C.c_int32, C.c_void_p, C.c_int32, C.c_void_p, C.c_int32]
         L.trexhip_fetch_rethreshold.argtypes = [C.c_void_p, C.POINTER(BatchResult)]
         L.trexhip_fetch.argtypes = [C.c_void_p, C.POINTER(BatchResult)]
+        L.trexhip_fetch_begin.argtypes = [C.c_void_p, C.POINTER(BatchResult)]
+        L.trexhip_fetch_wait.argtypes = [C.c_void_p]
         L.trexhip_device_view_get.argtypes = [C.c_void_p, C.POINTER(DeviceView)]
         L.trexhip_synchronize.argtypes = [C.c_void_p]
         L.trexhip_profile_enable.argtypes = [C.c_void_p, C.c_int32]
@@ -267,6 +271,8 @@
         L.trexhip_comm_count_ranks.argtypes = [C.c_void_p, C.POINTER(C.c_int32)]
         L.trexhip_set_identity_precision.argtypes = [C.c_void_p, C.c_int32]
         L.trexhip_identify_device.argtypes = [C.c_void_p, C.c_void_p, C.c_int32, C.c_void_p, C.c_void_p]
+        L.trexhip_identify_prepare_device.argtypes = [C.c_void_p, C.c_void_p, C.c_int32]
+        L.trexhip_identify_prepare_stats.argtypes = [C.c_void_p, C.POINTER(C.c_uint32), C.POINTER(C.c_uint32)]
         L.trexhip_identify.argtypes = [C.c_void_p, C.c_void_p, C.c_int32, C.c_void_p]
         L.trexhip_identify_guard_stats.argtypes = [C.c_void_p, C.POINTER(C.c_uint32), C.POINTER(C.c_uint32)]
         L.trexhip_identify_skip_stats.argtypes = [C.c_void_p, C.POINTER(C.c_uint32), C.POINTER(C.c_uint32), C.POINTER(C.c_uint64)]
@@ -483,6 +489,18 @@
             self.last_capacity_error = lib().trexhip_last_error().decode()
         return r
 
+    def fetch_begin_raw(self):
+        r = BatchResult()
+        rc = self.last_fetch_rc = lib().trexhip_fetch_begin(self._h, C.byref(r))
+        if rc != 0 and rc != -3:
+            _check(rc)
+        if rc == -3:
+            self.last_capacity_error = lib().trexhip_last_error().decode()
+        return r
+
+    def fetch_wait(self):
+        _check(lib().trexhip_fetch_wait(self._h))
+
     def fetch(self, copy=True, rethreshold=False):
         r = BatchResult()
         rc = (lib().trexhip_fetch_rethreshold if rethreshold else lib().trexhip_fetch)(self._h, C.byref(r))
@@ -659,6 +677,14 @@
         _check(lib().trexhip_identify_device(self._h, C.c_void_p(d_crops_ptr), n, C.c_void_p(d_probs_ptr),
                                              C.c_void_p(d_logits_ptr) if d_logits_ptr else None))
 
+    def identify_prepare_device(self, d_crops_ptr, n):
+        _check(lib().trexhip_identify_prepare_device(self._h, C.c_void_p(d_crops_ptr), n))
+
+    def prepare_stats(self):
+        a, b = C.c_uint32(0), C.c_uint32(0)
+        _check(lib().trexhip_identify_prepare_stats(self._h, C.byref(a), C.byref(b)))
+        return int(a.value), int(b.value)
+
     def device_alloc(self, nbytes):
         out = C.c_void_p()
         _check(lib().trexhip_device_alloc(self._h, nbytes, C.byref(out)))
diff --git a/trex_amd/csrc/capi.hip b/trex_amd/csrc/capi.hip
--- a/trex_amd/csrc/capi.hip
+++ b/trex_amd/csrc/capi.hip
@@ -82,7 +82,13 @@
     return TREXHIP_OK;
 }
 
-static int fetch_tables(trexhip_ctx* ctx, BlobTables& t, bool copy, trexhip_batch_result* out) {
+int fetch_wait(trexhip_ctx* ctx) {
+    if (!ctx->fetch_pending) return TREXHIP_OK;
+    ctx->fetch_pending = false;
+    TH_CHECK_HIP(hipEventSynchronize(ctx->fetch_ev));
+    return TREXHIP_OK;
+}
+static int fetch_tables(trexhip_ctx* ctx, BlobTables& t, bool copy, trexhip_batch_result* out, bool begin = false) {
     std::memset(out, 0, sizeof(*out));
     out->n_frames = t.valid_n;
     out->frames = t.h_info; out->blobs = t.h_blobs; out->runs = t.h_runs; out->pixels = t.h_pixels;
@@ -94,7 +100,13 @@
         if (tb) TH_CHECK_HIP(hipMemcpyAsync(t.h_blobs, t.d_blobs, sizeof(trexhip_blob) * tb, hipMemcpyDeviceToHost, s));
         if (tr) TH_CHECK_HIP(hipMemcpyAsync(t.h_runs, t.d_runs, sizeof(trexhip_run) * tr, hipMemcpyDeviceToHost, s));
         if (tp) TH_CHECK_HIP(hipMemcpyAsync(t.h_pixels, t.d_pixels, (size_t)tp * ctx->pix_ch, hipMemcpyDeviceToHost, s));
-        TH_CHECK_HIP(hipStreamSynchronize(s));
+        if (begin) {
+            if (!ctx->fetch_ev) TH_CHECK_HIP(hipEventCreateWithFlags(&ctx->fetch_ev, hipEventDisableTiming));
+            TH_CHECK_HIP(hipEventRecord(ctx->fetch_ev, s));
+            ctx->fetch_stream = s;
+            ctx->fetch_pending = true;
+        }
+        else TH_CHECK_HIP(hipStreamSynchronize(s));
     }
     out->total_blobs = tb; out->total_runs = tr; out->total_pixels = tp;
     t.fetched = true;
@@ -229,7 +241,9 @@
 void trexhip_destroy(trexhip_ctx* ctx) {
     if (!ctx) return;
     hipSetDevice(ctx->p.device);
+    (void)fetch_wait(ctx);
     if (ctx->stream) hipStreamSynchronize(ctx->stream);
+    if (ctx->fetch_ev) hipEventDestroy(ctx->fetch_ev);
     net_free(ctx);
     ctx->pass2.mem.free_all();
     upload_free(ctx);
@@ -304,7 +318,7 @@
 
 int trexhip_set_stream(trexhip_ctx* ctx, void* hip_stream) {
     if (!ctx) { set_error("null ctx"); return TREXHIP_E_INVALID; }
-    TH_CHECK_HIP(hipStreamSynchronize(ctx->stream));
+    if (!(ctx->fetch_pending && ctx->fetch_stream == ctx->stream)) TH_CHECK_HIP(hipStreamSynchronize(ctx->stream));
     ctx->stream = hip_stream ? reinterpret_cast<hipStream_t>(hip_stream) : ctx->own_stream;
     return TREXHIP_OK;
 }
@@ -407,9 +421,10 @@
 }
 extern "C" {
 
-int trexhip_fetch(trexhip_ctx* ctx, trexhip_batch_result* out) {
-    if (!ctx || !out) { set_error("trexhip_fetch: null argument"); return TREXHIP_E_INVALID; }
-    TH_CHECK_HIP(hipSetDevice(ctx->p.device));
+static int fetch_batch(trexhip_ctx* ctx, trexhip_batch_result* out, const char* who, const bool begin) {
+    if (!ctx || !out) { set_error(std::string(who) + ": null argument"); return TREXHIP_E_INVALID; }
+    TH_CHECK_HIP(hipSetDevice(ctx->p.device));
+    if (const int rc = fetch_wait(ctx)) return rc;
     BlobTables& t = ctx->tables;
     const int n = t.valid_n;
     const bool by_kernel = n <= EXPORT_MAX_FRAMES;
@@ -424,7 +439,7 @@
             if (rc1) return rc1;
         }
     }
-    int rc = fetch_tables(ctx, t, !by_kernel, out);
+    int rc = fetch_tables(ctx, t, !by_kernel, out, begin);
     if (rc || n == 0) return rc;
     for (int i = 0; i < n; ++i)
         if (t.h_info[i].flags & TREXHIP_FRAME_MALFORMED) {
@@ -444,6 +459,13 @@
     return rc;
 }
 
+int trexhip_fetch(trexhip_ctx* ctx, trexhip_batch_result* out) { return fetch_batch(ctx, out, "trexhip_fetch", false); }
+int trexhip_fetch_begin(trexhip_ctx* ctx, trexhip_batch_result* out) { return fetch_batch(ctx, out, "trexhip_fetch_begin", true); }
+int trexhip_fetch_wait(trexhip_ctx* ctx) {
+    if (!ctx) { set_error("trexhip_fetch_wait: null ctx"); return TREXHIP_E_INVALID; }
+    return fetch_wait(ctx);
+}
+
 static int pass2_alloc(trexhip_ctx* ctx, const char* who) {
     Pass2& q = ctx->pass2;
     if (q.allocated) return TREXHIP_OK;
diff --git a/trex_amd/csrc/cnn.hip b/trex_amd/csrc/cnn.hip
--- a/trex_amd/csrc/cnn.hip
+++ b/trex_amd/csrc/cnn.hip
@@ -1188,6 +1188,7 @@
 #define TRY(x) do { if (rc == TREXHIP_OK) rc = (x); } while (0)
 static int make_empty_v3(trexhip_ctx* ctx, Net* net);
 int net_load(trexhip_ctx* ctx, const void* blob, size_t bytes) {
+    ctx->prepared.weights_loaded();
     const int arch = blob_arch_id(blob, bytes);
     if (arch >= TREXHIP_NET_V100 && arch <= TREXHIP_NET_V200) return arch_load(ctx, blob, bytes);
     WeightBlob wb;
@@ -1240,6 +1241,7 @@
 static int ensure_act(trexhip_ctx* ctx, Net* net, int n) {
     if (n <= net->max_crops) return TREXHIP_OK;
     drop_graphs(net);
+    ctx->prepared.batch_reallocated();
     net->batch.free_all();
     net->h_probs = nullptr;
     net->max_crops = 0;
@@ -1425,7 +1427,13 @@
     return TREXHIP_OK;
 }
 
-static void launch_skip_prep(const Pass& f, const bool direct, const bool x3 ) {
+struct PrepArgs { long long alloc_rows; bool direct, x3 ; };
+static PrepArgs prep_args(const Net& net, const CnnPlan& p) {
+    const long long alloc_rows = (long long)net.max_crops * SkipGeom::V3_ROWS;
+    const bool direct = p.v3_direct && skip3_direct_fits(alloc_rows);
+    return {alloc_rows, direct, p.skip3x && direct && skip3x_direct_fits(alloc_rows)};
+}
+static void launch_skip_prep(const Pass& f, const bool direct, const bool x3) {
     const Net& net = f.net;
     const CnnPlan& p = f.p;
     const int n = f.n, lb = ceil_div(p.conv2.items, SKIP_LB);
@@ -1443,18 +1451,34 @@
               reinterpret_cast<uint4*>(net.v3), (int)direct);
 }
 
-static int net_forward_launch(trexhip_ctx* ctx, const uint8_t* d_crops, int n, float* d_probs, float* d_logits) {
-    const Net& net = *static_cast<Net*>(ctx->net);
+enum : int { PREP_LISTS = 1, PREP_ACT3 = 2 };
+static bool plan_prepares(const CnnPlan& p) { return p.chain == Chain::ROLE_SPLIT && p.skip; }
+static void launch_prep(const Pass& f, const int parts) {
+    const Net& net = f.net;
+    const CnnPlan& p = f.p;
+    if (!plan_prepares(p)) return;
+    const PrepArgs a = prep_args(net, p);
+    if (parts & PREP_LISTS) launch_skip_prep(f, a.direct, a.x3);
+    if ((parts & PREP_ACT3) && p.skip3)
+        K_ACT3_FILL(f.s, p.act3_fill.grid, net.skip_bands, a.x3 ? net.skipx_cols : nullptr, f.n, net.d_skip, reinterpret_cast<const uint4*>(net.act3e),
+                    reinterpret_cast<uint4*>(net.act3), net.skip3_desc, net.skip3_rows, net.skip3x_desc, net.skip3x_rows, a.alloc_rows, (int)a.direct, (int)!p.fc1_listed);
+}
+
+static int set_cnn_attrs(trexhip_ctx* ctx) {
     if (!ctx->attr_cnn) {
         for (const LdsAttr& a : lds_attrs()) TH_CHECK_HIP(hipFuncSetAttribute(a.fn, hipFuncAttributeMaxDynamicSharedMemorySize, a.bytes));
         ctx->attr_cnn = true;
     }
+    return TREXHIP_OK;
+}
+
+static int net_forward_launch(trexhip_ctx* ctx, const uint8_t* d_crops, int n, float* d_probs, float* d_logits, const bool prepared = false) {
+    const Net& net = *static_cast<Net*>(ctx->net);
+    if (const int rc = set_cnn_attrs(ctx)) return rc;
     const CnnPlan p = cnn_plan(net.W, net.H, net.CH, ctx->cnn_mode, (reinterpret_cast<uintptr_t>(d_crops) & 15) == 0, ctx->tune_conv_geom, n, ctx->n_cus);
     const Pass f{net, p, ctx->stream, ctx->cnn_mode, d_crops, n, d_probs, d_logits};
     hipStream_t s = f.s;
-    const long long alloc_rows = (long long)net.max_crops * SkipGeom::V3_ROWS;
-    const bool direct = p.v3_direct && skip3_direct_fits(alloc_rows);
-    const bool x3 = p.skip3x && direct && skip3x_direct_fits(alloc_rows);
+    const bool x3 = prep_args(net, p).x3;
     stage_begin(ctx, TREXHIP_STAGE_CNN_ALL);
     launch_conv1(f, p.conv1, nullptr);
     if (p.chain == Chain::ANY_SIZE) {
@@ -1465,7 +1489,7 @@
         stage_begin(ctx, TREXHIP_STAGE_CONV2);
         switch (p.chain) {
         case Chain::ROLE_SPLIT:
-            if (p.skip) launch_skip_prep(f, direct, x3);
+            if (!prepared) launch_prep(f, PREP_LISTS);
             if (p.skipx)
                 K_CONV12_RSX(s, p.conv2.grid, d_crops, net.w1h, net.b1, net.inv1h, net.w2w, net.b2, net.v3, net.inv2w, net.ovf(OVF_RANGE), n, net.d_skip + SKX_CTR,
                              p.pk2, net.d_ovfc, net.skipx_list, net.d_skip + SKX_PASSES, net.act2e, net.skipx_rows, net.bgtab);
@@ -1488,8 +1512,7 @@
         stage_begin(ctx, TREXHIP_STAGE_CONV3);
         if (pre) {
             if (p.skip3) {
-                K_ACT3_FILL(s, p.act3_fill.grid, net.skip_bands, x3 ? net.skipx_cols : nullptr, n, net.d_skip, reinterpret_cast<const uint4*>(net.act3e),
-                            reinterpret_cast<uint4*>(net.act3), net.skip3_desc, net.skip3_rows, net.skip3x_desc, net.skip3x_rows, alloc_rows, (int)direct, (int)!p.fc1_listed);
+                if (!prepared) launch_prep(f, PREP_ACT3);
                 if (x3)
                     K_CONV3_WPAIR_LISTX(s, p.conv3.grid, net.v3, net.w3w, net.b3, net.act3, net.inv3w, n, net.d_skip + SK3X_CTR, 0, net.skip3x_desc, net.skip3x_rows, net.d_skip);
                 K_CONV3_WPAIR_LIST(s, p.conv3.grid, net.v3, net.w3w, net.b3, net.act3, net.inv3w, n, net.ovf(OVF_PASS3), 0, net.skip3_desc, net.skip3_rows, net.d_skip);
@@ -1512,14 +1535,20 @@
 static constexpr size_t GRAPH_CACHE = 8;
 static constexpr int GRAPH_MIN_SEEN = 3;
 
-static int net_forward_inner(trexhip_ctx* ctx, const uint8_t* d_crops, int n, float* d_probs, float* d_logits);
+static bool graph_path(const trexhip_ctx* ctx, const Net* net, const int n) {
+    static const bool enabled = [] { const char* e = std::getenv("TREXHIP_GRAPHS"); return !(e && std::atoi(e) == 0); }();
+    return enabled && net->graphs_ok && n <= GRAPH_MAX_CROPS && !ctx->profiling && ctx->attr_cnn;
+}
+
+static int net_forward_inner(trexhip_ctx* ctx, const uint8_t* d_crops, int n, float* d_probs, float* d_logits, bool prepared);
 int net_forward(trexhip_ctx* ctx, const uint8_t* d_crops, int n, float* d_probs, float* d_logits) {
     Net* net = static_cast<Net*>(ctx->net);
+    const bool prepared = ctx->prepared.consume(ctx->prepared.make(d_crops, n, ctx->cnn_mode, ctx->tune_conv_geom, ctx->stream));
     if (ctx->cnn_mode == TREXHIP_CNN_FP16X3) {
         if (!net->ovf_clean) TH_CHECK_HIP(hipMemsetAsync(net->d_ovf, 0, OVF_PLAN * 4, ctx->stream));
         net->ovf_clean = false;
     }
-    const int rc = net_forward_inner(ctx, d_crops, n, d_probs, d_logits);
+    const int rc = net_forward_inner(ctx, d_crops, n, d_probs, d_logits, prepared);
     if (rc == TREXHIP_OK) { net->last_mode = ctx->cnn_mode; if (ctx->cnn_mode == TREXHIP_CNN_FP16X3) net->ovf_clean = true; }
     net->last_fc1_n = rc == TREXHIP_OK && !net->arch && cnn_plan(net->W, net->H, net->CH, ctx->cnn_mode, (reinterpret_cast<uintptr_t>(d_crops) & 15) == 0,
                                                                  ctx->tune_conv_geom, n, ctx->n_cus).fc1_listed ? n : 0;
@@ -1548,11 +1577,10 @@
     return true;
 }
 
-static int net_forward_inner(trexhip_ctx* ctx, const uint8_t* d_crops, int n, float* d_probs, float* d_logits) {
+static int net_forward_inner(trexhip_ctx* ctx, const uint8_t* d_crops, int n, float* d_probs, float* d_logits, const bool prepared) {
     Net* net = static_cast<Net*>(ctx->net);
     if (net->arch) return arch_forward(ctx, *net, d_crops, n, d_probs, d_logits);
-    static const bool enabled = [] { const char* e = std::getenv("TREXHIP_GRAPHS"); return !(e && std::atoi(e) == 0); }();
-    if (!enabled || !net->graphs_ok || n > GRAPH_MAX_CROPS || ctx->profiling || !ctx->attr_cnn) return net_forward_launch(ctx, d_crops, n, d_probs, d_logits);
+    if (!graph_path(ctx, net, n)) return net_forward_launch(ctx, d_crops, n, d_probs, d_logits, prepared);
     hipStream_t s = ctx->stream;
     const Net::GraphKey key{d_crops, n, d_probs, d_logits, ctx->cnn_mode, ctx->tune_conv_geom, s};
     ++net->tick;
@@ -1606,6 +1634,30 @@
     const int rc = identify_prepare(ctx, ctx && d_crops && d_probs, "trexhip_identify_device", n, &net);
     if (rc || !net) return rc;
     return net_forward(ctx, d_crops, n, d_probs, d_logits);
+}
+
+int trexhip_identify_prepare_device(trexhip_ctx* ctx, const uint8_t* d_crops, int32_t n) {
+    Net* net;
+    const int rc = identify_prepare(ctx, ctx && d_crops, "trexhip_identify_prepare_device", n, &net);
+    if (rc || !net) return rc;
+    ctx->prepared.drop();
+    if (net->arch || ctx->cnn_mode != TREXHIP_CNN_FP16X3 || graph_path(ctx, net, n)) return TREXHIP_OK;
+    const CnnPlan p = cnn_plan(net->W, net->H, net->CH, ctx->cnn_mode, (reinterpret_cast<uintptr_t>(d_crops) & 15) == 0, ctx->tune_conv_geom, n, ctx->n_cus);
+    if (!plan_prepares(p)) return TREXHIP_OK;
+    const Pass f{*net, p, ctx->stream, ctx->cnn_mode, d_crops, n, nullptr, nullptr};
+    stage_begin(ctx, TREXHIP_STAGE_PREPARE);
+    launch_prep(f, PREP_LISTS | PREP_ACT3);
+    stage_end(ctx, TREXHIP_STAGE_PREPARE);
+    TH_CHECK_HIP(hipGetLastError());
+    ctx->prepared.set(ctx->prepared.make(d_crops, n, ctx->cnn_mode, ctx->tune_conv_geom, ctx->stream));
+    return TREXHIP_OK;
+}
+
+int trexhip_identify_prepare_stats(trexhip_ctx* ctx, uint32_t* records, uint32_t* hits) {
+    if (!ctx) { set_error("trexhip_identify_prepare_stats: null ctx"); return TREXHIP_E_INVALID; }
+    if (records) *records = ctx->prepared.records;
+    if (hits) *hits = ctx->prepared.hits;
+    return TREXHIP_OK;
 }
 
 int trexhip_identify(trexhip_ctx* ctx, const uint8_t* crops, int32_t n, float* probs) {
@@ -1724,6 +1776,7 @@
 int trexhip_set_identity_precision(trexhip_ctx* ctx, int32_t mode) {
     if (!ctx || mode < 0 || mode > 3) { set_error("trexhip_set_identity_precision: mode must be one of TREXHIP_CNN_*"); return TREXHIP_E_INVALID; }
     ctx->cnn_mode = mode;
+    ctx->prepared.precision_changed();
     return TREXHIP_OK;
 }
 
@@ -1766,6 +1819,7 @@
 
 namespace trexhip {
 void net_free(trexhip_ctx* ctx) {
+    ctx->prepared.closed();
     free_net(static_cast<Net*>(ctx->net)); ctx->net = nullptr;
     free_net(static_cast<Net*>(ctx->cat)); ctx->cat = nullptr;
 }
diff --git a/trex_amd/csrc/cnn_prepared.h b/trex_amd/csrc/cnn_prepared.h
--- /dev/null
+++ b/trex_amd/csrc/cnn_prepared.h
@@ -0,0 +1,40 @@
+#pragma once
+#include <cstdint>
+
+namespace trexhip {
+
+struct PreparedKey {
+    const void* crops;
+    int n, mode, geom;
+    const void* stream;
+    uint64_t weights_gen, batch_gen;
+};
+inline bool operator==(const PreparedKey& a, const PreparedKey& b) {
+    return a.crops == b.crops && a.n == b.n && a.mode == b.mode && a.geom == b.geom && a.stream == b.stream && a.weights_gen == b.weights_gen &&
+           a.batch_gen == b.batch_gen;
+}
+
+struct PreparedState {
+    bool valid = false;
+    PreparedKey key{};
+    uint64_t weights_gen = 0, batch_gen = 0;
+    uint32_t records = 0, hits = 0;
+
+    PreparedKey make(const void* crops, const int n, const int mode, const int geom, const void* stream) const {
+        return {crops, n, mode, geom, stream, weights_gen, batch_gen};
+    }
+    void set(const PreparedKey& k) { key = k; valid = true; ++records; }
+    void drop() { valid = false; }
+    bool consume(const PreparedKey& k) {
+        const bool hit = valid && key == k;
+        valid = false;
+        hits += hit ? 1u : 0u;
+        return hit;
+    }
+    void weights_loaded() { ++weights_gen; drop(); }
+    void precision_changed() { drop(); }
+    void batch_reallocated() { ++batch_gen; drop(); }
+    void closed() { drop(); }
+};
+
+}
diff --git a/trex_amd/csrc/internal.h b/trex_amd/csrc/internal.h
--- a/trex_amd/csrc/internal.h
+++ b/trex_amd/csrc/internal.h
@@ -5,6 +5,7 @@
 #include <string>
 #include <vector>
 #include "../../include/trexhip.h"
+#include "cnn_prepared.h"
 
 #define TREXHIP_ROW_SLOT 16
 #define TREXHIP_CTR_STRIDE 32
@@ -128,6 +129,9 @@
 
     trexhip::Mem mem;
     trexhip::BlobTables tables;
+    hipEvent_t fetch_ev = nullptr;
+    hipStream_t fetch_stream = nullptr;
+    bool fetch_pending = false;
     trexhip::LabelState label;
     uint8_t* d_bg = nullptr;
     uint8_t* d_staging = nullptr;
@@ -155,6 +159,7 @@
     trexhip::Scratch med;
     trexhip::Pass2 pass2;
     int cnn_mode = TREXHIP_CNN_FP16X3;
+    trexhip::PreparedState prepared;
 
     bool profiling = false;
     int tune_conv_geom = 0;
@@ -178,6 +183,7 @@
 void stage_begin(trexhip_ctx* ctx, int stage);
 void stage_end(trexhip_ctx* ctx, int stage);
 void net_free(trexhip_ctx* ctx);
+int fetch_wait(trexhip_ctx* ctx);
 int launch_pending(trexhip_ctx* ctx);
 int launch_morphology(trexhip_ctx* ctx, const uint8_t* d_frames, int n, const uint32_t** result);
 int launch_rethreshold(trexhip_ctx* ctx, int thr, int method, const double* ranges, int n_ranges, const int32_t* d_blob_thr);
diff --git a/trex_amd/csrc/posture.hip b/trex_amd/csrc/posture.hip
--- a/trex_amd/csrc/posture.hip
+++ b/trex_amd/csrc/posture.hip
@@ -787,6 +787,7 @@
     } else if (table != 0) { set_error("trexhip_posture_device: table must be 0 (detect) or 1 (re-threshold)"); return TREXHIP_E_INVALID; }
     const BlobTables& t = table == 0 ? ctx->tables : ctx->pass2.tables;
     TH_CHECK_HIP(hipSetDevice(ctx->p.device));
+    if (const int rc = fetch_wait(ctx)) return rc;
     const PosturePlan plan(pp, t, n_blobs, false);
     if (int rc = launch_posture(ctx, plan, t, n_blobs, PostureOut{reinterpret_cast<float2*>(d_outline), reinterpret_cast<float4*>(d_segments), d_info}, nullptr, nullptr)) return rc;
     TH_CHECK_HIP(hipGetLastError());
@@ -897,6 +898,7 @@
     hipStream_t s = ctx->stream;
     const dim3 g256((unsigned)((n + 255) / 256));
     hipLaunchKernelGGL(k_auto_init, g256, dim3(256), 0, s, n, (int)track_posture_threshold, a, d_info);
+    if (const int rc = fetch_wait(ctx)) return rc;
     PosturePlan plan(pp, ctx->tables, n, true);
     for (int round = 0; round < 51; ++round) {
         int rc = trexhip_rethreshold_per_blob_device(ctx, 0, a.thr, method, nullptr, 0);
diff --git a/trex_amd/csrc/segment.hip b/trex_amd/csrc/segment.hip
--- a/trex_amd/csrc/segment.hip
+++ b/trex_amd/csrc/segment.hip
@@ -1482,6 +1482,7 @@
 }
 
 int launch_segment(trexhip_ctx* ctx, const uint8_t* d_frames, int n) {
+    if (const int rc = fetch_wait(ctx)) return rc;
     SegCfg c = ctx->cfg;
     c.B = n;
     ctx->batch_invert = c.invert; ctx->batch_zero_bg = c.zero_bg;
diff --git a/trex_amd/csrc/split.hip b/trex_amd/csrc/split.hip
--- a/trex_amd/csrc/split.hip
+++ b/trex_amd/csrc/split.hip
@@ -302,6 +302,7 @@
                        split_lds_bytes(S_PX, S_RUNS, S_SUB), ctx->stream, C, ctx->d_frames,
                        ctx->d_bg, ctx->tables.d_info, ctx->tables.d_blob_frame, ctx->tables.d_blobs, ctx->tables.d_runs, d_presumed, n_blobs, d_thr, d_info);
     bool huge = false;
+    if (const int rc = fetch_wait(ctx)) return rc;
     for (int i = 0; i < n_blobs && !huge; ++i) huge = ctx->tables.h_blobs[i].n_pixels > (uint32_t)S_PX || ctx->tables.h_blobs[i].n_runs > (uint32_t)S_RUNS;
     if (huge) {
         const int bytes = split_lds_bytes(S_PX_HUGE, S_RUNS_HUGE, S_SUB_HUGE);
diff --git a/trex_amd/csrc/unpack.hip b/trex_amd/csrc/unpack.hip
--- a/trex_amd/csrc/unpack.hip
+++ b/trex_amd/csrc/unpack.hip
@@ -308,6 +308,7 @@
     if (ctx->p.width > 32768) { set_error("trexhip_load_frames_v6_device: LegacyShortHorizontalLine holds x1 < 32768 (pv.h:36)"); return TREXHIP_E_UNSUPPORTED; }
     if (ctx->p.max_blobs > 65535) { set_error("trexhip_load_frames_v6_device: a frame holds at most 65535 objects (u16 n, pv.cpp:686)"); return TREXHIP_E_UNSUPPORTED; }
     TH_CHECK_HIP(hipSetDevice(ctx->p.device));
+    if (int rc = fetch_wait(ctx)) return rc;
     const size_t B = (size_t)ctx->p.max_batch, W = (size_t)ctx->p.width, H = (size_t)ctx->p.height, NB = (size_t)ctx->p.max_blobs;
     if (int rc = ensure_staging(ctx, "trexhip_load_frames_v6_device")) return rc;
     if (int rc = ctx->load.reserve(ctx, B * NB * sizeof(LoadBlob) + B * sizeof(LoadFrame), "trexhip_load_frames_v6_device")) return rc;
diff --git a/trex_amd/pipeline.py b/trex_amd/pipeline.py
--- a/trex_amd/pipeline.py
+++ b/trex_amd/pipeline.py
@@ -64,7 +64,7 @@
     def identify(self, step_idx):
         pl, seg = self.pl, self.seg
         o = pl.opt
-        res = self.res = seg.fetch_raw()
+        res = self.res = seg.fetch_raw() if pl.with_posture else seg.fetch_begin_raw()
         n = self.n = int(res.total_blobs)
         assert n <= pl.rows, "identity table too small"
         if self.hi is not None:
@@ -78,6 +78,7 @@
                     seg.crops_posture_device(self.crops.data_ptr(), n, self.p_minfo.data_ptr())
                 else:
                     seg.crops_device(self.crops.data_ptr(), n, normalization=1 if o["normalize"] == "moments" else 0)
+                seg.identify_prepare_device(self.crops.data_ptr(), n)
                 if self.after is not None and n > 1024:
                     self.stream.wait_event(self.after.done)
                 seg.identify_device(self.crops.data_ptr(), n, self.probs.data_ptr())
@@ -106,6 +107,7 @@
             self.done.record(self.stream)
 
     def drain(self):
+        self.seg.fetch_wait()
         self.stream.synchronize()
         if self.copy_stream is not None:
             self.copy_stream.synchronize()
```

Measured after the change: 49680, median of 6. +2.3%, better.
